# genome/breakdancer

Hardware: AMD Instinct MI355X
Metric: read-pairs/s, records resident in HBM -> scored SV table (SURVEY 8d timing i); end to end from BAM: config.timings.bam_to_table (vs_baseline is taken there) (higher is better)
Workload: dtype int32

## Files before the change

breakdancer_amd/csrc/bdx_api.hip:

```cpp
#include <hip/hip_runtime.h>

#include <algorithm>
#include <atomic>
#include <functional>
#include <memory>
#include <chrono>
#include <cmath>
#include <cstdio>
#include <cstddef>
#include <cstring>
#include <string>
#include <thread>
#include <unordered_map>
#include <utility>
#include <vector>

#include "../../include/bdx.h"
#include "bdx_buf.h"
#include "bdx_dev.h"
#include "bdx_k3.h"
#include "bdx_shard.h"
#include "bdx_scan.h"
#include "bdx_walk.h"
#include "bdx_bam_dev.h"
// ... 81 lines not shown
    std::vector<uint32_t> cnt;
    std::vector<uint32_t> cnt_local;
    uint32_t g_covered = 0;
    int32_t g_window = 0;
    uint32_t ntiles = 0, tstride = 0;
    Compact cp{};
    K3Arrays k3{};
    K4Arrays k4{};
    std::vector<double> log_tail;
    bool collect_support = false;
    std::vector<uint32_t> ov_cnt;
    uint32_t ov_covered = 0;
    bool replayed = false;
    bool use_stash = false;
    std::atomic<int> sizing{0};
    std::string sizing_err;
    std::vector<uint32_t> sup_off;
    std::vector<uint64_t> sup_idx;
    std::vector<uint8_t> sup_flag;
    std::vector<float> seqcov, lib_density, key_density;
    std::vector<HostRegion> regions;
    std::vector<uint32_t> r_pk;
    const HostRegion* reg = nullptr;
    size_t nreg = 0;
    const uint32_t* rpk = nullptr;
    std::vector<GroupPart> parts;
    WalkResult walk;
    std::unique_ptr<WalkScratch, void (*)(WalkScratch*)> walk_scratch{nullptr, walk_scratch_free};
    uint32_t n_printed = 0;
    uint32_t n_sv_host = 0;
    int speculate = 2;
    int spec_test = 0;
    uint32_t last_na = 0;
    size_t last_n = 0;
    uint32_t count_chunks = 0;
    uint32_t na_alloc = 0;
    bool region_of_fused = false;
    uint32_t join_table_clean = 0;
    float stage_ms[kNumStages] = {0};
    Event ev[8];

    Event ev_copy;
    bool copy_pending = false;
    bool k1_live = false;
    uint32_t k1_done = 0, k1_cap_tiles = 0;
    struct Stage {
        PinBuf buf;
        size_t cap = 0;
        Event done;
        bool busy = false;
    };
    Stage ring[4];
    int ring_next = 0, ring_cur = -1;
    struct KeySeg { uint64_t begin; const uint64_t* host; const uint16_t* host_qlen; const uint64_t* host_check; };
    std::vector<KeySeg> key_segs;
    DevBuf b_seg;

    size_t cls_n = (size_t)-1;
    DevBuf b_qin, b_qout;
    bool mark_dup = false;
    bool dup_done = false;
    uint64_t dup_marked = 0, dup_groups = 0;
    KdScratch kd;
};

namespace {

int fail(bdx_ctx* c, int code, const std::string& msg) {
    if (c) c->err = msg;
    return code;
}
#define NOT_WHILE_SIZING(c)                                                                                                              \
    do {                                                                                                                                 \
        if ((c)->sizing.load(std::memory_order_acquire))                                                                                 \
            return fail(c, BDX_ESTATE, "the buffers of the later stages are being sized on another thread (bdx_bamdec_finish has not returned)"); \
    } while (0)
int hipfail(bdx_ctx* c, hipError_t e, const char* what) {
    return fail(c, BDX_EHIP, std::string(what) + ": " + hipGetErrorString(e));
}
#define HIPCHK(ctx, expr)                                   \
    do {                                                    \
        hipError_t _e = (expr);                             \
        if (_e != hipSuccess) return hipfail(ctx, _e, #expr); \
    } while (0)
#define BDX_TRY(expr)                      \
    do {                                   \
        const int _rc = (expr);            \
        if (_rc != BDX_OK) return _rc;     \
    } while (0)

size_t round_up(size_t x, size_t m) { return (x + m - 1) / m * m; }

hipError_t next_lb_stamp(bdx_ctx* c, uint32_t* out) {
    if (((++c->lb_seq) & 0x3FFFFFFFu) == 0) {
        if (c->sb.b_lb.p) { const hipError_t e = hipMemsetAsync(c->sb.b_lb.p, 0, c->sb.b_lb.bytes, c->stream); if (e != hipSuccess) return e; }
        if (c->sb.b_ws6.p) { const hipError_t e = hipMemsetAsync(c->sb.b_ws6.p, 0, c->sb.b_ws6.bytes, c->stream); if (e != hipSuccess) return e; }
        ++c->lb_seq;
    }
    *out = c->lb_seq & 0x3FFFFFFFu;
    return hipSuccess;
}

int alloc_reads(bdx_ctx* c, size_t cap) {
    cap = round_up(std::max<size_t>(cap, 1), 1024);
    if (cap <= c->cap) return BDX_OK;
    if (c->copy_stream) HIPCHK(c, hipStreamSynchronize(c->copy_stream));
    HIPCHK(c, hipStreamSynchronize(c->stream));
    c->k1_live = false;
    struct Col { DevBuf* b; size_t esz; const void** slot; };
    Col cols[] = {{&c->b_tid, 4, (const void**)&c->d.tid},     {&c->b_pos, 4, (const void**)&c->d.pos},
                  {&c->b_mtid, 4, (const void**)&c->d.mtid},   {&c->b_mpos, 4, (const void**)&c->d.mpos},
                  {&c->b_isize, 4, (const void**)&c->d.isize}, {&c->b_flag, 2, (const void**)&c->d.flag},
                  {&c->b_qlen, 2, (const void**)&c->d.qlen},   {&c->b_mapq, 1, (const void**)&c->d.mapq},
                  {&c->b_lib, 1, (const void**)&c->d.lib},     {&c->b_bam, 1, (const void**)&c->d.bam},
                  {&c->b_key, 8, (const void**)&c->d.key},     {&c->b_check, 8, (const void**)&c->d.check}};
    for (Col& col : cols) {
        if (col.b == &c->b_check && !c->use_check) continue;
        DevBuf nb;
        HIPCHK(c, nb.ensure(cap * col.esz));
        if (c->n) HIPCHK(c, hipMemcpyAsync(nb.p, col.b->p, c->n * col.esz, hipMemcpyDeviceToDevice, c->stream));
        HIPCHK(c, hipStreamSynchronize(c->stream));
        col.b->release();
        *col.b = std::move(nb);
        *col.slot = col.b->p;
    }
    c->cap = cap;
    return BDX_OK;
}

void stage_view(const bdx_ctx::Stage& st, bdx_batch_buf* out) {
    char* p = (char*)st.buf.p;
    const size_t K = st.cap;
    out->name_key = (uint64_t*)p; p += K * 8;
    out->name_check = (uint64_t*)p; p += K * 8;
    out->tid = (int32_t*)p; p += K * 4;
    out->pos = (int32_t*)p; p += K * 4;
    out->mtid = (int32_t*)p; p += K * 4;
    out->mpos = (int32_t*)p; p += K * 4;
    out->isize = (int32_t*)p; p += K * 4;
    out->flag = (uint16_t*)p; p += K * 2;
    out->qlen = (uint16_t*)p; p += K * 2;
    out->mapq = (uint8_t*)p; p += K;
    out->lib = (uint8_t*)p; p += K;
    out->bam = (uint8_t*)p;
    out->capacity = K;
}

enum class RegionDst { HostAndHbm, Hbm };
struct StageDims {
    uint32_t na = 0;
    int nkeys = 0, nlibs = 0;
    bool use_check = false;
    bool k2_clears_join = false;
    RegionDst regions = RegionDst::HostAndHbm;
    bool groups_in_hbm = false, table_in_hbm = false;
    uint32_t k6_cap = 0;
    int big_walk = -1;
    uint32_t join_n = 0, join_own = 0, join_slots = 0;
    bool join_pair_lo = false;

    uint32_t join_groups() const { return join_n / 2 + 1; }
    uint32_t k6_regions() const { return std::max(na, k6_cap); }
    int walks_big() const { return big_walk >= 0 ? big_walk : (k6_regions() > 500000u ? 1 : 0); }
};

StageDims stage_dims(const bdx_ctx* c, uint32_t na) {
    StageDims d;
    d.na = na; d.nkeys = c->nkeys; d.nlibs = c->nlibs; d.use_check = c->use_check;
    d.k2_clears_join = c->force_direct_join || (!c->bucketed_join && na <= kDirectJoinMax);
    d.groups_in_hbm = c->groups_in_hbm; d.table_in_hbm = c->table_in_hbm; d.k6_cap = c->k6_cap;
    d.big_walk = c->big_walk_mode >= 0 ? c->big_walk_mode : (c->last_big_groups >= 0 ? (c->last_big_groups > 2000 ? 1 : 0) : -1);
    d.join_n = d.join_own = na; d.join_slots = d.k2_clears_join ? direct_join_slots(na) : 0;
    return d;
}

int pass1_prepare(bdx_ctx* c, uint32_t tiles_cap);
int presize_stages(bdx_ctx* c, const StageDims& dm);
int presize_stages_here(bdx_ctx* c, const StageDims& dm);
int pass1_classify(bdx_ctx* c, uint32_t upto, bool timed);

constexpr uint32_t kStreamTilesMin = 4096;

int enqueue_batch(bdx_ctx* c, const bdx_batch& b, bool lazy_keys) {
    if (c->n + b.n > c->cap) {
        BDX_TRY(alloc_reads(c, std::max(c->n + b.n, c->cap * 2)));
    }
    const size_t o = c->n, n = b.n;
    if (c->mark_dup && c->dup_done && o)
        return fail(c, BDX_ESTATE, "duplicates of this load are marked already: reads cannot be appended behind a run (bdx_reset_reads starts the next load)");
    hipStream_t s = c->copy_stream;
    if (o == 0) {
        c->key_segs.clear();
        const uint64_t tiles = (c->cap + kTile - 1) / kTile;
        if (tiles <= 0xFFFFFFFFull) {
            BDX_TRY(pass1_prepare(c, (uint32_t)tiles));
            c->k1_live = !c->mark_dup;
        }
    }
    hipStream_t s2 = s;
    HIPCHK(c, hipMemcpyAsync((void*)(c->d.tid + o), b.tid, n * 4, hipMemcpyHostToDevice, s));
    HIPCHK(c, hipMemcpyAsync((void*)(c->d.pos + o), b.pos, n * 4, hipMemcpyHostToDevice, s2));
    HIPCHK(c, hipMemcpyAsync((void*)(c->d.mtid + o), b.mtid, n * 4, hipMemcpyHostToDevice, s));
    HIPCHK(c, hipMemcpyAsync((void*)(c->d.mpos + o), b.mpos, n * 4, hipMemcpyHostToDevice, s2));
    HIPCHK(c, hipMemcpyAsync((void*)(c->d.isize + o), b.isize, n * 4, hipMemcpyHostToDevice, s));
    HIPCHK(c, hipMemcpyAsync((void*)(c->d.flag + o), b.flag, n * 2, hipMemcpyHostToDevice, s2));
    HIPCHK(c, hipMemcpyAsync((void*)(c->d.mapq + o), b.mapq, n, hipMemcpyHostToDevice, s2));
    if (c->nlibs > 1) HIPCHK(c, hipMemcpyAsync((void*)(c->d.lib + o), b.lib, n, hipMemcpyHostToDevice, s2));
    if (c->nbams > 1) HIPCHK(c, hipMemcpyAsync((void*)(c->d.bam + o), b.bam, n, hipMemcpyHostToDevice, s2));
    const uint64_t* dev_view = nullptr;
    const uint16_t* dev_qlen = nullptr;
    const uint64_t* dev_check = nullptr;
    if (lazy_keys && c->key_segs.size() < 64) {
        auto device_view = [](const void* hp) -> void* {
            hipPointerAttribute_t attr{};
            void* dp = nullptr;
            if (hipPointerGetAttributes(&attr, hp) == hipSuccess && attr.type == hipMemoryTypeHost &&
                hipHostGetDevicePointer(&dp, (void*)hp, 0) == hipSuccess)
                return dp;
            (void)hipGetLastError();
            return nullptr;
        };
        dev_view = (const uint64_t*)device_view(b.name_key);
        dev_qlen = dev_view ? (const uint16_t*)device_view(b.qlen) : nullptr;
        if (dev_qlen && c->use_check) dev_check = (const uint64_t*)device_view(b.name_check);
        if (!dev_qlen || (c->use_check && !dev_check)) dev_view = nullptr;
    }
    if (!dev_view) {
        HIPCHK(c, hipMemcpyAsync((void*)(c->d.key + o), b.name_key, n * 8, hipMemcpyHostToDevice, s2));
        HIPCHK(c, hipMemcpyAsync((void*)(c->d.qlen + o), b.qlen, n * 2, hipMemcpyHostToDevice, s));
        if (c->use_check) HIPCHK(c, hipMemcpyAsync((void*)(c->d.check + o), b.name_check, n * 8, hipMemcpyHostToDevice, s2));
    }
    if (c->key_segs.empty() || dev_view || c->key_segs.back().host)
        c->key_segs.push_back(bdx_ctx::KeySeg{(uint64_t)o, dev_view, dev_qlen, dev_check});
    HIPCHK(c, hipEventRecord(c->ev_copy, s));
    c->copy_pending = true;
    c->n += n;
    c->ran = false;
    if (o == 0) c->dup_done = false;
    if (c->k1_live) {
        const uint32_t full = (uint32_t)(c->n / kTile);
        if (full >= c->k1_done + kStreamTilesMin) {
            HIPCHK(c, hipStreamWaitEvent(c->stream, c->ev_copy, 0));
            c->copy_pending = false;
            BDX_TRY(pass1_classify(c, full, false));
        }
    }
    return BDX_OK;
}

}

extern "C" {

void bdx_opts_default(bdx_opts* o) {
    if (!o) return;
    o->min_len = 7; o->cut_sd = 3; o->max_sd = 1000000000; o->min_map_qual = 35; o->min_read_pair = 2;
    o->seq_coverage_lim = 1000; o->buffer_size = 100; o->transchr_rearrange = 0; o->fisher = 0;
    o->illumina_long_insert = 0; o->cn_lib = 0; o->print_af = 0; o->score_threshold = 30; o->chr_restricted = 0;
}

const char* bdx_strerror(int code) {
    switch (code) {
        case BDX_OK: return "ok";
        case BDX_EINVAL: return "invalid argument";
        case BDX_ENOMEM: return "out of memory";
        case BDX_EHIP: return "HIP runtime error";
        case BDX_ESTATE: return "call out of order";
        case BDX_ELIMIT: return "limit exceeded";
        default: return "internal error";
    }
}
const char* bdx_last_error(const bdx_ctx* ctx) { return ctx ? ctx->err.c_str() : ""; }
int bdx_device(const bdx_ctx* ctx) { return ctx ? ctx->device : -1; }
void* bdx_stream(const bdx_ctx* ctx) { return ctx ? (void*)ctx->stream : nullptr; }

int bdx_create(bdx_ctx** out, const bdx_opts* opts, const bdx_lib* libs, int nlibs, int nbams, int ntids,
               int max_read_window_size0, int device) {
    if (!out || !opts || !libs || nlibs < 1 || nbams < 1) return BDX_EINVAL;
    if (nlibs > 255 || nbams > 254) return BDX_ELIMIT;
    const int nkeys = opts->cn_lib ? nlibs : nbams;
    if (nkeys > 60) return BDX_ELIMIT;
    for (int i = 0; i < nlibs; ++i)
        if (libs[i].bam_index < 0 || libs[i].bam_index >= nbams) return BDX_EINVAL;
    int ndev = 0;
    if (hipGetDeviceCount(&ndev) != hipSuccess || ndev <= 0 || device < 0 || device >= ndev) return BDX_EHIP;
    if (hipSetDevice(device) != hipSuccess) return BDX_EHIP;
    std::unique_ptr<bdx_ctx> c(new (std::nothrow) bdx_ctx);
    if (!c) return BDX_ENOMEM;
    c->device = device;
    c->opts = *opts;
    c->libs.assign(libs, libs + nlibs);
    c->nlibs = nlibs; c->nbams = nbams; c->ntids = ntids; c->nkeys = nkeys; c->w0 = max_read_window_size0;
    if (c->stream.create(hipStreamNonBlocking) != hipSuccess) return BDX_EHIP;
    for (auto& e : c->ev)
        if (e.create() != hipSuccess) return BDX_EHIP;
    if (c->copy_stream.create(hipStreamNonBlocking) != hipSuccess) return BDX_EHIP;
    if (c->ev_copy.create(hipEventDisableTiming) != hipSuccess) return BDX_EHIP;
    for (auto& st : c->ring)
        if (st.done.create(hipEventDisableTiming) != hipSuccess) return BDX_EHIP;
    if (c->ev_groups.create(hipEventDisableTiming) != hipSuccess) return BDX_EHIP;
    if (c->ev_regions.create(hipEventDisableTiming) != hipSuccess) return BDX_EHIP;
    std::vector<DevLib> dl(nlibs);
    for (int i = 0; i < nlibs; ++i) {
        dl[i].upper = libs[i].uppercutoff;
        dl[i].lower = libs[i].lowercutoff;
        dl[i].min_mapq = libs[i].min_mapping_quality < 0 ? opts->min_map_qual : libs[i].min_mapping_quality;
        dl[i].key = opts->cn_lib ? i : libs[i].bam_index;
    }
    std::vector<float> means(nlibs);
    for (int i = 0; i < nlibs; ++i) means[i] = libs[i].mean_insertsize;
    if (c->b_libs.ensure(nlibs * sizeof(DevLib)) != hipSuccess ||
        hipMemcpy(c->b_libs.p, dl.data(), nlibs * sizeof(DevLib), hipMemcpyHostToDevice) != hipSuccess ||
        c->b_lib_mean.ensure(nlibs * 4) != hipSuccess ||
        hipMemcpy(c->b_lib_mean.p, means.data(), nlibs * 4, hipMemcpyHostToDevice) != hipSuccess)
        return BDX_EHIP;
    *out = c.release();
    return BDX_OK;
}

void bdx_destroy(bdx_ctx* c) {
    if (!c) return;
    (void)hipSetDevice(c->device);
// ... 323 lines not shown
    c->na_alloc = 0;
    c->regions.clear(); c->r_pk.clear(); c->parts.clear();
    c->reg = nullptr; c->nreg = 0; c->rpk = nullptr;
    c->walk.clear();
    if (!c->walk_scratch) c->walk_scratch.reset(walk_scratch_new());
    c->n_printed = 0;
    memset(&c->counts, 0, sizeof(c->counts));
    for (float& m : c->stage_ms) m = 0;

    if (c->copy_pending) {
        HIPCHK(c, hipStreamWaitEvent(s, c->ev_copy, 0));
        c->copy_pending = false;
    }
    if (!(c->k1_live && c->k1_cap_tiles >= ntiles)) {
        BDX_TRY(pass1_prepare(c, ntiles));
    }
    c->k1_live = false;
    if (c->mark_dup && c->k1_done == 0) {
        BDX_TRY(mark_duplicates(c));
    }
    const uint32_t tstride = c->tstride;
    const bool time_k1 = (c->stage_timing || c->seq % kK1EventPeriod == 0) && c->k1_done == 0 && ntiles > 0;
    {
        BDX_TRY(pass1_classify(c, ntiles, time_k1));
    }
    FinalizeParams fp{};
    fp.ntiles = ntiles; fp.tstride = tstride; fp.nblk = 0;
    fp.nfold = std::max<uint32_t>(1, std::min<uint32_t>(64, (ntiles + 1023) / 1024));
    HIPCHK(c, c->b_fold.ensure((size_t)nbams * fp.nfold * sizeof(MonoRec)));
    fp.fold_part = c->b_fold.as<MonoRec>();
    fp.nlibs = nlibs; fp.nbams = nbams; fp.nkeys = nkeys; fp.ncols = ncols; fp.ncnt = ncnt; fp.w0 = c->w0;
    fp.tile_tot = c->b_tile_tot.as<uint32_t>(); fp.tile_pre = c->b_tile_pre.as<uint32_t>(); fp.tile_mono = c->b_tile_mono.as<MonoRec>();
    {
        const uint32_t nsuper = (ntiles + kK2TilesPerWave - 1) / kK2TilesPerWave;
        const uint32_t round = 4096;
        const uint32_t rounds = std::max<uint32_t>(1, (nsuper + round - 1) / round);
        const uint32_t max_chunks = c->dbg_max_chunks > 0 ? (uint32_t)std::min(c->dbg_max_chunks, (int)kMaxChunks) : (uint32_t)kMaxChunks;
        fp.chunk_super = round * ((rounds + max_chunks - 1) / max_chunks);
        fp.nchunk = std::max<uint32_t>(1, (nsuper + fp.chunk_super - 1) / fp.chunk_super);
        HIPCHK(c, c->b_chunk_tot.ensure((size_t)ncols * kMaxChunks * 8));
        fp.chunk_tot = c->b_chunk_tot.as<uint32_t>();
        fp.chunk_base = fp.chunk_tot + (size_t)ncols * kMaxChunks;
    }
    fp.blk_cnt = c->b_blk_cnt.as<uint32_t>(); fp.cnt = c->b_cnt.as<uint32_t>(); fp.p1 = c->b_p1.as<Pass1>();
    HIPCHK(c, c->b_kdens.ensure(64 * 4));
    fp.libs = c->b_libs.as<DevLib>(); fp.cn_lib = c->opts.cn_lib; fp.key_density = c->b_kdens.as<float>();
    fp.cnt_host = c->h_cnt.as<uint32_t>(); fp.p1_host = c->h_p1.as<Pass1>();
    memset(c->h_p1.p, 0, sizeof(Pass1));
    HIPCHK(c, c->h_flags.ensure(64));
    ++c->seq;
    fp.flag_host = c->h_flags.as<uint32_t>(); fp.flag_value = c->seq;
    fp.na_cap = na_cap;
    fp.count_host = post_count && c->poll ? c->h_count.as<uint64_t>() : nullptr; fp.count_stamp = c->seq;
    c->count_chunks = fp.count_host ? fp.nchunk : 0;
    c->fp_deferred = fp;
    c->finalize2_deferred = defer_second;
    launch_finalize(fp, s, !defer_second);
    c->k1_timed = time_k1;
    return wait ? wait_pass1(c) : BDX_OK;
}

int wait_pass1(bdx_ctx* c) {
    const int ncnt = c->nlibs * kNumFlags + c->nlibs + c->nbams;
    if (!wait_flag(c, 0, c->seq)) {
        HIPCHK(c, hipStreamSynchronize(c->stream));
        if (c->h_flags.p && *((volatile uint32_t*)c->h_flags.p) != c->seq) return fail(c, BDX_EINTERNAL, "the pass-1 record did not arrive: its kernel was not launched");
    }
    c->p1 = *c->h_p1.as<Pass1>();
    c->cnt_local.assign(c->h_cnt.as<uint32_t>(), c->h_cnt.as<uint32_t>() + ncnt);
    if (c->k1_timed) {
        float ms = 0;
        if (hipEventElapsedTime(&ms, c->ev[0], c->ev[1]) == hipSuccess) c->k1_ms_last = ms;
    }
    c->stage_ms[0] = c->k1_ms_last;
    if (c->p1.n_anom > kMaxAnomalous) return fail(c, BDX_ELIMIT, "more than 2^31 anomalous reads in one context");
    if (!c->na_alloc && c->p1.n_anom) c->na_alloc = (uint32_t)std::min<uint64_t>((uint64_t)c->p1.n_anom + c->p1.n_anom / 8 + 1024, kMaxAnomalous);
    c->cls_n = c->n;
    return BDX_OK;
}

int32_t window_from(const bdx_ctx* c, const uint32_t* cnt, uint32_t covered) {
    int W = c->w0;
    for (int i = 0; i < c->nlibs; ++i) {
        const int nd = (int)(cnt[i * kNumFlags + F_LARGE] + cnt[i * kNumFlags + F_SMALL]);
        const int tmp = nd > 0 ? (int)((float)covered / (float)nd) : 50;
        W = std::min(W, tmp);
    }
    return W;
}

int set_pass1(bdx_ctx* c, const uint32_t* cnt, uint32_t covered, int32_t window, bool upload) {
    const int nlibs = c->nlibs, nkeys = c->nkeys;
    const int ncnt = nlibs * kNumFlags + nlibs + c->nbams;
    c->cnt.assign(cnt, cnt + ncnt);
    c->g_covered = covered;
    c->g_window = window;
    const uint32_t* lib_cnt = c->cnt.data() + nlibs * kNumFlags;
    const uint32_t* bam_cnt = lib_cnt + nlibs;
    c->seqcov.assign(nlibs, 0.f);
    c->lib_density.assign(nlibs, 0.f);
    c->key_density.assign(nkeys, 0.000001f);
    for (int i = 0; i < nlibs; ++i) {
        float covg = 0;
        if (lib_cnt[i] != 0 && covered != 0) covg = float(lib_cnt[i]) * c->libs[i].readlens / covered;
        c->seqcov[i] = covg;
        float dens = 0.000001f;
        if (c->opts.cn_lib) {
            if (lib_cnt[i] != 0) dens = float(lib_cnt[i]) / covered;
        } else {
            dens = float(bam_cnt[c->libs[i].bam_index]) / covered;
        }
        c->lib_density[i] = dens;
        c->key_density[c->opts.cn_lib ? i : c->libs[i].bam_index] = dens;
    }
    struct { uint32_t covered; int32_t window; } hdr{covered, window};
    static_assert(offsetof(Pass1, covered_ref_len) == 0 && offsetof(Pass1, window) == 4, "Pass1 header layout");
    if (upload) {
        HIPCHK(c, hipMemcpyAsync(c->b_p1.p, &hdr, sizeof(hdr), hipMemcpyHostToDevice, c->stream));
        HIPCHK(c, hipStreamSynchronize(c->stream));
    }
    return BDX_OK;
}

#define SZCHK(expr)                                                                                       \
    do {                                                                                                  \
        const hipError_t _e = (expr);                                                                     \
        if (_e != hipSuccess) { *err = std::string(#expr) + ": " + hipGetErrorString(_e); return BDX_EHIP; } \
    } while (0)

hipError_t size_c_maxq(StageBufs& b, size_t cap) { return b.b_c_maxq.ensure(cap * 4); }
hipError_t size_out_deg(StageBufs& b, size_t cap) { return b.b_out_deg.ensure(cap * 6 * 4); }
hipError_t size_join_words(StageBufs& b, size_t n_own, bool pair_lo) {
    const hipError_t e = b.b_partner.ensure(n_own * 4);
    return e == hipSuccess && pair_lo ? b.b_pair_lo.ensure(n_own * 4) : e;
}
hipError_t size_zero_once(DevBuf& b, size_t bytes, hipStream_t s) {
    if (b.bytes >= bytes) return hipSuccess;
    const hipError_t e = b.ensure(bytes);
    return e == hipSuccess ? hipMemsetAsync(b.p, 0, b.bytes, s) : e;
}

int size_compact(StageBufs& b, const StageDims& d, std::string* err) {
    if (!d.na) return BDX_OK;
    if (d.na > kMaxAnomalous) { *err = "more than 2^31 anomalous reads in one context"; return BDX_ELIMIT; }
    const size_t cap = d.na;
    SZCHK(b.b_c_tid.ensure(cap * 4)); SZCHK(b.b_c_pos.ensure(cap * 4)); SZCHK(b.b_c_isize.ensure(cap * 4));
    SZCHK(b.b_c_meta.ensure(cap * 4)); SZCHK(b.b_c_key.ensure(cap * 8)); SZCHK(b.b_c_nn.ensure(cap * 4));
    SZCHK(b.b_c_idx.ensure(cap * 4));
    if (d.use_check) SZCHK(b.b_c_check.ensure(cap * 8));
    SZCHK(b.b_c_pk.ensure(cap * 4 * d.nkeys));
    SZCHK(size_c_maxq(b, cap));
    if (d.k2_clears_join) {
        SZCHK(b.b_t_key.ensure((size_t)direct_join_slots(d.na) * 8));
        SZCHK(size_join_words(b, cap, true));
    }
    return BDX_OK;
}

int size_cut(StageBufs& b, const StageDims& d, hipStream_t s, std::string* err) {
    if (!d.na) return BDX_OK;
    const size_t cap = d.na;
    for (DevBuf* u : {&b.b_cand, &b.b_pre_q, &b.b_pre_rev, &b.b_pre_nonctx, &b.b_c_first, &b.b_c_rid, &b.b_region_of}) SZCHK(u->ensure(cap * 4));
    SZCHK(size_c_maxq(b, cap));
    if (d.regions != RegionDst::Hbm) {
        SZCHK(b.h_regs.ensure(cap * sizeof(RegionRec)));
        SZCHK(b.h_pk.ensure(cap * 2 * d.nkeys * 4));
    }
    SZCHK(b.b_r_rec.ensure(cap * sizeof(RegionRec)));
    SZCHK(b.b_r_pk.ensure(cap * 2 * d.nkeys * 4));
    if (d.regions == RegionDst::HostAndHbm) {
        SZCHK(size_out_deg(b, cap));
        SZCHK(b.h_counts0.ensure(sizeof(StageCounts)));
    }
    SZCHK(size_zero_once(b.b_lb, 5 * (scan_grid(d.na, 1) + 1) * 8, s));
    return BDX_OK;
}

int size_join(StageBufs& b, const StageDims& d, std::string* err) {
    if (!d.join_n) return BDX_OK;
    if (d.groups_in_hbm) SZCHK(b.b_groups.ensure((size_t)d.join_groups() * sizeof(GroupRec)));
    else SZCHK(b.h_groups.ensure((size_t)d.join_groups() * sizeof(GroupRec)));
    SZCHK(size_join_words(b, d.join_own, d.join_slots && d.join_pair_lo));
    if (d.join_slots) SZCHK(b.b_t_key.ensure((size_t)d.join_slots * 8));
    return BDX_OK;
}

struct K6Caps {
    uint32_t sv, term, cn, lib_stride;
    size_t p2, nsort;
};
K6Caps k6_caps(const StageDims& d) {
    K6Caps k{};
    const uint32_t na = d.k6_regions();
    k.sv = na / 2 + 1; k.term = na / 2 + 1; k.cn = (na / 2 + 1) * (uint32_t)d.nkeys;
    k.lib_stride = (uint32_t)std::min(d.nlibs, kK6LibStride);
    k.p2 = 1;
    while (k.p2 < k.sv) k.p2 <<= 1;
    k.nsort = std::min<size_t>(k.sv, kK6RankSortMax);
    return k;
}

int size_k6(StageBufs& b, const StageDims& d, hipStream_t s, std::string* err) {
    const size_t cap = d.k6_regions();
    if (!cap) return BDX_OK;
    const K6Caps k = k6_caps(d);
    SZCHK(size_out_deg(b, cap));
    SZCHK(b.b_parts.ensure(cap * sizeof(PartRec)));
    SZCHK(b.b_rs.ensure(cap * sizeof(RegSum)));
    SZCHK(b.b_members.ensure(cap * kK6MaxMembers * sizeof(MemberInfo)));
    SZCHK(b.b_own.ensure(cap * 7 * 4 + 64 * 4 * 4));
    if (d.walks_big()) SZCHK(b.b_member_ids.ensure(cap * kK6BigMembers * 4));
    SZCHK(b.b_slot.ensure(cap * sizeof(SvOut)));
    SZCHK(b.b_lib_stage.ensure(cap * k.lib_stride * sizeof(LibStage)));
    SZCHK(b.b_cn_stage.ensure(cap * (size_t)d.nkeys * sizeof(CnStage) + 16));
    SZCHK(b.b_t_lambda.ensure((size_t)k.term * 8)); SZCHK(b.b_t_k.ensure((size_t)k.term * 4));
    if (d.table_in_hbm) {
        SZCHK(b.b_sv_out.ensure((size_t)k.sv * sizeof(SvOut))); SZCHK(b.b_sv_key.ensure((size_t)k.sv * 8));
        SZCHK(b.b_lib_index_out.ensure((size_t)k.term * 4)); SZCHK(b.b_lib_pairs_out.ensure((size_t)k.term * 4));
        SZCHK(b.b_cn_key_out.ensure((size_t)k.cn * 4 + 16)); SZCHK(b.b_cn_value_out.ensure((size_t)k.cn * 4 + 16));
        SZCHK(b.b_ltail_out.ensure((size_t)k.term * 8));
    } else {
        SZCHK(b.h_sv_out.ensure((size_t)k.sv * sizeof(SvOut)));
        SZCHK(b.h_lib_index.ensure((size_t)k.term * 4)); SZCHK(b.h_lib_pairs.ensure((size_t)k.term * 4));
        SZCHK(b.h_cn_key.ensure((size_t)k.cn * 4 + 16)); SZCHK(b.h_cn_value.ensure((size_t)k.cn * 4 + 16));
        SZCHK(b.h_ltail_dev.ensure((size_t)k.term * 8));
    }
    SZCHK(b.h_counts2.ensure(sizeof(StageCounts)));
    SZCHK(b.b_sv_src.ensure((size_t)k.sv * 16)); SZCHK(b.b_ltail.ensure((size_t)k.term * 8));
    SZCHK(b.b_dlists.ensure((size_t)k.term * 4 + (size_t)k.cn * 8 + 64));
    SZCHK(b.b_ins.ensure(k.p2 * 12 + (size_t)k.sv * 8 + ((size_t)k.sv + 1) * 16 + k.nsort * 12 + k.nsort * 4 * kK6RankSlices + 64));
    SZCHK(size_zero_once(b.b_ws6, 4 * (scan_grid((uint32_t)cap, 1) + 1) * 8, s));
    return BDX_OK;
}

int do_compact(bdx_ctx* c) {
    HIPCHK(c, hipSetDevice(c->device));
    hipStream_t s = c->stream;
    const int nkeys = c->nkeys;
    const uint32_t na = c->na_alloc;
    if (c->stage_timing) HIPCHK(c, hipEventRecord(c->ev[2], s));
    Compact& cp = c->cp;
    cp = Compact{};
    c->k3 = K3Arrays{};
    if (na) {
        const StageDims dm = stage_dims(c, na);
        BDX_TRY(size_compact(c->sb, dm, &c->err));
        const StageBufs& b = c->sb;
        cp.tid = b.b_c_tid.as<int32_t>(); cp.pos = b.b_c_pos.as<int32_t>(); cp.isize = b.b_c_isize.as<int32_t>();
        cp.meta = b.b_c_meta.as<uint32_t>(); cp.key = b.b_c_key.as<uint64_t>(); cp.nn = b.b_c_nn.as<uint32_t>();
        cp.idx = b.b_c_idx.as<uint32_t>();
        cp.check = c->use_check ? b.b_c_check.as<uint64_t>() : nullptr;
        cp.pk = b.b_c_pk.as<uint32_t>(); cp.cap = na;
        K2Params k2{};
        k2.r = c->d; k2.n = c->n; k2.ntiles = c->ntiles; k2.tstride = c->tstride; k2.nkeys = nkeys; k2.nlibs = c->nlibs; k2.libs = c->b_libs.as<DevLib>();
        k2.cls = c->b_cls.as<uint8_t>(); k2.tile_pre = c->b_tile_pre.as<uint32_t>(); k2.c = cp;
        k2.tile_tot = c->b_tile_tot.as<uint32_t>(); k2.stash = c->use_stash ? c->b_stash.as<StashRec>() : nullptr;
        k2.chunk_tot = c->fp_deferred.chunk_tot; k2.chunk_base = c->fp_deferred.chunk_base; k2.chunk_super = c->fp_deferred.chunk_super;
        k2.fill_ptr[0] = b.b_c_maxq.as<uint32_t>(); k2.fill_words[0] = na; k2.fill_value[0] = 0u;
        c->join_table_clean = 0;
        if (dm.k2_clears_join) {
            const uint32_t slots = dm.join_slots;
            k2.fill_ptr[1] = b.b_t_key.as<uint32_t>(); k2.fill_words[1] = 2 * slots; k2.fill_value[1] = 0xFFFFFFFFu;
            k2.fill_ptr[2] = b.b_partner.as<uint32_t>(); k2.fill_words[2] = na; k2.fill_value[2] = 0xFFFFFFFFu;
            k2.fill_ptr[3] = b.b_pair_lo.as<uint32_t>(); k2.fill_words[3] = na; k2.fill_value[3] = 0xFFFFFFFFu;
            c->join_table_clean = slots;
        }
        {
            size_t ns = 0;
            BDX_TRY(upload_key_segs(c, &ns));
            if (ns) {
                k2.nseg = (int)ns;
                k2.seg_begin = c->b_seg.as<uint64_t>();
                k2.seg_ptr = (const uint64_t* const*)(c->b_seg.as<uint64_t>() + ns + 1);
                k2.seg_qlen = (const uint16_t* const*)(c->b_seg.as<uint64_t>() + 2 * ns + 1);
                k2.seg_check = (const uint64_t* const*)(c->b_seg.as<uint64_t>() + 3 * ns + 1);
            }
        }
        launch_k2(k2, k2_lds_bytes(nkeys), s, c->finalize2_deferred ? &c->fp_deferred : nullptr);
        c->finalize2_deferred = false;
    }
    if (c->finalize2_deferred) {
        launch_finalize2_only(c->fp_deferred, s);
        c->finalize2_deferred = false;
    }
    if (c->stage_timing) HIPCHK(c, hipEventRecord(c->ev[3], s));
    return BDX_OK;
}

void own_borrowed_regions(bdx_ctx* c) {
    if (!c->reg || (const void*)c->reg != c->sb.h_regs.p) return;
    const HostRegion* r = c->reg;
    const uint32_t* pk = c->rpk;
    const size_t n = c->nreg;
    std::vector<HostRegion> keep(r, r + n);
    std::vector<uint32_t> keep_pk;
    if (pk) keep_pk.assign(pk, pk + n * 2 * (size_t)c->nkeys);
    c->regions.swap(keep); c->r_pk.swap(keep_pk);
    c->reg = c->regions.data(); c->rpk = c->r_pk.data();
}

int do_cut(bdx_ctx* c, const uint32_t* tid_tail, RegionDst dst) {
    HIPCHK(c, hipSetDevice(c->device));
    hipStream_t s = c->stream;
    const uint32_t na = c->na_alloc;
    if (na) {
        StageDims dm = stage_dims(c, na);
        dm.regions = dst;
        BDX_TRY(size_cut(c->sb, dm, s, &c->err));
        const StageBufs& b = c->sb;
        K3Arrays& k3 = c->k3;
        const bool for_k6 = dst == RegionDst::HostAndHbm;
        k3.cap = na;
        k3.cand = b.b_cand.as<int32_t>(); k3.pre_q = b.b_pre_q.as<uint32_t>(); k3.pre_rev = b.b_pre_rev.as<uint32_t>();
        k3.pre_nonctx = b.b_pre_nonctx.as<uint32_t>(); k3.c_first = b.b_c_first.as<uint32_t>();
        k3.c_maxq = b.b_c_maxq.as<int32_t>(); k3.c_rid = b.b_c_rid.as<int32_t>(); k3.region_of = b.b_region_of.as<int32_t>();
        k3.r_rec = for_k6 ? b.h_regs.as<RegionRec>() : b.b_r_rec.as<RegionRec>();
        k3.r_pk = for_k6 ? b.h_pk.as<uint32_t>() : b.b_r_pk.as<uint32_t>();
        if (for_k6) {
            k3.r_rec_dev = b.b_r_rec.as<RegionRec>(); k3.r_pk_dev = b.b_r_pk.as<uint32_t>(); k3.out_deg = b.b_out_deg.as<uint32_t>();
            k3.host_copy_later = (!c->bucketed_join && na <= kDirectJoinMax) ? 1 : 0;
            memset(b.h_counts0.p, 0, sizeof(StageCounts));
            k3.counts_host = b.h_counts0.as<StageCounts>();
        } else {
            k3.r_rec_dev = nullptr; k3.r_pk_dev = nullptr; k3.host_copy_later = 0;
        }
        k3.lb_state = b.b_lb.as<unsigned long long>();
        HIPCHK(c, next_lb_stamp(c, &k3.lb_stamp));
        k3.counts = c->b_counts.as<StageCounts>();
        c->region_of_fused = for_k6 && !c->bucketed_join && na <= kDirectJoinMax;
        launch_k3(k3, c->cp, c->b_p1.as<Pass1>(), na, c->opts.min_len, c->opts.seq_coverage_lim, c->nkeys, tid_tail, !c->region_of_fused, s);
        if (for_k6 && !k3.host_copy_later) {
            BDX_TRY(signal_ready(c, 3, c->ev_regions));
        }
    }
    if (c->stage_timing) HIPCHK(c, hipEventRecord(c->ev[4], s));
    return BDX_OK;
}

int do_join_local(bdx_ctx* c, uint32_t n, const Entries& en, const uint32_t* n_ptr) {
    hipStream_t s = c->stream;
    K4Arrays& k4 = c->k4;
    k4 = K4Arrays{};
    if (!n) return BDX_OK;
    const bool direct = c->force_direct_join || (!c->bucketed_join && n <= kDirectJoinMax);
    StageDims dm = stage_dims(c, c->na_alloc);
    dm.join_n = n;
    dm.join_own = en.n_local ? std::min<uint32_t>(n, std::max<uint32_t>(c->na_alloc, 1u)) : n;
    dm.join_slots = !direct ? 0u : (c->join_table_clean && (uint64_t)n * 2 <= c->join_table_clean) ? c->join_table_clean : direct_join_slots(n);
    dm.join_pair_lo = en.want_pair_lo != 0;
    BDX_TRY(size_join(c->sb, dm, &c->err));
    StageBufs& b = c->sb;
    k4.g_cap = dm.join_groups();
    k4.g_rec = c->groups_in_hbm ? b.b_groups.as<GroupRec>() : b.h_groups.as<GroupRec>();
    k4.partner = b.b_partner.as<int32_t>();
    if (direct) {
        const uint32_t slots = dm.join_slots;
        const size_t n_own = dm.join_own;
        const bool want_lo = en.c_rid || en.want_pair_lo;
        if (c->join_table_clean != slots) {
            HIPCHK(c, hipMemsetAsync(b.b_t_key.p, 0xFF, (size_t)slots * 8, s));
            HIPCHK(c, hipMemsetAsync(b.b_partner.p, 0xFF, n_own * 4, s));
            if (en.want_pair_lo) HIPCHK(c, hipMemsetAsync(b.b_pair_lo.p, 0xFF, n_own * 4, s));
        }
        k4.pair_lo = ((c->join_table_clean == slots && want_lo) || en.want_pair_lo) ? b.b_pair_lo.as<int32_t>() : nullptr;
        c->join_table_clean = 0;
        k4.direct = 1; k4.t_mask = slots - 1;
        k4.t_key = b.b_t_key.as<uint64_t>(); k4.t_idx = b.b_t_idx.as<int32_t>();
        launch_k4_join_only(k4, en, n_ptr, n, c->b_counts.as<StageCounts>(), s);
        return BDX_OK;
    }
    uint32_t nb = 1, lg = 0;
    while (nb < (uint32_t)kMaxBuckets && (size_t)nb * 384 < n) { nb <<= 1; ++lg; }
    k4.nbuckets = nb; k4.log2b = lg;
    if ((size_t)nb * 4 > b.b_bcnt.bytes) {
        HIPCHK(c, b.b_bcnt.ensure((size_t)kMaxBuckets * 4));
        HIPCHK(c, hipMemsetAsync(b.b_bcnt.p, 0, b.b_bcnt.bytes, s));
    }
    HIPCHK(c, b.b_boff.ensure((nb + 1) * 4)); HIPCHK(c, b.b_bcur.ensure(nb * 4));
    HIPCHK(c, b.b_e_key.ensure((size_t)n * 8)); HIPCHK(c, b.b_e_idx.ensure((size_t)n * 4));
    HIPCHK(c, b.b_t_key.ensure((size_t)n * 16)); HIPCHK(c, b.b_t_idx.ensure((size_t)n * 8));
    k4.bcnt = b.b_bcnt.as<uint32_t>(); k4.boff = b.b_boff.as<uint32_t>(); k4.bcur = b.b_bcur.as<uint32_t>();
    k4.e_key = b.b_e_key.as<uint64_t>(); k4.e_idx = b.b_e_idx.as<uint32_t>();
    k4.t_key = b.b_t_key.as<uint64_t>(); k4.t_idx = b.b_t_idx.as<int32_t>();
    launch_k4_join_only(k4, en, n_ptr, n, c->b_counts.as<StageCounts>(), s);
    return BDX_OK;
}

constexpr uint32_t kBorrowRegionsMin = 32768;
void decode_regions(bdx_ctx* c, const RegionRec* rr, const uint32_t* pk, uint32_t nr, uint32_t ph, bool borrow) {
    static_assert(sizeof(HostRegion) == sizeof(RegionRec) && offsetof(HostRegion, first) == offsetof(RegionRec, first), "region layout");
    const int nkeys = c->nkeys;
    if (borrow && !ph) {
        c->reg = (const HostRegion*)rr; c->nreg = nr; c->rpk = pk;
        return;
    }
    c->regions.resize(nr + ph);
    if (ph) c->regions[0] = HostRegion{-1, -1, -1, 0, 0, 0, 0, 0, 0};
    if (nr) memcpy(c->regions.data() + ph, rr, (size_t)nr * sizeof(RegionRec));
    c->r_pk.assign((size_t)ph * 2 * nkeys, 0u);
    c->r_pk.insert(c->r_pk.end(), pk, pk + (size_t)nr * 2 * nkeys);
    c->reg = c->regions.data(); c->nreg = c->regions.size(); c->rpk = c->r_pk.data();
}

void decode_groups(bdx_ctx* c, const GroupRec* gr, uint32_t ng, uint32_t ph) {
    c->parts.resize(ng);
    for (uint32_t i = 0; i < ng; ++i) {
        const uint64_t k = gr[i].key;
        c->parts[i] = GroupPart{(uint32_t)(k >> 38) + ph, (uint32_t)((k >> 12) & ((1u << 26) - 1)) + ph, (uint8_t)(k & 15),
                                (uint8_t)((k >> 4) & 255), gr[i].pairs, gr[i].sum_isize};
    }
}

int k6_prepare(bdx_ctx* c, bool force_host, int rounds) {
    hipStream_t s = c->stream;
    K6Arrays& a = c->k6;
    a = K6Arrays{};
    const StageDims dm = stage_dims(c, c->na_alloc);
    const uint32_t na = dm.k6_regions();
    if (!na) return BDX_OK;
    BDX_TRY(size_k6(c->sb, dm, s, &c->err));
    const StageBufs& b = c->sb;
    const K6Caps k = k6_caps(dm);
    const int nkeys = c->nkeys, nlibs = c->nlibs;
    const size_t cap = na, p2 = k.p2, svc = k.sv, nsort = k.nsort;
    a.sv_cap = k.sv; a.term_cap = k.term; a.cn_cap = k.cn; a.lib_stride = k.lib_stride;
    a.old_key = b.b_ins.as<uint64_t>(); a.hs_key_dev = a.old_key + p2;
    a.old_slot = (uint32_t*)(a.hs_key_dev + svc); a.ins_T = a.old_slot + p2; a.ins_src = a.ins_T + svc + 1;
    a.ins_pre_l = a.ins_src + svc + 1; a.ins_pre_c = a.ins_pre_l + svc + 1;
    a.sorted_key = (uint64_t*)(((uintptr_t)(a.ins_pre_c + svc + 1) + 7) & ~(uintptr_t)7); a.sorted_slot = (uint32_t*)(a.sorted_key + nsort);
    a.rank_part = a.sv_cap > 2048u ? a.sorted_slot + nsort : nullptr;
    a.sv_begin = b.b_sv_src.as<uint2>(); a.sv_src = (uint32_t*)(a.sv_begin + a.sv_cap); a.ltail = b.b_ltail.as<double>();
    a.d_lib_index = b.b_dlists.as<int32_t>(); a.d_cn_key = a.d_lib_index + a.term_cap; a.d_cn_value = (float*)(a.d_cn_key + a.cn_cap);
    a.cap = na;
    a.r_rec = c->k6_r_rec ? c->k6_r_rec : b.b_r_rec.as<RegionRec>(); a.r_pk = c->k6_r_pk ? c->k6_r_pk : b.b_r_pk.as<uint32_t>();
    a.taint = c->k6_taint;
    a.region_of = c->k3.region_of; a.partner = c->k4.partner; a.pair_lo = c->k4.pair_lo; a.meta = c->cp.meta; a.isize = c->cp.isize;
    a.in_groups = c->k6_in_groups; a.in_goff = c->k6_in_goff; a.first_of = c->k6_in_groups ? c->k6_in_goff : nullptr;
    a.parts = b.b_parts.as<PartRec>();
    a.rs = b.b_rs.as<RegSum>();
    a.out_deg = b.b_out_deg.as<uint32_t>(); a.label = a.out_deg + cap; a.bad_v = a.out_deg + 2 * cap; a.bad = a.out_deg + 3 * cap;
    a.mcount = a.out_deg + 4 * cap; a.pcount = a.out_deg + 5 * cap;
    a.members = b.b_members.as<MemberInfo>();
    a.own_nsv = b.b_own.as<uint32_t>(); a.own_nacc = a.own_nsv + cap; a.own_ncn = a.own_nsv + 2 * cap; a.own_first = a.own_nsv + 3 * cap; a.slot_next = a.own_nsv + 4 * cap; a.owners = a.own_nsv + 5 * cap; a.owners_big = a.own_nsv + 6 * cap; a.emit_part = a.own_nsv + 7 * cap;
    a.big_walk = dm.walks_big();
    a.member_ids = a.big_walk ? b.b_member_ids.as<uint32_t>() : nullptr;
    a.sv_stage = b.b_slot.as<SvOut>(); a.lib_stage = b.b_lib_stage.as<LibStage>(); a.cn_stage = b.b_cn_stage.as<CnStage>();
    if (c->table_in_hbm) {
        a.sv_out = b.b_sv_out.as<SvOut>(); a.lib_index = b.b_lib_index_out.as<int32_t>(); a.lib_pairs = b.b_lib_pairs_out.as<int32_t>();
        a.cn_key = b.b_cn_key_out.as<int32_t>(); a.cn_value = b.b_cn_value_out.as<float>();
        a.sv_key = b.b_sv_key.as<unsigned long long>();
    } else {
        a.sv_out = b.h_sv_out.as<SvOut>(); a.lib_index = b.h_lib_index.as<int32_t>(); a.lib_pairs = b.h_lib_pairs.as<int32_t>();
        a.cn_key = b.h_cn_key.as<int32_t>(); a.cn_value = b.h_cn_value.as<float>();
    }
    a.sv_vx = a.sv_key ? a.sv_src + a.sv_cap : nullptr;
    a.t_lambda = b.b_t_lambda.as<double>(); a.t_k = b.b_t_k.as<int32_t>();
    a.g_rec = c->k4.g_rec; a.g_cap = c->k4.g_cap;
    a.lb_state = b.b_ws6.as<unsigned long long>();
    HIPCHK(c, next_lb_stamp(c, &a.lb_stamp));
    a.counts = c->b_counts.as<StageCounts>();
    a.hist = c->b_cnt.as<uint32_t>();
    a.key_density = c->b_kdens.as<float>();
    a.lib_mean = c->b_lib_mean.as<float>();
    a.counts_host = c->h_counts.as<StageCounts>();
    a.counts_host2 = b.h_counts2.as<StageCounts>();
    memset(c->h_counts.p, 0, sizeof(StageCounts));
    memset(b.h_counts2.p, 0, sizeof(StageCounts));
    a.p1 = c->b_p1.as<Pass1>();
    a.nlibs = nlibs; a.nkeys = nkeys; a.min_read_pair = c->opts.min_read_pair; a.chr_restricted = c->opts.chr_restricted;
    a.period = std::max(1, c->opts.buffer_size + 1);
    a.force_host = force_host ? 1 : 0;
    a.ins_plain = c->dbg_ins_plain;
    a.asm_plain = c->dbg_asm_plain;
    a.propagation_rounds = rounds ? rounds : (a.big_walk ? kK6LabelRoundsBig : kK6LabelRounds);
    if (c->poll) {
        a.flag_value = c->seq;
        a.flag_groups = c->h_flags.as<uint32_t>() + 1;
        if (c->k3.host_copy_later) a.flag_regions = c->h_flags.as<uint32_t>() + 3;
        a.mirror_in_walk = force_host ? 0 : 1;
    }
    return BDX_OK;
}

void k6_pairs(bdx_ctx* c) {
    if (c->k6.cap) launch_k6_pairs(c->k6, c->k6.cap, c->stream);
}
int k6_then_walk(bdx_ctx* c, void (*first)(const K6Arrays&, uint32_t, hipStream_t)) {
    const K6Arrays& a = c->k6;
    if (!a.cap) return BDX_OK;
    first(a, a.cap, c->stream);
    if (!c->poll) BDX_TRY(signal_ready(c, 1, c->ev_groups));
    launch_k6_walk(a, a.cap, c->stream);
    return BDX_OK;
}

int presize_stages(bdx_ctx* c, const StageDims& dm) {
    struct Guard {
        bdx_ctx* c;
        explicit Guard(bdx_ctx* c_) : c(c_) { c->sizing.fetch_add(1, std::memory_order_acq_rel); c->sizing_err.clear(); }
        ~Guard() { c->sizing.fetch_sub(1, std::memory_order_acq_rel); }
    } guard(c);
    std::string* err = &c->sizing_err;
    SZCHK(hipSetDevice(c->device));
    own_borrowed_regions(c);
    BDX_TRY(size_compact(c->sb, dm, err));
    BDX_TRY(size_cut(c->sb, dm, c->stream, err));
    BDX_TRY(size_join(c->sb, dm, err));
    return size_k6(c->sb, dm, c->stream, err);
}

int presize_stages_here(bdx_ctx* c, const StageDims& dm) {
    const int r = presize_stages(c, dm);
    if (r != BDX_OK) c->err = c->sizing_err;
    return r;
}

int do_k6_table(bdx_ctx* c) {
    hipStream_t s = c->stream;
    K6Arrays& a = c->k6;
    const uint32_t na = a.cap;
    if (!na) return BDX_OK;
    const WalkResult& H = c->walk;
    const uint32_t nh = (uint32_t)H.svs.size(), nt = (uint32_t)H.terms.size(), nc = (uint32_t)H.cn_key.size();
    a.nh = nh;
    if (nh) {
        const uint64_t period = (uint64_t)std::max(1, c->opts.buffer_size + 1);
        HIPCHK(c, c->h_hs_rec.ensure((size_t)nh * sizeof(SvOut)));
        HIPCHK(c, c->h_hs_aux.ensure((size_t)nh * 12 + 16));
        HIPCHK(c, c->h_hs_lists.ensure((size_t)nt * 16 + (size_t)nc * 8 + 16));
        memcpy(c->h_hs_rec.p, H.svs.data(), (size_t)nh * sizeof(HostSv));
        uint64_t* hkey = c->h_hs_aux.as<uint64_t>();
        uint32_t* hcnt = (uint32_t*)(hkey + nh);
        for (uint32_t j = 0; j < nh; ++j) {
            const uint64_t key = H.sv_key[j];
            const bool from_old = !((key >> 32) & 1ull);
            const uint64_t start = key & 0xffffffffull;
            const uint64_t T = from_old ? (key >> 33) * period : start;
            hkey[j] = (T << 34) | (from_old ? 0ull : 1ull << 33) | (start << 7);
            if (a.force_host) hkey[j] = 0;
            hcnt[j] = (uint32_t)H.svs[j].sv.lib_count | ((uint32_t)H.svs[j].sv.cn_count << 16);
        }
        double* lam = c->h_hs_lists.as<double>();
        int32_t* li = (int32_t*)(lam + nt);
        int32_t* lp = li + nt;
        int32_t* ck = lp + nt;
        float* cv = (float*)(ck + nc);
        for (uint32_t i = 0; i < nt; ++i) { lam[i] = H.terms[i].lambda; li[i] = H.lib_index[i]; lp[i] = H.lib_pairs[i]; }
        for (uint32_t i = 0; i < nc; ++i) { ck[i] = H.cn_key[i]; cv[i] = H.cn_value[i]; }
        a.hs_rec = c->h_hs_rec.as<SvOut>(); a.hs_key = hkey; a.hs_cnt = hcnt;
        a.hs_lambda = lam; a.hs_lib_index = li; a.hs_lib_pairs = lp; a.hs_cn_key = ck; a.hs_cn_value = cv;
    }
    a.ltail_host = c->table_in_hbm ? c->sb.b_ltail_out.as<double>() : (c->opts.fisher ? c->sb.h_ltail_dev.as<double>() : nullptr);
    a.fin_regions = (c->counts.n_regions && c->counts.n_regions <= na) ? c->counts.n_regions : na;
    HIPCHK(c, c->h_printed.ensure((size_t)k6_score_grid(a) * 4));
    a.printed_host = c->h_printed.as<uint32_t>();
    if (c->poll) { a.flag_done = c->h_flags.as<uint32_t>() + 2; a.flag_value = c->seq; }
    a.wire_rows = c->table_in_hbm ? 0 : 1;
    c->rows_packed = a.wire_rows != 0;
    launch_k6_table(a, na, std::log(10), c->opts.score_threshold, c->opts.fisher ? 0 : 1, s);
    if (!a.flag_done) {
        BDX_TRY(signal_ready(c, 2, nullptr));
    }
    return BDX_OK;
}

int materialize(bdx_ctx* c) {
    if (c->materialized) return BDX_OK;
    WalkResult& M = c->walk;
    M.clear();
    const uint32_t n = c->n_sv_total, nt = c->n_terms_total, nc = c->n_cn_total;
    if (c->rows_packed) {
        const SvWire* w = c->sb.h_sv_out.as<SvWire>();
        M.svs.resize(n);
        int32_t lb = 0, cb = 0;
        for (uint32_t i = 0; i < n; ++i) {
            const SvWire& r = w[i];
            HostSv& o = M.svs[i];
            bdx_sv& v = o.sv;
            const HostRegion& ra = c->reg[r.region[0]];
            const HostRegion& rb = r.region[1] >= 0 ? c->reg[r.region[1]] : ra;
            v.chr[0] = ra.tid; v.chr[1] = rb.tid;
            v.pos[0] = r.pos[0]; v.pos[1] = r.pos[1];
            v.fwd[0] = (int32_t)(ra.n - ra.rev); v.rev[0] = (int32_t)ra.rev;
            v.fwd[1] = (int32_t)(rb.n - rb.rev); v.rev[1] = (int32_t)rb.rev;
            v.flag = (int32_t)((r.bits >> 16) & 15u); v.size = r.size; v.score = r.score; v.num_reads = r.num_reads; v.printed = (int32_t)((r.bits >> 23) & 1u);
            v.region[0] = r.region[0]; v.region[1] = r.region[1];
            v.lib_begin = lb; v.lib_count = (int32_t)(r.bits & 255u); lb += v.lib_count;
            v.cn_begin = cb; v.cn_count = (int32_t)((r.bits >> 8) & 255u); cb += v.cn_count;
            v.allele_frequency = r.allele_frequency; v.logp = r.logp;
            o.grp_mask = (r.bits >> 20) & 7u; o.start = r.start;
        }
    } else {
        const HostSv* d = c->sb.h_sv_out.as<HostSv>();
        M.svs.assign(d, d + n);
    }
    M.lib_index.assign(c->sb.h_lib_index.as<int32_t>(), c->sb.h_lib_index.as<int32_t>() + nt);
    M.lib_pairs.assign(c->sb.h_lib_pairs.as<int32_t>(), c->sb.h_lib_pairs.as<int32_t>() + nt);
    M.cn_key.assign(c->sb.h_cn_key.as<int32_t>(), c->sb.h_cn_key.as<int32_t>() + nc);
    M.cn_value.assign(c->sb.h_cn_value.as<float>(), c->sb.h_cn_value.as<float>() + nc);
    if (c->opts.fisher) c->log_tail.assign(c->sb.h_ltail_dev.as<double>(), c->sb.h_ltail_dev.as<double>() + nt); else c->log_tail.clear();
    M.n_groups = c->n_groups_total;
    c->materialized = true;
    return BDX_OK;
}

int finish_table(bdx_ctx* c) {
    hipStream_t s = c->stream;
    const auto tf0 = std::chrono::steady_clock::now();
    if (!wait_flag(c, 2, c->seq)) {
        HIPCHK(c, hipStreamSynchronize(s));
        if (!flag_arrived(c, 2)) return fail(c, BDX_EINTERNAL, "the SV table did not arrive: its kernels were not launched");
    }
    const auto tf1 = std::chrono::steady_clock::now();
    static_assert(sizeof(HostSv) == sizeof(SvOut) && offsetof(HostSv, grp_mask) == offsetof(SvOut, grp_mask) &&
                      offsetof(HostSv, start) == offsetof(SvOut, start), "SV record layout");
    c->n_sv_host = (uint32_t)c->walk.svs.size();
    c->n_groups_total = c->walk.n_groups + c->counts.n_groups_dev;
    const StageCounts c2 = *c->sb.h_counts2.as<StageCounts>();
    if (c2.overflow) return fail(c, BDX_EINTERNAL, "SV list overflow");
    c->n_sv_total = c2.n_sv_dev; c->n_terms_total = c2.n_terms_dev; c->n_cn_total = c2.n_cn_dev;
    c->counts.n_sv_dev = c2.n_sv_dev - c->n_sv_host;
    {
        const uint32_t g = c->k6.printed_host ? k6_score_grid(c->k6) : 0u;
        const uint32_t* pb = c->k6.printed_host;
        uint32_t np = 0;
        for (uint32_t i = 0; i < g; ++i) np += pb[i];
        c->n_printed = np;
    }
    c->counts.n_old = c2.n_old;
    c->materialized = false;
    if (c->opts.fisher && !c->table_in_hbm) {
        materialize(c);
        finish_scores(c->opts, c->log_tail.data(), c->walk.svs.data(), c->walk.svs.size(), &c->n_printed);
    }
    const auto tf2 = std::chrono::steady_clock::now();
    c->stage_ms[8] = ms_between(tf0, tf1);
    c->stage_ms[9] = ms_between(tf1, tf2);
    c->stage_ms[10] = 0;
    c->ran = true;
    return BDX_OK;
}

int host_walk(bdx_ctx* c, int32_t last_maxq, bool any_anomalous) {
    HIPCHK(c, hipSetDevice(c->device));
    WalkInput wi{};
    wi.opts = c->opts; wi.libs = c->libs.data(); wi.nlibs = c->nlibs; wi.nbams = c->nbams; wi.nkeys = c->nkeys;
    wi.hist = c->cnt.data(); wi.covered_ref_len = c->g_covered; wi.key_density = c->key_density.data();
    wi.regions = c->reg; wi.nregions = c->nreg; wi.r_pk = c->rpk; wi.parts = &c->parts; wi.last_maxq = last_maxq;
    wi.any_anomalous = any_anomalous;
    c->walk.clear();
    if (!c->parts.empty()) greedy_walk(wi, c->walk_scratch.get(), c->walk);
    return BDX_OK;
}

int score_host_terms(bdx_ctx* c) {
    hipStream_t s = c->stream;
    const uint32_t nt = (uint32_t)c->walk.terms.size();
    if (nt) {
        HIPCHK(c, c->h_terms.ensure((size_t)nt * 20 + 16));
        double* hl = c->h_terms.as<double>();
        int32_t* hk = (int32_t*)(hl + nt);
        double* ho = (double*)((char*)c->h_terms.p + (((size_t)nt * 12 + 7) & ~(size_t)7));
        for (uint32_t i = 0; i < nt; ++i) { hl[i] = c->walk.terms[i].lambda; hk[i] = c->walk.terms[i].k; }
        launch_k5(hl, hk, ho, nt, s);
    }
    return BDX_OK;
}

int finish_host_walk(bdx_ctx* c) {
    hipStream_t s = c->stream;
    HIPCHK(c, hipStreamSynchronize(s));
    HIPCHK(c, hipGetLastError());
    const uint32_t nt = (uint32_t)c->walk.terms.size();
    const double* host_tail = nt ? (const double*)((char*)c->h_terms.p + (((size_t)nt * 12 + 7) & ~(size_t)7)) : nullptr;
    c->log_tail.assign(host_tail, host_tail + nt);
    finish_scores(c->opts, c->log_tail.data(), c->walk.svs.data(), c->walk.svs.size(), &c->n_printed);
    c->n_sv_host = c->n_sv_total = (uint32_t)c->walk.svs.size();
    c->n_terms_total = nt; c->n_cn_total = (uint32_t)c->walk.cn_key.size();
    c->n_groups_total = c->walk.n_groups;
    c->counts.n_sv_dev = 0;
    c->materialized = true;
    c->ran = true;
    return BDX_OK;
}

int collect_support(bdx_ctx* c, uint32_t ph) {
    c->sup_off.assign(1, 0);
    c->sup_idx.clear();
    c->sup_flag.clear();
    const uint32_t na = c->p1.n_anom;
    std::vector<int32_t> partner(na), region_of(na);
    std::vector<uint32_t> idx(na), meta(na);
    if (na) {
        HIPCHK(c, hipMemcpy(partner.data(), c->k4.partner, (size_t)na * 4, hipMemcpyDeviceToHost));
        HIPCHK(c, hipMemcpy(region_of.data(), c->k3.region_of, (size_t)na * 4, hipMemcpyDeviceToHost));
        HIPCHK(c, hipMemcpy(idx.data(), c->cp.idx, (size_t)na * 4, hipMemcpyDeviceToHost));
        HIPCHK(c, hipMemcpy(meta.data(), c->cp.meta, (size_t)na * 4, hipMemcpyDeviceToHost));
    }
    std::vector<std::pair<uint32_t, uint32_t>> pairs;
    for (const HostSv& hs : c->walk.svs) {
        pairs.clear();
        const uint32_t rA = (uint32_t)hs.sv.region[0], rB = (uint32_t)hs.sv.region[1];
        const uint32_t glo[3] = {rA, rA, rB}, ghi_[3] = {rA, rB, rB};
        for (uint32_t g = 0; g < 3; ++g) {
            if (!(hs.grp_mask & (1u << g))) continue;
            const uint32_t lo = glo[g], hi = ghi_[g];
            const uint32_t f = c->reg[hi].first, n = c->reg[hi].n;
            for (uint32_t j = f; j < f + n; ++j) {
                const int32_t p = partner[j];
                if (p < 0 || (uint32_t)p >= j) continue;
                if ((uint32_t)(region_of[p] + (int32_t)ph) != lo) continue;
                pairs.emplace_back(j, (uint32_t)p);
            }
        }
        std::sort(pairs.begin(), pairs.end());
        for (auto const& pr : pairs) {
            c->sup_idx.push_back(idx[pr.first]); c->sup_flag.push_back((uint8_t)meta_flag(meta[pr.first]));
            c->sup_idx.push_back(idx[pr.second]); c->sup_flag.push_back((uint8_t)meta_flag(meta[pr.second]));
        }
        c->sup_off.push_back((uint32_t)c->sup_idx.size());
    }
    return BDX_OK;
}

int replay_arrays(bdx_ctx* c, uint32_t na, const uint64_t* key, const int32_t* region_of, const uint32_t* meta, const int32_t* isize, uint32_t ph,
                  std::vector<uint32_t>* sup) {
    ReadWalkInput ri{};
    WalkInput& wi = ri.base;
    wi.opts = c->opts; wi.libs = c->libs.data(); wi.nlibs = c->nlibs; wi.nbams = c->nbams; wi.nkeys = c->nkeys;
    wi.hist = c->cnt.data(); wi.covered_ref_len = c->g_covered; wi.key_density = c->key_density.data();
    wi.regions = c->reg; wi.nregions = c->nreg; wi.r_pk = c->rpk; wi.parts = nullptr; wi.last_maxq = c->counts.last_maxq;
    wi.any_anomalous = na != 0;
    ri.n_reads = na; ri.key = key; ri.region_of = region_of; ri.meta = meta; ri.isize = isize;
    ri.phantom = ph;
    if (sup) { ri.support_off = &c->sup_off; ri.support = sup; }
    c->walk.clear();
    read_level_walk(ri, c->walk);
    c->counts.n_groups = 0; c->counts.n_pairs = 0;
    int rc = score_host_terms(c);
    if (rc == BDX_OK) rc = finish_host_walk(c);
    if (rc != BDX_OK) return rc;
    c->replayed = true;
    return BDX_OK;
}

void unify_names(uint64_t* key, const uint64_t* check, size_t n) {
    struct PairHash {
        size_t operator()(const std::pair<uint64_t, uint64_t>& p) const { return (size_t)(p.first ^ (p.second * 0x9E3779B97F4A7C15ull)); }
    };
    std::unordered_map<std::pair<uint64_t, uint64_t>, uint64_t, PairHash> ids;
    ids.reserve(n);
    for (size_t i = 0; i < n; ++i) key[i] = ids.emplace(std::make_pair(key[i], check[i]), (uint64_t)ids.size()).first->second;
}

int replay_reads(bdx_ctx* c, uint32_t ph) {
    hipStream_t s = c->stream;
    HIPCHK(c, hipStreamSynchronize(s));
    const uint32_t na = c->p1.n_anom;
    std::vector<uint64_t> key(na);
    std::vector<int32_t> region_of(na), isize(na);
    std::vector<uint32_t> meta(na);
    HIPCHK(c, hipMemcpy(key.data(), c->cp.key, (size_t)na * 8, hipMemcpyDeviceToHost));
    HIPCHK(c, hipMemcpy(region_of.data(), c->k3.region_of, (size_t)na * 4, hipMemcpyDeviceToHost));
    HIPCHK(c, hipMemcpy(meta.data(), c->cp.meta, (size_t)na * 4, hipMemcpyDeviceToHost));
    HIPCHK(c, hipMemcpy(isize.data(), c->cp.isize, (size_t)na * 4, hipMemcpyDeviceToHost));
    if (c->cp.check && na) {
        std::vector<uint64_t> check(na);
        HIPCHK(c, hipMemcpy(check.data(), c->cp.check, (size_t)na * 8, hipMemcpyDeviceToHost));
        unify_names(key.data(), check.data(), na);
    }
    if (ph)
        for (int32_t& r : region_of)
            if (r >= 0) r += (int32_t)ph;
    std::vector<uint32_t> sup;
    BDX_TRY(replay_arrays(c, na, key.data(), region_of.data(), meta.data(), isize.data(), ph, c->collect_support ? &sup : nullptr));
    if (c->collect_support) {
        std::vector<uint32_t> idx(na);
        HIPCHK(c, hipMemcpy(idx.data(), c->cp.idx, (size_t)na * 4, hipMemcpyDeviceToHost));
        c->sup_idx.resize(sup.size());
        c->sup_flag.resize(sup.size());
        for (size_t i = 0; i < sup.size(); ++i) { c->sup_idx[i] = idx[sup[i]]; c->sup_flag[i] = (uint8_t)meta_flag(meta[sup[i]]); }
    }
    return BDX_OK;
}

}

extern "C" {

int bdx_run(bdx_ctx* c) {
    if (!c) return BDX_EINVAL;
    NOT_WHILE_SIZING(c);
    const auto t_begin = std::chrono::steady_clock::now();
    hipStream_t s = c->stream;
    const bool ph_opt = 0 > c->opts.min_len && 0.0f < (float)c->opts.seq_coverage_lim;
    const bool force_host = c->host_walk_only || ph_opt || c->opts.min_read_pair < 1;
    auto enqueue_middle = [&]() -> int {
        BDX_TRY(do_compact(c));
        BDX_TRY(do_cut(c, nullptr, RegionDst::HostAndHbm));
        if (!c->na_alloc) return BDX_OK;
        Entries en{};
        en.key = c->cp.key; en.check = c->cp.check; en.region = c->k3.region_of; en.meta = c->cp.meta; en.isize = c->cp.isize;
        if (c->region_of_fused) {
            en.cand = c->k3.cand; en.c_rid = c->k3.c_rid; en.region_out = c->k3.region_of;
            en.k6_scratch = c->k3.out_deg; en.scratch_cap = c->k3.cap;
            if (c->k3.host_copy_later) {
                en.r_rec_dev = c->k3.r_rec_dev; en.r_pk_dev = c->k3.r_pk_dev; en.r_rec_host = c->k3.r_rec; en.r_pk_host = c->k3.r_pk;
                en.counts = c->b_counts.as<StageCounts>(); en.nkeys2 = 2 * c->nkeys;
            }
        }
        BDX_TRY(do_join_local(c, c->na_alloc, en, &c->b_p1.as<Pass1>()->n_anom));
        if (c->k3.host_copy_later && !c->poll) {
            BDX_TRY(signal_ready(c, 3, c->ev_regions));
        }
        BDX_TRY(k6_prepare(c, force_host, 0));
        return k6_then_walk(c, launch_k6_groups);
    };
    uint32_t guess = 0;
    const bool restored = !c->ov_cnt.empty();
    if (!restored && c->speculate == 2 && c->ran && c->last_n == c->n && c->last_na) {
        guess = c->spec_test ? std::max(1u, c->last_na / 2) : c->last_na + c->last_na / 8 + 1024;
        if (guess > kMaxAnomalous) guess = 0;
    } else if (!restored && c->speculate && c->n >= (1u << 20) && (c->speculate == 1 || c->n < (1u << 25))) {
        const uint64_t prior = (uint64_t)c->n / (c->spec_test ? 4096 : 32) + 4096;
        guess = prior > kMaxAnomalous ? 0 : (uint32_t)prior;
    }
    int rc;
    if (restored) {
        BDX_TRY(do_pass1(c));
        BDX_TRY(set_pass1(c, c->ov_cnt.data(), c->ov_covered, window_from(c, c->ov_cnt.data(), c->ov_covered), true));
        HIPCHK(c, hipMemcpyAsync(c->b_cnt.p, c->ov_cnt.data(), c->ov_cnt.size() * 4, hipMemcpyHostToDevice, s));
        HIPCHK(c, hipMemcpyAsync(c->b_kdens.p, c->key_density.data(), c->key_density.size() * 4, hipMemcpyHostToDevice, s));
        HIPCHK(c, hipStreamSynchronize(s));
        BDX_TRY(enqueue_middle());
    } else if (guess) {
        BDX_TRY(do_pass1(c, guess, false, true));
        c->na_alloc = guess;
        BDX_TRY(enqueue_middle());
        BDX_TRY(wait_pass1(c));
        BDX_TRY(set_pass1(c, c->cnt_local.data(), c->p1.covered_ref_len, c->p1.window, false));
        if (c->p1.n_anom > guess) {
            HIPCHK(c, hipStreamSynchronize(s));
            HIPCHK(c, hipMemcpy(&c->b_p1.as<Pass1>()->n_anom, &c->p1.n_anom, 4, hipMemcpyHostToDevice));
            HIPCHK(c, hipMemset(c->b_counts.p, 0, sizeof(StageCounts)));
            ++c->seq;
            c->na_alloc = c->p1.n_anom;
            BDX_TRY(enqueue_middle());
        }
    } else {
        BDX_TRY(do_pass1(c, 0, false, false, true));
        uint64_t count = 0;
        if (wait_count(c, &count)) {
            if (count > kMaxAnomalous) {
                HIPCHK(c, hipStreamSynchronize(s));
                return fail(c, BDX_ELIMIT, "more than 2^31 anomalous reads in one context");
            }
            if (count) c->na_alloc = (uint32_t)std::min<uint64_t>(count + count / 8 + 1024, kMaxAnomalous);
            BDX_TRY(enqueue_middle());
            BDX_TRY(wait_pass1(c));
            if (c->p1.n_anom != count) {
                HIPCHK(c, hipStreamSynchronize(s));
                return fail(c, BDX_EINTERNAL, "the count of anomalous reads posted ahead of the pass-1 record differs from the record's");
            }
            BDX_TRY(set_pass1(c, c->cnt_local.data(), c->p1.covered_ref_len, c->p1.window, false));
        } else {
            BDX_TRY(wait_pass1(c));
            BDX_TRY(set_pass1(c, c->cnt_local.data(), c->p1.covered_ref_len, c->p1.window, false));
            BDX_TRY(enqueue_middle());
        }
    }
    c->last_n = c->n;
    c->last_na = c->p1.n_anom;
    const uint32_t na = c->p1.n_anom;
    const uint32_t ph = (na && ph_opt) ? 1u : 0u;
    if (c->stage_timing) HIPCHK(c, hipEventRecord(c->ev[5], s));
    const auto t_h0 = std::chrono::steady_clock::now();
    auto t_h1 = t_h0;
    if (na) {
        if (!wait_flag(c, 3, c->seq)) {
            if (c->poll) HIPCHK(c, hipStreamSynchronize(s)); else HIPCHK(c, hipEventSynchronize(c->ev_regions));
            if (!flag_arrived(c, 3)) return fail(c, BDX_EINTERNAL, "the region table did not arrive: its kernels were not launched");
        }
        if ((uint64_t)c->sb.h_counts0.as<StageCounts>()->n_regions + ph > kMaxRegions) {
            HIPCHK(c, hipStreamSynchronize(s));
            return fail(c, BDX_ELIMIT, "more than 2^26 - 2 accepted regions in one context");
        }
        const uint32_t nr_host = c->sb.h_counts0.as<StageCounts>()->n_regions;
        const bool copy_first = c->dbg_regions_copy == 1 || (c->dbg_regions_copy == 0 && nr_host < kBorrowRegionsMin);
        if (copy_first) decode_regions(c, c->sb.h_regs.as<RegionRec>(), c->sb.h_pk.as<uint32_t>(), nr_host, ph, false);
        if (!wait_flag(c, 1, c->seq)) {
            if (c->poll) HIPCHK(c, hipStreamSynchronize(s)); else HIPCHK(c, hipEventSynchronize(c->ev_groups));
            if (!flag_arrived(c, 1)) return fail(c, BDX_EINTERNAL, "the pair groups did not arrive: their kernels were not launched");
        }
        c->counts = *c->h_counts.as<StageCounts>();
        if (!copy_first) decode_regions(c, c->sb.h_regs.as<RegionRec>(), c->sb.h_pk.as<uint32_t>(), nr_host, ph,
                                        c->dbg_regions_copy == 2 || (uint64_t)c->counts.n_groups * 8 < nr_host);
        if (c->counts.irregular) {
            t_h1 = std::chrono::steady_clock::now();
            BDX_TRY(replay_reads(c, ph));
            const auto t_r = std::chrono::steady_clock::now();
            c->stage_ms[4] = ms_between(t_h0, t_h1); c->stage_ms[5] = ms_between(t_h1, t_r); c->stage_ms[7] = ms_between(t_begin, t_r);
            return BDX_OK;
        }
        if (c->counts.overflow) return fail(c, BDX_EINTERNAL, "group list overflow");
        decode_groups(c, c->sb.h_groups.as<GroupRec>(), c->counts.n_groups, ph);
        c->last_big_groups = (int64_t)c->counts.n_groups + c->counts.n_groups_big;
    }
    t_h1 = std::chrono::steady_clock::now();
    BDX_TRY(host_walk(c, c->counts.last_maxq, na != 0));
    const auto t_h2 = std::chrono::steady_clock::now();
    if (na) {
        BDX_TRY(do_k6_table(c));
        rc = finish_table(c);
    } else {
        rc = finish_host_walk(c);
    }
    if (rc != BDX_OK) return rc;
    if (c->collect_support) {
        materialize(c);
        BDX_TRY(collect_support(c, ph));
    }
    const auto t_end = std::chrono::steady_clock::now();
    if (c->stage_timing) {
        (void)hipEventSynchronize(c->ev[5]);
        auto evms = [&](int a, int b) { float ms = 0; (void)hipEventElapsedTime(&ms, c->ev[a], c->ev[b]); return ms; };
        c->stage_ms[1] = evms(2, 3);
        c->stage_ms[2] = evms(3, 4);
        c->stage_ms[3] = evms(4, 5);
    }
    c->stage_ms[4] = ms_between(t_h0, t_h1);
    c->stage_ms[5] = ms_between(t_h1, t_h2);
    c->stage_ms[6] = ms_between(t_h2, t_end);
    c->stage_ms[7] = ms_between(t_begin, t_end);
    return BDX_OK;
}

int bdx_get_summary(const bdx_ctx* c, bdx_summary* o) {
    if (!c || !o) return BDX_EINVAL;
    if (!c->ran) return BDX_ESTATE;
    o->n_reads = c->n; o->n_anomalous = c->p1.n_anom; o->covered_ref_len = c->g_covered; o->window = c->g_window;
    o->n_candidates = c->counts.n_cand; o->n_regions = (uint32_t)c->nreg; o->n_pairs = c->counts.n_pairs;
    o->n_groups = c->n_groups_total; o->n_svs = c->n_sv_total; o->n_svs_printed = c->n_printed;
    return BDX_OK;
}

int bdx_get_counters(const bdx_ctx* c, uint32_t* lib_read_count, uint32_t* bam_read_count, uint32_t* flag_hist, float* seqcov,
                     float* density) {
    if (!c) return BDX_EINVAL;
    if (!c->ran) return BDX_ESTATE;
    const uint32_t* hist = c->cnt.data();
    const uint32_t* lib_cnt = hist + c->nlibs * kNumFlags;
    const uint32_t* bam_cnt = lib_cnt + c->nlibs;
    if (flag_hist) memcpy(flag_hist, hist, (size_t)c->nlibs * kNumFlags * 4);
    if (lib_read_count) memcpy(lib_read_count, lib_cnt, (size_t)c->nlibs * 4);
    if (bam_read_count) memcpy(bam_read_count, bam_cnt, (size_t)c->nbams * 4);
    if (seqcov) memcpy(seqcov, c->seqcov.data(), (size_t)c->nlibs * 4);
    if (density) memcpy(density, c->lib_density.data(), (size_t)c->nlibs * 4);
    return BDX_OK;
}

int bdx_get_regions(const bdx_ctx* c, bdx_region* out, size_t cap) {
    if (!c || (!out && cap)) return BDX_EINVAL;
    if (!c->ran) return BDX_ESTATE;
    const size_t n = std::min(cap, c->nreg);
    for (size_t i = 0; i < n; ++i) {
        const HostRegion& r = c->reg[i];
        const int valid = c->opts.chr_restricted ? (int)r.nonctx : (int)r.n;
        out[i] = bdx_region{r.tid, r.start, r.end, (int32_t)r.nnormal, (int32_t)(r.n - r.rev), (int32_t)r.rev, (int32_t)r.n,
                            valid >= c->opts.min_read_pair ? 1 : 0, r.maxq};
// ... 374 lines not shown
```

breakdancer_amd/csrc/bdx_k3.h:

```cpp
#pragma once
#include "../../include/bdx.h"
#include "bdx_dev.h"

namespace bdx {

struct U4;

struct StageCounts {
    uint32_t n_cand;
    uint32_t n_regions;
    int32_t last_maxq;
    uint32_t n_pairs;
    uint32_t n_groups;
    uint32_t n_entries;
    uint32_t overflow;
    uint32_t n_printed;
    uint32_t n_sv_dev;
    uint32_t n_terms_dev;
    uint32_t n_cn_dev;
    uint32_t n_groups_dev;
    uint32_t stage_sv;
    uint32_t stage_lib;
    uint32_t stage_cn;
    uint32_t n_owners;
    uint32_t n_owners_big;
    uint32_t n_groups_big;
    uint32_t n_old;
    uint32_t n_ins;
    uint32_t sort_done;
    uint32_t irregular;
};

struct RegionRec {
    int32_t tid, start, end;
    uint32_t n, rev, nonctx, nnormal;
    int32_t maxq;
    uint32_t first;
};

struct GroupRec {
    uint64_t key;
    uint32_t pairs;
    uint32_t sum_isize;
};

struct K3Arrays {
    uint32_t cap;
    int32_t* cand;
    uint32_t *pre_q, *pre_rev, *pre_nonctx;
    uint32_t* c_first;
    int32_t* c_maxq;
    int32_t* c_rid;
    int32_t* region_of;
    RegionRec* r_rec;
    uint32_t* r_pk;
    RegionRec* r_rec_dev;
    uint32_t* r_pk_dev;
    int host_copy_later;
    uint32_t* out_deg;
    unsigned long long* lb_state;
    uint32_t lb_stamp;
    StageCounts* counts;
    StageCounts* counts_host;
};

void launch_k3(const K3Arrays& a, const Compact& cp, const Pass1* p1, uint32_t n_anom_host, int min_len, int seq_coverage_lim,
               int nkeys, const uint32_t* tid_tail, bool region_of_launch, hipStream_t s);

constexpr int kMaxBuckets = 8192;
constexpr int kJoinLdsSlots = 8192;
constexpr uint32_t kDirectJoinMax = 1u << 22;
inline uint32_t direct_join_slots(uint32_t n) {
    uint32_t slots = 1024;
    while (slots < 4 * (uint64_t)n) slots <<= 1;
    return slots;
}

struct K4Arrays {
    uint32_t nbuckets;
    uint32_t log2b;
    uint32_t* bcnt;
    uint32_t* boff;
    uint32_t* bcur;
    uint64_t* e_key;
    uint32_t* e_idx;
    int32_t* partner;
    int32_t* pair_lo;
    uint64_t* t_key;
    int32_t* t_idx;
    uint32_t direct;
    uint32_t t_mask;
    GroupRec* g_rec;
    uint32_t g_cap;
};

__host__ __device__ __forceinline__ uint64_t group_pack(uint32_t rlo, uint32_t rhi, uint32_t lib, uint32_t flag) {
    return ((uint64_t)rlo << 38) | ((uint64_t)rhi << 12) | ((uint64_t)lib << 4) | (uint64_t)flag;
}
constexpr uint32_t kMaxRegions = (1u << 26) - 2;
constexpr uint32_t kMaxAnomalous = 0x7FFFFF00u;

struct Entries {
    const uint64_t* key;
    const uint64_t* check;
    const int32_t* region;
    const uint32_t* meta;
    const int32_t* isize;
    const int32_t* cand;
    const int32_t* c_rid;
    int32_t* region_out;
    const RegionRec* r_rec_dev;
    const uint32_t* r_pk_dev;
    RegionRec* r_rec_host;
    uint32_t* r_pk_host;
    const StageCounts* counts;
    int nkeys2;
    uint32_t* k6_scratch;
    uint32_t scratch_cap;
    const uint32_t* n_local;
    const uint64_t* fkey;
    const uint64_t* fcheck;
    const int32_t* fregion;
    int want_pair_lo;
};

void launch_k4_join_only(const K4Arrays& k4, const Entries& e, const uint32_t* n_ptr, uint32_t n_upper, StageCounts* counts, hipStream_t s);

constexpr int kMaxRanks = 64;
struct ExchangeEntry {
    uint64_t key;
    uint32_t order;
    int32_t region;
    uint32_t meta;
    int32_t isize;
    uint64_t check;
};
static_assert(sizeof(ExchangeEntry) == 32, "exchange entries travel as four 64-bit words");
__host__ __device__ __forceinline__ uint32_t exchange_owner(uint64_t k, uint32_t world) {
    k = (k ^ (k >> 33)) * 0xff51afd7ed558ccdull;
    k ^= k >> 29;
    return (uint32_t)(k % world);
}
struct GatherPackage { uint64_t regions_off, pk_off, groups_off; uint32_t nr, ng; };
struct GatherDesc { GatherPackage p[kMaxRanks]; int world; };
void launch_k8_place_regions(const char* all, const GatherDesc& D, uint32_t max_nr, const uint64_t* rbase, int ntids, int nkeys2, RegionRec* r_rec,
                             uint32_t* r_pk, uint32_t* err, hipStream_t s);

void launch_k5(const double* lambda, const int32_t* k, double* out, uint32_t n, hipStream_t s);

constexpr int kK6MaxMembers = 4;
constexpr int kK6MaxIn = 3;
constexpr int kK6BigMembers = 64;
constexpr int kK6LibStride = 16;
constexpr int kK6LabelRoundsBig = 8;
constexpr uint32_t kK6RankSlices = 16;
constexpr uint32_t kK6RankSortMax = 1u << 17;
constexpr int kK6LabelRounds = 2;
constexpr int kK6LabelRoundsGather = 3;

struct RegSum {
    uint32_t np_all;
    uint32_t np_emit;
    uint32_t np_self;
    uint32_t w_self;
    uint32_t n_in;
    uint32_t n_pairs;
    uint32_t n_weak;
    uint32_t big;
    uint32_t e_lo[kK6MaxIn];
    uint32_t e_w[kK6MaxIn];
    uint32_t e_off[kK6MaxIn];
    uint32_t e_cnt[kK6MaxIn];
};
constexpr uint64_t kWeakPart = 1ull << 63;

struct PartRec {
    uint64_t key;
    uint32_t pairs;
    uint32_t sum;
};

struct MemberInfo {
    uint32_t r;
    RegionRec rec;
    uint32_t np_all, np_self, w_self, n_in;
    uint32_t e_lo[kK6MaxIn], e_w[kK6MaxIn], e_off[kK6MaxIn], e_cnt[kK6MaxIn];
    uint32_t stored;
    uint32_t pad;
};
constexpr int kMemberWords = sizeof(MemberInfo) / 4;

struct SvOut {
    bdx_sv sv;
    uint32_t grp_mask;
    uint32_t start;
};

struct SvWire {
    int32_t pos[2], region[2];
    int32_t size, score, num_reads;
    float allele_frequency;
    double logp;
    uint32_t start;
    uint32_t bits;
};
static_assert(sizeof(SvWire) == 48, "twelve 32-bit words");
constexpr int kWireWords = sizeof(SvWire) / 4;

struct LibStage { int32_t lib, rc; double lambda; };
struct CnStage { int32_t key; float value; };

struct K6Arrays {
    uint32_t cap;
    const RegionRec* r_rec;
    const uint32_t* r_pk;
    const int32_t* region_of;
    const int32_t* partner;
    const int32_t* pair_lo;
    const uint32_t* meta;
    const int32_t* isize;
    const GroupRec* in_groups;
    const uint32_t* in_goff;
    const uint32_t* first_of;
    PartRec* parts;
    RegSum* rs;
    uint32_t* out_deg;
    uint32_t* label;
    uint32_t* bad_v;
    uint32_t* bad;
    uint32_t* mcount;
    uint32_t* pcount;
    MemberInfo* members;
    uint32_t* owners;
    uint32_t* own_nsv;
    uint32_t* own_nacc;
    uint32_t* own_ncn;
    uint32_t* own_first;
    uint32_t* slot_next;
    uint32_t* emit_part;
    uint32_t* owners_big;
    uint32_t* member_ids;
    SvOut* sv_stage;
    LibStage* lib_stage;
    CnStage* cn_stage;
    uint32_t lib_stride;
    uint32_t* sv_src;
    uint2* sv_begin;
    uint32_t* sv_vx;
    int32_t* d_lib_index;
    int32_t* d_cn_key;
    float* d_cn_value;
    double* t_lambda;
    int32_t* t_k;
    SvOut* sv_out;
    int32_t* lib_index;
    int32_t* lib_pairs;
    int32_t* cn_key;
    float* cn_value;
    uint32_t sv_cap, term_cap, cn_cap;
    double* ltail;
    uint32_t* printed_host;
    double* ltail_host;
    const SvOut* hs_rec;
    const uint64_t* hs_key;
    const uint32_t* hs_cnt;
    uint64_t* old_key;
    uint32_t* old_slot;
    uint64_t* sorted_key;
    uint32_t* sorted_slot;
    uint32_t* rank_part;
    uint64_t* hs_key_dev;
    uint32_t* ins_T;
    uint32_t* ins_src;
    uint32_t* ins_pre_l;
    uint32_t* ins_pre_c;
    const int32_t* hs_lib_index;
    const int32_t* hs_lib_pairs;
    const double* hs_lambda;
    const int32_t* hs_cn_key;
    const float* hs_cn_value;
    uint32_t nh;
    GroupRec* g_rec;
    uint32_t g_cap;
    unsigned long long* lb_state;
    uint32_t lb_stamp;
    StageCounts* counts;
    StageCounts* counts_host;
    StageCounts* counts_host2;
    uint32_t* flag_regions;
    uint32_t* flag_groups;
    uint32_t* flag_done;
    uint32_t flag_value;
    const uint32_t* hist;
    const float* key_density;
    const float* lib_mean;
    const Pass1* p1;
    int nlibs, nkeys, min_read_pair, chr_restricted, period, force_host;
    int mirror_in_walk;
    int big_walk;
    uint32_t fin_regions;
    int asm_plain;
    int ins_plain;
    int propagation_rounds;
    uint8_t* taint;
    int wire_rows;
    unsigned long long* sv_key;
};

void launch_k6_groups(const K6Arrays& a, uint32_t n_anom_host, hipStream_t s);
void launch_k6_pairs(const K6Arrays& a, uint32_t n_upper, hipStream_t s);
void launch_k6_components(const K6Arrays& a, uint32_t n_upper, hipStream_t s);
void launch_k6_scratch_init(uint32_t* out_deg, uint32_t cap, hipStream_t s);
void launch_k6_walk(const K6Arrays& a, uint32_t n_anom_host, hipStream_t s);
void launch_k6_table(const K6Arrays& a, uint32_t n_anom_host, double ln10, int score_threshold, int with_scores, hipStream_t s);
uint32_t k6_score_grid(const K6Arrays& a);

}
```

breakdancer_amd/csrc/bdx_scan.h:

```cpp
#pragma once
#include "bdx_dev.h"

namespace bdx {

#ifdef BDX_KPROF
static __device__ unsigned long long g_kprof[8 * 65536];
#define KPROF(row, col) do { if ((threadIdx.x & 63) == 0 && (row) < 65536u) g_kprof[(size_t)(row) * 8 + (col)] = wall_clock64(); } while (0)
#else
#define KPROF(row, col) do {} while (0)
#endif

struct U4 {
    uint32_t x, y, z, w;
};
__host__ __device__ __forceinline__ U4 operator+(const U4& a, const U4& b) { return U4{a.x + b.x, a.y + b.y, a.z + b.z, a.w + b.w}; }
__host__ __device__ __forceinline__ U4 operator-(const U4& a, const U4& b) { return U4{a.x - b.x, a.y - b.y, a.z - b.z, a.w - b.w}; }

template <class T> __device__ __forceinline__ T zero_of();
template <> __device__ __forceinline__ uint32_t zero_of<uint32_t>() { return 0u; }
template <> __device__ __forceinline__ U4 zero_of<U4>() { return U4{0, 0, 0, 0}; }

__device__ __forceinline__ uint32_t shfl_up_t(uint32_t v, int o) { return __shfl_up(v, o); }
__device__ __forceinline__ U4 shfl_up_t(const U4& v, int o) {
    return U4{(uint32_t)__shfl_up(v.x, o), (uint32_t)__shfl_up(v.y, o), (uint32_t)__shfl_up(v.z, o), (uint32_t)__shfl_up(v.w, o)};
// ... 42 lines not shown
        if (j < n) acc = acc + in(j, n);
    }
    T tot;
    block_incl_scan(acc, s_ws, &tot);
    if (threadIdx.x == 0) blk[blockIdx.x] = tot;
}

template <class T, class In, int kIters> __global__ __launch_bounds__(kScanBlock) void scan_phase1(In in, const uint32_t* n_ptr, T* blk) {
    scan_phase1_body<T, In, kIters>(in, n_ptr, blk);
}

template <class T, int kIters> __global__ __launch_bounds__(1024) void scan_phase2(T* blk, const uint32_t* n_ptr, T* total) {
    constexpr int kScanChunk = kScanBlock * kIters;
    __shared__ T s_ws[16];
    __shared__ T s_carry;
    const uint32_t n = *n_ptr;
    const uint32_t nb = (n + kScanChunk - 1) / kScanChunk;
    const int lane = threadIdx.x & 63, w = threadIdx.x >> 6;
    if (threadIdx.x == 0) s_carry = zero_of<T>();
    __syncthreads();
    for (uint32_t base = 0; base < nb; base += 1024) {
        const uint32_t i = base + threadIdx.x;
        T v = i < nb ? blk[i] : zero_of<T>();
        T inc = wave_incl_scan_t(v);
        if (lane == 63) s_ws[w] = inc;
        __syncthreads();
        T off = s_carry;
        for (int k = 0; k < w; ++k) off = off + s_ws[k];
        if (i < nb) blk[i] = off + inc - v;
        __syncthreads();
        if (threadIdx.x == 1023) s_carry = off + inc;
        __syncthreads();
    }
    if (threadIdx.x == 0) *total = s_carry;
}

template <class T, class In, class Out, int kIters, bool kSelfSum>
__global__ __launch_bounds__(kScanBlock) void scan_phase3(In in, Out out, const uint32_t* n_ptr, const T* blk) {
    constexpr int kScanChunk = kScanBlock * kIters;
    __shared__ T s_ws[kScanBlock / 64];
    const uint32_t n = *n_ptr;
    const uint32_t base = blockIdx.x * kScanChunk;
    if (base >= n) return;
    T carry;
    if (kSelfSum) {
        T acc = zero_of<T>();
        for (uint32_t i = threadIdx.x; i < blockIdx.x; i += kScanBlock) acc = acc + blk[i];
        block_incl_scan(acc, s_ws, &carry);
    } else {
        carry = blk[blockIdx.x];
    }
#pragma unroll 1
    for (int it = 0; it < kIters; ++it) {
        const uint32_t j = base + it * kScanBlock + threadIdx.x;
        if (base + it * kScanBlock >= n) break;
        T e = j < n ? in(j, n) : zero_of<T>();
        T tot;
        T inc = carry + block_incl_scan(e, s_ws, &tot);
        if (j < n) out(j, n, inc, e);
        carry = carry + tot;
    }
}

inline uint32_t scan_grid(uint32_t n_upper, int iters = kScanIters) {
    const uint32_t chunk = (uint32_t)(kScanBlock * iters);
    return n_upper ? (n_upper + chunk - 1) / chunk : 1;
}

constexpr uint32_t kScanSelfSumMax = 1024;

template <class T, int kIters = kScanIters, class In, class Out>
void scan_launch(In in, Out out, const uint32_t* n_ptr, uint32_t n_upper, T* blk_ws, T* total, hipStream_t s) {
    const uint32_t g = scan_grid(n_upper, kIters);
    hipLaunchKernelGGL((scan_phase1<T, In, kIters>), dim3(g), dim3(kScanBlock), 0, s, in, n_ptr, blk_ws);
    if (g <= kScanSelfSumMax) {
        hipLaunchKernelGGL((scan_phase3<T, In, Out, kIters, true>), dim3(g), dim3(kScanBlock), 0, s, in, out, n_ptr, blk_ws);
        return;
    }
    hipLaunchKernelGGL((scan_phase2<T, kIters>), dim3(1), dim3(1024), 0, s, blk_ws, n_ptr, total);
    hipLaunchKernelGGL((scan_phase3<T, In, Out, kIters, false>), dim3(g), dim3(kScanBlock), 0, s, in, out, n_ptr, blk_ws);
}

template <class T> struct ScanCols;
template <> struct ScanCols<uint32_t> {
    static constexpr int n = 1;
    __device__ static __forceinline__ uint32_t get(const uint32_t& v, int) { return v; }
    __device__ static __forceinline__ void set(uint32_t& v, int, uint32_t x) { v = x; }
};
template <> struct ScanCols<U4> {
    static constexpr int n = 4;
    __device__ static __forceinline__ uint32_t get(const U4& v, int c) { return c == 0 ? v.x : c == 1 ? v.y : c == 2 ? v.z : v.w; }
    __device__ static __forceinline__ void set(U4& v, int c, uint32_t x) { if (c == 0) v.x = x; else if (c == 1) v.y = x; else if (c == 2) v.z = x; else v.w = x; }
};

template <class T>
__device__ __forceinline__ T lookback_exclusive(const T& tot, unsigned long long* state, uint32_t stamp, uint32_t bid, uint32_t* s_prefix ) {
    constexpr int kCols = ScanCols<T>::n;
    constexpr int kWin = 64 / kCols;
    const unsigned long long stamp_bits = (unsigned long long)(stamp & 0x3FFFFFFFu) << 32;
    if (threadIdx.x < 64) {
        const int lane = threadIdx.x;
        if (lane < kCols)
            __hip_atomic_store(&state[(size_t)bid * kCols + lane],
                               (unsigned long long)ScanCols<T>::get(tot, lane) | stamp_bits | ((bid == 0 ? 2ull : 1ull) << 62), __ATOMIC_RELAXED,
                               __HIP_MEMORY_SCOPE_AGENT);
        const int col = lane / kWin, k = lane % kWin;
        uint32_t acc = 0;
        bool frozen = false;
        constexpr int kAhead = 4;
        for (uint32_t back = 0;; back += kWin * kAhead) {
            unsigned long long w[kAhead];
#pragma unroll
            for (int u = 0; u < kAhead; ++u) {
                const int64_t pred = (int64_t)bid - 1 - (int64_t)back - (int64_t)u * kWin - k;
                w[u] = (2ull << 62) | stamp_bits;
                if (!frozen && pred >= 0) w[u] = __hip_atomic_load(&state[(size_t)pred * kCols + col], __ATOMIC_RELAXED, __HIP_MEMORY_SCOPE_AGENT);
            }
            bool done = false;
#pragma unroll
            for (int u = 0; u < kAhead; ++u) {
                if (done) break;
                const int64_t pred = (int64_t)bid - 1 - (int64_t)back - (int64_t)u * kWin - k;
                unsigned long long x = w[u];
                if (!frozen && pred >= 0)
                    while ((x & (0x3FFFFFFFull << 32)) != stamp_bits || (x >> 62) == 0)
                        x = __hip_atomic_load(&state[(size_t)pred * kCols + col], __ATOMIC_RELAXED, __HIP_MEMORY_SCOPE_AGENT);
                const uint32_t val = (uint32_t)x, st = (uint32_t)(x >> 62);
                const uint64_t incl = __ballot(!frozen && st == 2);
                const uint64_t mine = kWin == 64 ? incl : ((incl >> (col * kWin)) & ((1ull << kWin) - 1));
                const int stop = mine ? __builtin_ctzll(mine) : kWin;
                uint32_t part = (!frozen && k <= stop) ? val : 0u;
#pragma unroll
                for (int o = 1; o < kWin; o <<= 1) part += __shfl_xor(part, o);
                acc += part;
                if (mine) frozen = true;
                if (!__ballot(!frozen)) done = true;
            }
            if (done) break;
        }
        if (k == 0) s_prefix[col] = acc;
    }
    __syncthreads();
    T carry = zero_of<T>();
#pragma unroll
    for (int c = 0; c < kCols; ++c) ScanCols<T>::set(carry, c, s_prefix[c]);
    if (threadIdx.x < kCols && bid != 0)
        __hip_atomic_store(&state[(size_t)bid * kCols + threadIdx.x],
                           (unsigned long long)(s_prefix[threadIdx.x] + ScanCols<T>::get(tot, threadIdx.x)) | stamp_bits | (2ull << 62), __ATOMIC_RELAXED,
                           __HIP_MEMORY_SCOPE_AGENT);
    return carry;
}

template <class T, class In, class Out, int kIters>
__global__ __launch_bounds__(kScanBlock) void scan_lookback(In in, Out out, const uint32_t* n_ptr, unsigned long long* state, uint32_t stamp) {
    __shared__ T s_ws[kScanBlock / 64];
    __shared__ uint32_t s_prefix[ScanCols<T>::n];
    const uint32_t n = *n_ptr;
    const uint32_t bid = blockIdx.x;
    const uint32_t base = bid * kScanBlock * kIters;
    if (base >= n) return;
    constexpr uint32_t kRow0 = ScanCols<T>::n == 4 ? 0u : 32768u;
    (void)kRow0;
    KPROF(kRow0 + bid * 4 + (threadIdx.x >> 6), 0);
    T e[kIters], inc[kIters];
#pragma unroll
    for (int it = 0; it < kIters; ++it) {
        const uint32_t j = base + it * kScanBlock + threadIdx.x;
        e[it] = j < n ? in(j, n) : zero_of<T>();
    }
    T tot = zero_of<T>();
#pragma unroll
    for (int it = 0; it < kIters; ++it) {
        T t;
        inc[it] = tot + block_incl_scan(e[it], s_ws, &t);
        tot = tot + t;
    }
    KPROF(kRow0 + bid * 4 + (threadIdx.x >> 6), 1);
    const T carry = lookback_exclusive<T>(tot, state, stamp, bid, s_prefix);
    KPROF(kRow0 + bid * 4 + (threadIdx.x >> 6), 2);
#pragma unroll
    for (int it = 0; it < kIters; ++it) {
        const uint32_t j = base + it * kScanBlock + threadIdx.x;
        if (j < n) out(j, n, carry + inc[it], e[it]);
    }
    KPROF(kRow0 + bid * 4 + (threadIdx.x >> 6), 3);
}

template <class T, int kIters = 1, class In, class Out>
void scan_launch_lb(In in, Out out, const uint32_t* n_ptr, uint32_t n_upper, unsigned long long* state, uint32_t stamp, hipStream_t s) {
    const uint32_t g = scan_grid(n_upper, kIters);
    hipLaunchKernelGGL((scan_lookback<T, In, Out, kIters>), dim3(g), dim3(kScanBlock), 0, s, in, out, n_ptr, state, stamp);
}

}
```

breakdancer_amd/csrc/k3_regions.hip:

```cpp
#include "bdx_k3.h"

#include "bdx_scan.h"

namespace bdx {

struct HeadIn {
    const int32_t* tid;
    const int32_t* pos;
    const uint32_t* meta;
    const Pass1* p1;
    __device__ U4 operator()(uint32_t j, uint32_t) const {
        const int W = p1->window;
        const bool head = j == 0 || tid[j] != tid[j - 1] || pos[j] - pos[j - 1] > W;
        const uint32_t m = meta[j];
        return U4{head ? 1u : 0u, (uint32_t)meta_qlen(m), (uint32_t)meta_rev(m), meta_flag(m) != F_CTX ? 1u : 0u};
    }
};

struct HeadOut {
    K3Arrays a;
    const int32_t* tid;
    int per_tid;
    __device__ void operator()(uint32_t j, uint32_t n, const U4& inc, const U4& e) const {
        const int c = (int)inc.x - 1;
        if (j == n - 1) a.counts->n_cand = inc.x;
        a.cand[j] = c;
        a.pre_q[j] = inc.y;
        a.pre_rev[j] = inc.z;
        a.pre_nonctx[j] = inc.w;
        if (e.x) a.c_first[c] = j;
        const int target = e.x ? c - 1 : c;
        const bool other_chromosome = per_tid && e.x && j > 0 && tid[j] != tid[j - 1];
        const int lane = (int)(threadIdx.x & 63u);
        int v = (target >= 0 && !other_chromosome) ? (int)e.y : INT32_MIN;
#pragma unroll
        for (int o = 1; o < 64; o <<= 1) {
            const int pv = __shfl_up(v, o), pt = __shfl_up(target, o);
            if (lane >= o && pt == target) v = max(v, pv);
        }
        const int nt = __shfl_down(target, 1);
        const bool last_of_run = lane == 63 || j == n - 1 || nt != target;
        if (last_of_run && target >= 0 && v != INT32_MIN) atomicMax(&a.c_maxq[target], v);
    }
};

struct CandStats {
    uint32_t first, last, n, rev, nonctx, nnormal;
    int32_t maxq;
    bool accept;
};

struct CandCtx {
    K3Arrays a;
    Compact cp;
    const Pass1* p1;
    int min_len, seq_coverage_lim;
    const uint32_t* tid_tail;
    __device__ CandStats stats(uint32_t c, uint32_t nc) const {
        CandStats s;
        const uint32_t na = p1->n_anom;
        const uint32_t f = a.c_first[c];
        const uint32_t nxt = c + 1 < nc ? a.c_first[c + 1] : na;
        const uint32_t l = nxt - 1;
        const int start = cp.pos[f], end = cp.pos[l];
        s.first = f; s.last = l; s.n = nxt - f;
        s.rev = a.pre_rev[l] - (f ? a.pre_rev[f - 1] : 0u);
        s.nonctx = a.pre_nonctx[l] - (f ? a.pre_nonctx[f - 1] : 0u);
        const bool chrom_last = tid_tail && (c + 1 == nc || cp.tid[nxt] != cp.tid[f]);
        const uint32_t* tl = chrom_last ? tid_tail + 4 * (size_t)cp.tid[f] : nullptr;
        const uint32_t e = (c + 1 < nc && !chrom_last) ? nxt : l;
        int qsum = (int)(a.pre_q[e] - a.pre_q[f]);
        int maxq = a.c_maxq[c];
        const bool tail_closes = chrom_last && tl[0];
        if (tail_closes) {
            const int tail_qlen = (int)tl[1];
            qsum += tail_qlen;
            maxq = max(maxq, tail_qlen);
        }
        s.maxq = maxq;
        const float cov = __fdiv_rn((float)qsum, (float)(end - start + 1 + maxq));
        s.accept = (end - start > min_len) && (cov < (float)seq_coverage_lim);
        const uint32_t nn_end = chrom_last ? tl[2] : (c + 1 < nc ? cp.nn[nxt] : p1->n_normal);
        s.nnormal = nn_end - cp.nn[f];
        return s;
    }
};

struct AcceptIn {
    CandCtx x;
    __device__ uint32_t operator()(uint32_t c, uint32_t nc) const { return x.stats(c, nc).accept ? 1u : 0u; }
};
struct AcceptOut {
    CandCtx x;
    int nkeys;
    __device__ void operator()(uint32_t c, uint32_t n, uint32_t inc, uint32_t e) const {
        const K3Arrays& a = x.a;
        const Compact& cp = x.cp;
        a.c_rid[c] = e ? (int)inc - 1 : -1;
        if (c != n - 1 && !e) return;
        const CandStats st = x.stats(c, n);
        if (c == n - 1) {
            a.counts->last_maxq = st.maxq; a.counts->n_regions = inc;
            if (a.counts_host) { a.counts_host->last_maxq = st.maxq; a.counts_host->n_regions = inc; a.counts_host->n_cand = n; }
        }
        if (!e) return;
        const uint32_t r = inc - 1;
        const uint32_t f = st.first, l = st.last;
        RegionRec rr;
        rr.tid = cp.tid[f]; rr.start = cp.pos[f]; rr.end = cp.pos[l];
        rr.n = st.n; rr.rev = st.rev; rr.nonctx = st.nonctx; rr.nnormal = st.nnormal;
        rr.maxq = st.maxq;
        rr.first = f;
        const bool to_host = !a.host_copy_later;
        if (to_host) a.r_rec[r] = rr;
        if (a.r_rec_dev) a.r_rec_dev[r] = rr;
        for (int k = 0; k < nkeys; ++k) {
            const uint32_t pf = cp.pk[(size_t)k * cp.cap + f], pl = cp.pk[(size_t)k * cp.cap + l];
            if (to_host) {
                a.r_pk[(size_t)r * 2 * nkeys + k] = pf;
                a.r_pk[(size_t)r * 2 * nkeys + nkeys + k] = pl;
            }
            if (a.r_pk_dev) { a.r_pk_dev[(size_t)r * 2 * nkeys + k] = pf; a.r_pk_dev[(size_t)r * 2 * nkeys + nkeys + k] = pl; }
        }
    }
};


__global__ __launch_bounds__(256) void k3_region_of_kernel(K3Arrays a, const Pass1* p1) {
    const uint32_t j = blockIdx.x * blockDim.x + threadIdx.x;
    if (j < p1->n_anom) {
        a.region_of[j] = a.c_rid[a.cand[j]];
        if (a.out_deg) {
            a.out_deg[j] = 0;
            a.out_deg[(size_t)a.cap + j] = j;
            a.out_deg[2 * (size_t)a.cap + j] = 0;
            a.out_deg[3 * (size_t)a.cap + j] = 0;
            a.out_deg[4 * (size_t)a.cap + j] = 0;
            a.out_deg[5 * (size_t)a.cap + j] = 0;
        }
    }
}

void launch_k3(const K3Arrays& a, const Compact& cp, const Pass1* p1, uint32_t n_anom_host, int min_len, int seq_coverage_lim,
               int nkeys, const uint32_t* tid_tail, bool region_of_launch, hipStream_t s) {
    if (n_anom_host == 0) return;
    const uint32_t* n_ptr = &p1->n_anom;
    HeadIn hin{cp.tid, cp.pos, cp.meta, p1};
    HeadOut hout{a, cp.tid, tid_tail ? 1 : 0};
    const size_t nblk = scan_grid(a.cap, 1);
    if (n_anom_host > (1u << 19)) scan_launch_lb<U4, 2>(hin, hout, n_ptr, n_anom_host, a.lb_state, a.lb_stamp, s);
    else scan_launch_lb<U4, 1>(hin, hout, n_ptr, n_anom_host, a.lb_state, a.lb_stamp, s);
    const CandCtx cx{a, cp, p1, min_len, seq_coverage_lim, tid_tail};
    scan_launch_lb<uint32_t, 1>(AcceptIn{cx}, AcceptOut{cx, nkeys}, &a.counts->n_cand, n_anom_host, a.lb_state + 4 * nblk, a.lb_stamp, s);
    if (region_of_launch) hipLaunchKernelGGL(k3_region_of_kernel, dim3((n_anom_host + 255) / 256), dim3(256), 0, s, a, p1);
}

}

__global__ void k3_noop_kernel() {}
namespace bdx { void warm_k3(hipStream_t s) { hipLaunchKernelGGL(k3_noop_kernel, dim3(1), dim3(64), 0, s); } }

#ifdef BDX_KPROF
extern "C" int bdx_debug_kprof3(unsigned long long* out, size_t n) {
    const int rc = (int)hipMemcpyFromSymbol(out, HIP_SYMBOL(bdx::g_kprof), n * sizeof(unsigned long long));
    void* p = nullptr;
    if (hipGetSymbolAddress(&p, HIP_SYMBOL(bdx::g_kprof)) == hipSuccess) (void)hipMemset(p, 0, sizeof(unsigned long long) * 8 * 65536);
    return rc;
}
#endif
```

breakdancer_amd/csrc/k4_join.hip:

```cpp
#include "bdx_k3.h"
#include "bdx_scan.h"

namespace bdx {

__device__ __forceinline__ uint64_t mix64(uint64_t h) {
    h ^= h >> 33;
    h *= 0xff51afd7ed558ccdull;
    h ^= h >> 33;
    h *= 0xc4ceb9fe1a85ec53ull;
    h ^= h >> 33;
    return h;
}
__device__ __forceinline__ uint32_t bucket_of(uint64_t h, uint32_t log2b) { return log2b ? (uint32_t)(h >> (64 - log2b)) : 0u; }

constexpr int kPartChunk = 512;

__global__ __launch_bounds__(256) void k4_count_kernel(K4Arrays k4, Entries en, const uint32_t* n_ptr) {
    extern __shared__ __attribute__((aligned(16))) unsigned char smem[];
    uint32_t* s_h = (uint32_t*)smem;
    const uint32_t na = *n_ptr;
    const uint32_t base = blockIdx.x * kPartChunk;
    if (base >= na) return;
    for (uint32_t b = threadIdx.x; b < k4.nbuckets; b += 256) s_h[b] = 0;
    __syncthreads();
    for (int it = 0; it < kPartChunk / 256; ++it) {
        const uint32_t j = base + it * 256 + threadIdx.x;
        if (j < na) atomicAdd(&s_h[bucket_of(mix64(en.key[j]), k4.log2b)], 1u);
    }
    __syncthreads();
    for (uint32_t b = threadIdx.x; b < k4.nbuckets; b += 256)
        if (s_h[b]) atomicAdd(&k4.bcnt[b], s_h[b]);
}

__global__ __launch_bounds__(1024) void k4_bucket_scan_kernel(K4Arrays k4, StageCounts* counts) {
    __shared__ uint32_t s_ws[16];
    __shared__ uint32_t s_carry;
    const int lane = threadIdx.x & 63, w = threadIdx.x >> 6;
    if (threadIdx.x == 0) s_carry = 0;
    __syncthreads();
    for (uint32_t base = 0; base < k4.nbuckets; base += 1024) {
        const uint32_t i = base + threadIdx.x;
        const uint32_t v = i < k4.nbuckets ? k4.bcnt[i] : 0u;
        const uint32_t inc = wave_incl_scan(v);
        if (lane == 63) s_ws[w] = inc;
        __syncthreads();
        uint32_t off = s_carry;
        for (int k = 0; k < w; ++k) off += s_ws[k];
        if (i < k4.nbuckets) { k4.boff[i] = off + inc - v; k4.bcur[i] = 0; k4.bcnt[i] = 0; }
        __syncthreads();
        if (threadIdx.x == 1023) s_carry = off + inc;
        __syncthreads();
    }
    if (threadIdx.x == 0) { k4.boff[k4.nbuckets] = s_carry; counts->n_entries = s_carry; }
}

__global__ __launch_bounds__(256) void k4_scatter_kernel(K4Arrays k4, Entries en, const uint32_t* n_ptr) {
    extern __shared__ __attribute__((aligned(16))) unsigned char smem[];
    uint32_t* s_h = (uint32_t*)smem;
    uint32_t* s_base = s_h + k4.nbuckets;
    const uint32_t na = *n_ptr;
    const uint32_t base = blockIdx.x * kPartChunk;
    if (base >= na) return;
    for (uint32_t b = threadIdx.x; b < k4.nbuckets; b += 256) s_h[b] = 0;
    __syncthreads();
    for (int it = 0; it < kPartChunk / 256; ++it) {
        const uint32_t j = base + it * 256 + threadIdx.x;
        if (j < na) atomicAdd(&s_h[bucket_of(mix64(en.key[j]), k4.log2b)], 1u);
    }
    __syncthreads();
    for (uint32_t b = threadIdx.x; b < k4.nbuckets; b += 256) {
        const uint32_t c = s_h[b];
        if (c) s_base[b] = k4.boff[b] + atomicAdd(&k4.bcur[b], c);
        s_h[b] = 0;
    }
    __syncthreads();
    for (int it = 0; it < kPartChunk / 256; ++it) {
        const uint32_t j = base + it * 256 + threadIdx.x;
        if (j < na) {
            const uint64_t key = en.key[j];
            const uint32_t b = bucket_of(mix64(key), k4.log2b);
            const uint32_t slot = s_base[b] + atomicAdd(&s_h[b], 1u);
            k4.e_key[slot] = key;
            k4.e_idx[slot] = j;
        }
    }
}

constexpr uint32_t kMaxProbes = 4096;

template <bool kLds>
__device__ __forceinline__ void join_bucket(uint64_t* tkey, int32_t* tidx, uint32_t cap, const K4Arrays& k4, const int32_t* region,
                                            const uint64_t* check, uint32_t off, uint32_t cnt, StageCounts* counts) {
    for (uint32_t s = threadIdx.x; s < cap; s += blockDim.x) tidx[s] = -1;
    __syncthreads();
    for (uint32_t e = threadIdx.x; e < cnt; e += blockDim.x) {
        const uint64_t key = k4.e_key[off + e];
        const int32_t j = (int32_t)k4.e_idx[off + e];
        uint32_t s = (uint32_t)(mix64(key) & 0xffffffffu) % cap;
        uint32_t probes = 0;
        bool placed = true;
        while (atomicCAS(&tidx[s], -1, j) != -1) {
            s = s + 1 == cap ? 0 : s + 1;
            if (++probes > kMaxProbes) { placed = false; break; }
        }
        if (placed) tkey[s] = key;
        else counts->irregular = 1;
    }
    __syncthreads();
    for (uint32_t e = threadIdx.x; e < cnt; e += blockDim.x) {
        const uint64_t key = k4.e_key[off + e];
        const int32_t j = (int32_t)k4.e_idx[off + e];
        uint32_t s = (uint32_t)(mix64(key) & 0xffffffffu) % cap;
        int32_t mate = -1;
        const uint32_t lim = cap < kMaxProbes ? cap : kMaxProbes;
        for (uint32_t probes = 0; probes < lim; ++probes) {
            const int32_t o = tidx[s];
            if (o == -1) break;
            if (o != j && tkey[s] == key && (!check || check[o] == check[j])) {
                if (mate != -1) counts->irregular = 1;
                mate = o;
            }
            s = s + 1 == cap ? 0 : s + 1;
        }
        if (mate >= 0 && (region[j] < 0 || region[mate] < 0)) mate = -2;
        k4.partner[j] = mate;
    }
}

__global__ __launch_bounds__(256) void k4_join_kernel(K4Arrays k4, const int32_t* region, const uint64_t* check, StageCounts* counts) {
    extern __shared__ __attribute__((aligned(16))) unsigned char smem[];
    const uint32_t b = blockIdx.x;
    const uint32_t off = k4.boff[b], cnt = k4.boff[b + 1] - off;
    if (cnt == 0) return;
    if (2 * cnt <= (uint32_t)kJoinLdsSlots) {
        uint64_t* tkey = (uint64_t*)smem;
        int32_t* tidx = (int32_t*)(tkey + kJoinLdsSlots);
        join_bucket<true>(tkey, tidx, 2 * cnt, k4, region, check, off, cnt, counts);
    } else {
        join_bucket<false>(k4.t_key + 2 * (size_t)off, k4.t_idx + 2 * (size_t)off, 2 * cnt, k4, region, check, off, cnt, counts);
    }
}

constexpr uint32_t kJoinForwardBlocks = 32;
__global__ __launch_bounds__(256) void k4_direct_join_kernel(K4Arrays k4, Entries en, const uint32_t* n_ptr, StageCounts* counts) {
    const uint32_t na = *n_ptr;
    const uint32_t fwd = en.r_rec_host ? kJoinForwardBlocks : 0u;
    if (blockIdx.x < fwd) {
        const uint32_t nr = en.counts->n_regions;
        const uint32_t t = blockIdx.x * 256 + threadIdx.x, gsz = fwd * 256;
        constexpr uint32_t kw = sizeof(RegionRec) / 4;
        {
            const uint32_t words = nr * kw, quads = words / 4;
            const uint4* src = (const uint4*)en.r_rec_dev;
            uint4* dst = (uint4*)en.r_rec_host;
            for (uint32_t i = t; i < quads; i += gsz) dst[i] = src[i];
            if (t < words - quads * 4) ((uint32_t*)en.r_rec_host)[quads * 4 + t] = ((const uint32_t*)en.r_rec_dev)[quads * 4 + t];
        }
        {
            const uint32_t words = nr * (uint32_t)en.nkeys2, quads = words / 4;
            const uint4* src = (const uint4*)en.r_pk_dev;
            uint4* dst = (uint4*)en.r_pk_host;
            for (uint32_t i = t; i < quads; i += gsz) dst[i] = src[i];
            if (t < words - quads * 4) en.r_pk_host[quads * 4 + t] = en.r_pk_dev[quads * 4 + t];
        }
    }
    const uint32_t j = blockIdx.x < fwd ? 0xFFFFFFFFu : (blockIdx.x - fwd) * 256 + threadIdx.x;
    const uint32_t kp = (blockIdx.x - fwd) * 4 + (threadIdx.x >> 6);
    (void)kp;
    KPROF(kp, 0);
    KPROF(kp, 1);
    if (j >= na) return;
    const uint32_t nl = en.n_local ? *en.n_local : na;
    const bool jf = j >= nl;
    int rj;
    if (jf) {
        rj = en.fregion[j - nl];
    } else if (en.c_rid) {
        rj = en.c_rid[en.cand[j]];
        en.region_out[j] = rj;
        if (en.k6_scratch) {
            const size_t cap = en.scratch_cap;
            en.k6_scratch[j] = 0; en.k6_scratch[cap + j] = j; en.k6_scratch[2 * cap + j] = 0; en.k6_scratch[3 * cap + j] = 0;
            en.k6_scratch[4 * cap + j] = 0; en.k6_scratch[5 * cap + j] = 0;
        }
    } else {
        rj = en.region[j];
    }
    const uint64_t key = jf ? en.fkey[j - nl] : en.key[j];
    const uint64_t chk = en.check ? (jf ? en.fcheck[j - nl] : en.check[j]) : 0ull;
    const uint64_t h = mix64(key);
    if (key != 0x5555AAAA5555AAAAull) KPROF(kp, 2);
    const uint32_t tag = (uint32_t)(h >> 32);
    unsigned long long* table = (unsigned long long*)k4.t_key;
    const unsigned long long mine = ((unsigned long long)tag << 32) | j;
    uint32_t s = (uint32_t)h & k4.t_mask;
    for (uint32_t probes = 0; probes <= kMaxProbes; ++probes) {
        const unsigned long long old = atomicCAS(&table[s], ~0ull, mine);
        if (probes == 0 && old != 0x5555AAAA5555AAAAull) KPROF(kp, 3);
        if (old == ~0ull) return;
        if ((uint32_t)(old >> 32) == tag) {
            const uint32_t o = (uint32_t)old;
            const bool of = o >= nl;
            const uint64_t okey = of ? en.fkey[o - nl] : en.key[o];
            if (okey == key && (!en.check || (of ? en.fcheck[o - nl] : en.check[o]) == chk)) {
                const int ro = of ? en.fregion[o - nl] : (en.c_rid ? en.c_rid[en.cand[o]] : en.region[o]);
                const bool alive = rj >= 0 && ro >= 0;
                if (!jf) k4.partner[j] = alive ? (int32_t)o : -2;
                if (!of && atomicExch(&k4.partner[o], alive ? (int32_t)j : -2) != -1) counts->irregular = 1;
                if (alive && k4.pair_lo) {
                    if (jf != of) {
                        if (jf) k4.pair_lo[o] = rj; else k4.pair_lo[j] = ro;
                    } else if (!jf) {
                        if (o < j) k4.pair_lo[j] = ro;
                        else k4.pair_lo[o] = rj;
                    }
                }
                KPROF(kp, 4);
                return;
            }
        }
        s = (s + 1) & k4.t_mask;
    }
    counts->irregular = 1;
}

void launch_k4_join_only(const K4Arrays& k4, const Entries& en, const uint32_t* n_ptr, uint32_t n_anom_host, StageCounts* counts,
                         hipStream_t s) {
    if (n_anom_host == 0) return;
    const uint32_t g = (n_anom_host + kPartChunk - 1) / kPartChunk;
    if (k4.direct) {
        const uint32_t gd = (n_anom_host + 255) / 256 + (en.r_rec_host ? kJoinForwardBlocks : 0u);
        hipLaunchKernelGGL(k4_direct_join_kernel, dim3(gd), dim3(256), 0, s, k4, en, n_ptr, counts);
        return;
    }
    hipLaunchKernelGGL(k4_count_kernel, dim3(g), dim3(256), (size_t)k4.nbuckets * 4, s, k4, en, n_ptr);
    hipLaunchKernelGGL(k4_bucket_scan_kernel, dim3(1), dim3(1024), 0, s, k4, counts);
    hipLaunchKernelGGL(k4_scatter_kernel, dim3(g), dim3(256), (size_t)k4.nbuckets * 8, s, k4, en, n_ptr);
    static bool attr_set = false;
    if (!attr_set) {
        (void)hipFuncSetAttribute((const void*)k4_join_kernel, hipFuncAttributeMaxDynamicSharedMemorySize, kJoinLdsSlots * 12);
        attr_set = true;
    }
    hipLaunchKernelGGL(k4_join_kernel, dim3(k4.nbuckets), dim3(256), (size_t)kJoinLdsSlots * 12, s, k4, en.region, en.check, counts);
}

}

__global__ void k4_noop_kernel() {}
namespace bdx { void warm_k4(hipStream_t s) { hipLaunchKernelGGL(k4_noop_kernel, dim3(1), dim3(64), 0, s); } }

#ifdef BDX_KPROF
extern "C" int bdx_debug_kprof4(unsigned long long* out, size_t n) {
    const int rc = (int)hipMemcpyFromSymbol(out, HIP_SYMBOL(bdx::g_kprof), n * sizeof(unsigned long long));
    void* p = nullptr;
    if (hipGetSymbolAddress(&p, HIP_SYMBOL(bdx::g_kprof)) == hipSuccess) (void)hipMemset(p, 0, sizeof(unsigned long long) * 8 * 65536);
    return rc;
}
#endif
```

breakdancer_amd/csrc/k6_assemble.hip:

```cpp
#include <algorithm>
#include <cstdint>

#include "bdx_k3.h"

#include "bdx_poisson.h"
#include "bdx_scan.h"

namespace bdx {

namespace {

__device__ __forceinline__ uint64_t readlane64(uint64_t v, int l) {
    const uint32_t lo = (uint32_t)__builtin_amdgcn_readlane((int)(uint32_t)v, l);
    const uint32_t hi = (uint32_t)__builtin_amdgcn_readlane((int)(uint32_t)(v >> 32), l);
    return ((uint64_t)hi << 32) | lo;
}

__device__ __forceinline__ uint32_t wave_sum_u32(uint32_t v) {
#pragma unroll
    for (int o = 32; o > 0; o >>= 1) v += __shfl_xor(v, o);
    return v;
}

__device__ __forceinline__ uint32_t wave_reserve(uint32_t need, uint32_t* counter) {
    const uint32_t inc = wave_incl_scan(need);
    const uint32_t tot = (uint32_t)__shfl((int)inc, 63);
    uint32_t base = 0;
    if ((threadIdx.x & 63) == 63 && tot) base = atomicAdd(counter, tot);
    base = (uint32_t)__shfl((int)base, 63);
    return base + inc - need;
}

struct GrpRange {
    uint32_t beg, cnt;
};

__device__ __forceinline__ bool region_stored(const RegionRec& R, const K6Arrays& a) {
    const int valid = a.chr_restricted ? (int)R.nonctx : (int)R.n;
    return valid >= a.min_read_pair;
}

}

struct Merged {
    uint32_t cnt, sum;
    uint32_t gw;
    uint32_t rank, gparts;
    uint32_t total, wself;
    uint64_t lmask;
    bool leader, gleader;
};

template <bool kWeighted>
__device__ __forceinline__ Merged merge_items(uint64_t key, uint32_t wc, uint32_t ws, bool has, uint32_t r, int lane) {
    Merged m{};
    const uint64_t hasmask = __ballot(has);
    uint32_t eq_before = 0;
    for (uint64_t mm = hasmask; mm; mm &= mm - 1) {
        const int t = __builtin_ctzll(mm);
        const uint64_t kt = readlane64(key, t);
        const uint32_t st = (uint32_t)__builtin_amdgcn_readlane((int)ws, t);
        const uint32_t ct = kWeighted ? (uint32_t)__builtin_amdgcn_readlane((int)wc, t) : 1u;
        const bool eq = kt == key;
        m.cnt += eq ? ct : 0u;
        m.sum += eq ? st : 0u;
        eq_before += (eq && t < lane) ? 1u : 0u;
        m.gw += ((kt >> 12) == (key >> 12)) ? ct : 0u;
        if (kWeighted) {
            m.total += ct;
            m.wself += (uint32_t)(kt >> 12) == r ? ct : 0u;
        }
    }
    if (!kWeighted) {
        m.total = (uint32_t)__popcll(hasmask);
        m.wself = (uint32_t)__popcll(__ballot(has && (uint32_t)(key >> 12) == r));
    }
    m.leader = has && eq_before == 0;
    m.lmask = __ballot(m.leader);
    bool lo_first = true;
    for (uint64_t mm = m.lmask; mm; mm &= mm - 1) {
        const int t = __builtin_ctzll(mm);
        const uint64_t kt = readlane64(key, t);
        const bool same_lo = (kt >> 12) == (key >> 12);
        m.gparts += same_lo ? 1u : 0u;
        if (kt < key) {
            ++m.rank;
            if (same_lo) lo_first = false;
        }
    }
    m.gleader = m.leader && lo_first;
    return m;
}

__global__ __launch_bounds__(256) void k6_pairs_kernel(K6Arrays a) {
    __shared__ PartRec s_stash[4][64];
    const int lane = threadIdx.x & 63, w = threadIdx.x >> 6;
    const uint32_t nwaves = gridDim.x * 4;
    if (a.flag_regions && blockIdx.x == 0 && threadIdx.x == 0) {
        __threadfence_system();
        *(volatile uint32_t*)a.flag_regions = a.flag_value;
    }
    if (blockIdx.x == 0 && a.emit_part) a.emit_part[threadIdx.x] = 0;
    const uint32_t NR = a.counts->n_regions;
    const uint32_t mrp = (uint32_t)max(a.min_read_pair, 0);
    for (uint32_t r = blockIdx.x * 4 + (threadIdx.x >> 6); r < NR; r += nwaves) {
        const RegionRec rr = a.r_rec[r];
        const uint32_t first = a.first_of ? a.first_of[r] : rr.first, n = rr.n;
        RegSum rs{};
        auto load_read = [&](uint32_t c0, uint64_t& key, uint32_t& is) -> bool {
            const uint32_t i = c0 + lane;
            key = ~0ull;
            is = 0;
            if (i >= n) return false;
            const uint32_t j = first + i;
            int32_t plo;
            if (a.pair_lo) {
                plo = a.pair_lo[j];
            } else {
                const int32_t p = a.partner[j];
                plo = (p >= 0 && (uint32_t)p < j) ? a.region_of[p] : -1;
            }
            if (plo < 0) return false;
            const uint32_t m = a.meta[j];
            key = ((uint64_t)(uint32_t)plo << 12) | ((uint64_t)meta_lib(m) << 4) | (uint64_t)meta_flag(m);
            is = (uint32_t)a.isize[j];
            return true;
        };
        uint64_t key = ~0ull;
        uint32_t is = 0;
        bool has = false, merged = false;
        Merged m{};
        if (a.in_groups) {
            const uint32_t g0 = a.in_goff[r], ng = a.in_goff[r + 1] - g0;
            auto load_group = [&](uint32_t c0, uint64_t& k, uint32_t& cnt, uint32_t& sm) -> bool {
                const uint32_t i = c0 + lane;
                k = ~0ull; cnt = 0; sm = 0;
                if (i >= ng) return false;
                const GroupRec g = a.in_groups[g0 + i];
                k = ((g.key >> 38) << 12) | (g.key & 0xFFFull);
                cnt = g.pairs; sm = g.sum_isize;
                return true;
            };
            if (ng <= 64) {
                uint32_t cnt;
                has = load_group(0, key, cnt, is);
                if (__ballot(has)) {
                    m = merge_items<true>(key, cnt, is, has, r, lane);
                    merged = true;
                }
            } else {
                rs.big = 1u;
                for (uint32_t c0 = 0; c0 < ng; c0 += 64) {
                    uint64_t ck;
                    uint32_t cc, ci;
                    const bool ch = load_group(c0, ck, cc, ci);
                    const Merged cm = merge_items<true>(ck, cc, ci, ch, r, lane);
                    const uint32_t clo = (uint32_t)(ck >> 12);
                    rs.n_pairs += cm.total;
                    rs.w_self += cm.wself;
                    if (cm.gleader && clo < r) {
                        atomicAdd(&a.out_deg[clo], 1u);
                        a.bad_v[clo] = 1u;
                        if (a.taint && a.r_rec[clo].n == 0) { a.taint[clo] = 1; a.taint[r] = 1; }
                    }
                    if (lane == 0) a.bad_v[r] = 1u;
                    const uint32_t nl = (uint32_t)__popcll(cm.lmask);
                    uint32_t base = 0;
                    if (lane == 0) base = atomicAdd(&a.counts->n_groups, nl);
                    base = (uint32_t)__builtin_amdgcn_readfirstlane((int)base);
                    if (cm.leader) {
                        const uint32_t o = base + cm.rank;
                        if (o < a.g_cap) {
                            GroupRec g;
                            g.key = group_pack(clo, r, (uint32_t)((ck >> 4) & 255), (uint32_t)(ck & 15));
                            g.pairs = cm.cnt;
                            g.sum_isize = cm.sum;
                            a.g_rec[o] = g;
                        } else {
                            a.counts->overflow = 1;
                        }
                    }
                }
            }
        } else if (n <= 64) {
            has = load_read(0, key, is);
            if (__ballot(has)) {
                m = merge_items<false>(key, 1u, is, has, r, lane);
                merged = true;
            }
        } else {
            uint32_t np = 0;
            bool fits = true;
            for (uint32_t c0 = 0; c0 < n && fits; c0 += 64) {
                uint64_t ck;
                uint32_t ci;
                const bool ch = load_read(c0, ck, ci);
                if (!__ballot(ch)) continue;
                const Merged cm = merge_items<false>(ck, 1u, ci, ch, r, lane);
                const uint32_t nl = (uint32_t)__popcll(cm.lmask);
                if (np + nl > 64u) { fits = false; break; }
                if (cm.leader) s_stash[w][np + cm.rank] = PartRec{ck, cm.cnt, cm.sum};
                np += nl;
            }
            __builtin_amdgcn_wave_barrier();
            if (fits) {
                if (np) {
                    has = (uint32_t)lane < np;
                    const PartRec q = has ? s_stash[w][lane] : PartRec{~0ull, 0u, 0u};
                    key = q.key;
                    m = merge_items<true>(key, q.pairs, q.sum, has, r, lane);
                    merged = true;
                }
            } else {
                rs.big = 1u;
                for (uint32_t c0 = 0; c0 < n; c0 += 64) {
                    uint64_t ck;
                    uint32_t ci;
                    const bool ch = load_read(c0, ck, ci);
                    if (!__ballot(ch)) continue;
                    const Merged cm = merge_items<false>(ck, 1u, ci, ch, r, lane);
                    const uint32_t clo = (uint32_t)(ck >> 12);
                    rs.n_pairs += cm.total;
                    rs.w_self += cm.wself;
                    if (cm.gleader && clo < r) {
                        atomicAdd(&a.out_deg[clo], 1u);
                        a.bad_v[clo] = 1u;
                        if (a.taint && a.r_rec[clo].n == 0) { a.taint[clo] = 1; a.taint[r] = 1; }
                    }
                    if (lane == 0) a.bad_v[r] = 1u;
                    const uint32_t nl = (uint32_t)__popcll(cm.lmask);
                    uint32_t base = 0;
                    if (lane == 0) base = atomicAdd(&a.counts->n_groups, nl);
                    base = (uint32_t)__builtin_amdgcn_readfirstlane((int)base);
                    if (cm.leader) {
                        const uint32_t o = base + cm.rank;
                        if (o < a.g_cap) {
                            GroupRec g;
                            g.key = group_pack(clo, r, (uint32_t)((ck >> 4) & 255), (uint32_t)(ck & 15));
                            g.pairs = cm.cnt;
                            g.sum_isize = cm.sum;
                            a.g_rec[o] = g;
                        } else {
                            a.counts->overflow = 1;
                        }
                    }
                }
            }
            __builtin_amdgcn_wave_barrier();
        }
        if (merged) {
            const uint32_t lo = (uint32_t)(key >> 12);
            rs.n_pairs = m.total;
            rs.w_self = m.wself;
            const bool strong = m.gw >= mrp;
            const bool in_edge = m.gleader && lo < r && strong;
            const uint64_t gl_in = __ballot(in_edge);
            if (in_edge) atomicAdd(&a.out_deg[lo], 1u);
            if (a.taint && in_edge && a.r_rec[lo].n == 0) { a.taint[lo] = 1; a.taint[r] = 1; }
            rs.np_all = (uint32_t)__popcll(m.lmask);
            rs.np_self = (uint32_t)__popcll(__ballot(m.leader && lo == r));
            rs.np_emit = (uint32_t)__popcll(__ballot(m.leader && (lo == r || strong)));
            rs.n_weak = (uint32_t)__popcll(__ballot(m.gleader && lo < r && !strong));
            rs.n_in = (uint32_t)__popcll(gl_in);
            if (rs.n_in > (uint32_t)kK6MaxIn) {
                if (in_edge) a.bad_v[lo] = 1u;
                if (lane == 0) a.bad_v[r] = 1u;
            } else {
                if (in_edge && !a.force_host) {
                    const uint32_t lr = a.label[r], ll = a.label[lo];
                    if (lr < ll) atomicMin(&a.label[lo], lr);
                    else if (ll < lr) atomicMin(&a.label[r], ll);
                }
                uint64_t mm = gl_in;
#pragma unroll
                for (int e = 0; e < kK6MaxIn; ++e) {
                    if (mm) {
                        const int t = __builtin_ctzll(mm);
                        mm &= mm - 1;
                        rs.e_lo[e] = (uint32_t)__builtin_amdgcn_readlane((int)lo, t);
                        rs.e_w[e] = (uint32_t)__builtin_amdgcn_readlane((int)m.gw, t);
                        rs.e_off[e] = (uint32_t)__builtin_amdgcn_readlane((int)m.rank, t);
                        rs.e_cnt[e] = (uint32_t)__builtin_amdgcn_readlane((int)m.gparts, t);
                    }
                }
            }
            if (m.leader) a.parts[first + m.rank] = PartRec{(lo < r && !strong) ? (key | kWeakPart) : key, m.cnt, m.sum};
        }
        if (lane == 0) a.rs[r] = rs;
    }
}

__global__ __launch_bounds__(256) void k6_label_kernel(K6Arrays a) {
    const uint32_t r = blockIdx.x * blockDim.x + threadIdx.x;
    if (r >= a.counts->n_regions) return;
    const RegSum* s = &a.rs[r];
    const uint32_t n_in = s->n_in;
    if (s->big || n_in == 0 || n_in > (uint32_t)kK6MaxIn) return;
    for (uint32_t e = 0; e < n_in; ++e) {
        const uint32_t lo = s->e_lo[e];
        const uint32_t lr = a.label[r], ll = a.label[lo];
        if (lr < ll) atomicMin(&a.label[lo], lr);
        else if (ll < lr) atomicMin(&a.label[r], ll);
    }
    const uint32_t l = a.label[r], l2 = a.label[l];
    if (l2 < l) atomicMin(&a.label[r], l2);
}

__global__ __launch_bounds__(256) void k6_classify_kernel(K6Arrays a) {
    const uint32_t r = blockIdx.x * blockDim.x + threadIdx.x;
    if (r >= a.counts->n_regions) return;
    const RegSum* s = &a.rs[r];
    const uint32_t n_in = s->n_in;
    const bool hub = s->big || n_in > (uint32_t)kK6MaxIn;
    if (!hub && n_in == 0 && a.out_deg[r] == 0 && s->np_self == 0) return;
    const uint32_t L = a.label[r];
    if (hub || a.bad_v[r] || (a.taint && a.taint[r])) a.bad[L] = 1u;
    if (!hub) {
#pragma unroll
        for (uint32_t e = 0; e < (uint32_t)kK6MaxIn; ++e) {
            if (e < n_in) {
                const uint32_t ll = a.label[s->e_lo[e]];
                if (ll != L) { a.bad[L] = 1u; a.bad[ll] = 1u; }
            }
        }
    }
    const uint32_t slot = atomicAdd(&a.mcount[L], 1u);
    if (a.big_walk && slot < (uint32_t)kK6BigMembers) a.member_ids[(size_t)L * kK6BigMembers + slot] = r;
    if (slot < (uint32_t)kK6MaxMembers) {
        static_assert(sizeof(MemberInfo) == 7 * 16 && sizeof(RegionRec) == 36 && offsetof(MemberInfo, rec) == 4 && offsetof(MemberInfo, np_all) == 40 &&
                          offsetof(MemberInfo, e_lo) == 56 && offsetof(MemberInfo, stored) == 104, "a member's record is seven 16-byte words");
        const uint32_t* rw = (const uint32_t*)&a.r_rec[r];
        const uint32_t r0 = rw[0], r1 = rw[1], r2 = rw[2], r3 = rw[3], r4 = rw[4], r5 = rw[5], r6 = rw[6], r7 = rw[7], r8 = a.first_of ? a.first_of[r] : rw[8];
        const uint32_t stored = (int)(a.chr_restricted ? r5 : r3) >= a.min_read_pair ? 1u : 0u;
        uint4* dst = (uint4*)&a.members[(size_t)L * kK6MaxMembers + slot];
        dst[0] = make_uint4(r, r0, r1, r2);
        dst[1] = make_uint4(r3, r4, r5, r6);
        dst[2] = make_uint4(r7, r8, s->np_all, s->np_self);
        dst[3] = make_uint4(s->w_self, hub ? 0u : n_in, s->e_lo[0], s->e_lo[1]);
        dst[4] = make_uint4(s->e_lo[2], s->e_w[0], s->e_w[1], s->e_w[2]);
        dst[5] = make_uint4(s->e_off[0], s->e_off[1], s->e_off[2], s->e_cnt[0]);
        dst[6] = make_uint4(s->e_cnt[1], s->e_cnt[2], stored, 0u);
    }
    if (s->np_emit) atomicAdd(&a.pcount[L], s->np_emit);
}

namespace {

struct RunConst {
    const float* lib_mean;
    const uint32_t* hist;
    const float* key_density;
    uint32_t covered;
};

constexpr int kFewLibs = 4;
__device__ bool assemble_sv(const K6Arrays& a, const RunConst& rc_, const PartRec* P, uint32_t A, int32_t B, const RegionRec& ra, const RegionRec& rb,
                            const uint32_t* pk_last_a, const uint32_t* pk_first_b, const GrpRange (&gs)[3], int max_readlen,
                            uint32_t slot, uint32_t start, bool store, uint32_t* nacc_out, uint32_t* ncn_out, uint32_t kprow = ~0u) {
    (void)kprow;
    KPROF(kprow, 0);
    const uint32_t lib_room = a.lib_stride;
    const int mrp = a.min_read_pair;
    int cv[kNumFlags];
#pragma unroll
    for (int f = 0; f < kNumFlags; ++f) cv[f] = 0;
    int num_pairs = 0;
    const PartRec none_part{0ull, 0u, 0u};
#pragma unroll
    for (int g = 0; g < 3; ++g)
        for (uint32_t i = 0; i < gs[g].cnt; i += 4) {
            PartRec q[4];
#pragma unroll
            for (int u = 0; u < 4; ++u) q[u] = i + u < gs[g].cnt ? P[gs[g].beg + i + u] : none_part;
#pragma unroll
            for (int u = 0; u < 4; ++u) {
                const int f = (int)(q[u].key & 15);
                const int pr = (int)q[u].pairs;
#pragma unroll
                for (int ff = 0; ff < kNumFlags; ++ff) cv[ff] += f == ff ? pr : 0;
                num_pairs += pr;
            }
        }
    if (num_pairs != 0x7FFFFFFF) KPROF(kprow, 1);
    if (num_pairs < mrp) return false;
    int flag = BDX_NA, flag_count;
    {
        int best = 0, bestv = cv[0];
#pragma unroll
        for (int f = 1; f < kNumFlags; ++f)
            if (cv[f] > bestv) { best = f; bestv = cv[f]; }
        if (bestv > 0) flag = best;
        flag_count = bestv > 0 ? bestv : cv[BDX_NA];
    }
    if (flag_count < mrp) return false;

    int chr[2], pos[2], fwd[2], rev[2];
    chr[0] = ra.tid; pos[0] = ra.start; pos[1] = ra.end;
    fwd[0] = (int)(ra.n - ra.rev); rev[0] = (int)ra.rev;
    int total_region_size = ra.end - ra.start + 1;
    if (B >= 0) {
        fwd[1] = (int)(rb.n - rb.rev); rev[1] = (int)rb.rev;
        if (flag == BDX_ARP_RF) pos[1] = rb.end + max_readlen - 5;
        else if (flag == BDX_ARP_FF) { pos[0] = pos[1]; pos[1] = rb.end + max_readlen - 5; }
        else if (flag == BDX_ARP_RR) pos[1] = rb.start;
        else { pos[0] = pos[1]; pos[1] = rb.start; }
        chr[1] = rb.tid;
        total_region_size += rb.end - rb.start + 1;
    } else {
        fwd[1] = fwd[0]; rev[1] = rev[0]; chr[1] = ra.tid; pos[1] = ra.end;
    }

    LibStage* ls = a.lib_stage + (size_t)slot * a.lib_stride;
    uint32_t nacc = 0;
    float diff = 0.0f;
    if (a.nlibs >= 2 && a.nlibs <= kFewLibs && !a.asm_plain) {
        int rcL[kFewLibs], spL[kFewLibs];
#pragma unroll
        for (int l = 0; l < kFewLibs; ++l) { rcL[l] = 0; spL[l] = 0; }
#pragma unroll
        for (int g = 0; g < 3; ++g)
            for (uint32_t i = 0; i < gs[g].cnt; i += 4) {
                PartRec q[4];
#pragma unroll
                for (int u = 0; u < 4; ++u) q[u] = i + u < gs[g].cnt ? P[gs[g].beg + i + u] : none_part;
#pragma unroll
                for (int u = 0; u < 4; ++u) {
                    const bool mine = (int)(q[u].key & 15) == flag;
                    const int lib = (int)((q[u].key >> 4) & 255);
#pragma unroll
                    for (int l = 0; l < kFewLibs; ++l) {
                        rcL[l] += (mine && lib == l) ? (int)q[u].pairs : 0;
                        spL[l] += (mine && lib == l) ? (int)q[u].sum : 0;
                    }
                }
            }
#pragma unroll
        for (int l = 0; l < kFewLibs; ++l) {
            if (rcL[l] == 0) continue;
            diff = __fadd_rn(diff, __fsub_rn((float)spL[l], __fmul_rn((float)rcL[l], rc_.lib_mean[l])));
            const uint32_t nflag = rc_.hist[(size_t)l * kNumFlags + flag];
            double lambda = __dmul_rn((double)total_region_size, __ddiv_rn((double)nflag, (double)rc_.covered));
            lambda = (1.0e-10 < lambda) ? lambda : 1.0e-10;
            if (store && nacc < lib_room) ls[nacc] = LibStage{l, rcL[l], lambda};
            ++nacc;
        }
    } else {
    uint32_t idx[3] = {0, 0, 0};
#pragma unroll
    for (int g = 0; g < 3; ++g)
        while (idx[g] < gs[g].cnt && (int)(P[gs[g].beg + idx[g]].key & 15) != flag) ++idx[g];
    while (true) {
        int best = 256;
#pragma unroll
        for (int g = 0; g < 3; ++g)
            if (idx[g] < gs[g].cnt) best = min(best, (int)((P[gs[g].beg + idx[g]].key >> 4) & 255));
        if (best == 256) break;
        int rc = 0, span = 0;
#pragma unroll
        for (int g = 0; g < 3; ++g)
            if (idx[g] < gs[g].cnt && (int)((P[gs[g].beg + idx[g]].key >> 4) & 255) == best) {
                rc += (int)P[gs[g].beg + idx[g]].pairs;
// ... 973 lines not shown
    }
}

__global__ __launch_bounds__(kScanBlock) void k6_score_kernel(K6Arrays a, double ln10, int score_threshold, int with_scores) {
    __shared__ uint32_t s_rec[kScanBlock / 64][64 * kSvWords];
    __shared__ uint32_t s_fromw[kScanBlock / 64][64];
    __shared__ uint32_t s_printed;
    const uint32_t tid = threadIdx.x;
    const int lane = tid & 63, w = tid >> 6;
    const uint32_t bid = blockIdx.x;
    const uint32_t kp = 32768u + 16384u + (bid * 4 + w < 16384u ? bid * 4 + w : 16383u);
    (void)kp;
    KPROF(kp, 0);
    if (tid == 0) s_printed = 0;
    __syncthreads();
    const uint32_t n_sv = a.counts->overflow ? 0u : a.counts->n_sv_dev;
    for (uint32_t c0 = (bid * (kScanBlock / 64) + (uint32_t)w) * 64u; c0 < n_sv; c0 += gridDim.x * kScanBlock) {
        const uint32_t cnt = min(64u, n_sv - c0);
        const bool act = (uint32_t)lane < cnt;
        uint32_t* rec = s_rec[w];
        const uint32_t from = act ? a.sv_src[c0 + lane] : 0u;
        const uint2 bg = act ? a.sv_begin[c0 + lane] : make_uint2(0u, 0u);
        s_fromw[w][lane] = from;
        __builtin_amdgcn_wave_barrier();
        for (uint32_t i = lane; i < cnt * kSvWords; i += 64) {
            const uint32_t sv = i / kSvWords, wd = i - sv * kSvWords;
            const uint32_t f = s_fromw[w][sv];
            const uint32_t* src = (f & 0x80000000u) ? (const uint32_t*)(a.hs_rec + (f & 0x7FFFFFFFu)) : (const uint32_t*)(a.sv_stage + f);
            rec[i] = src[wd];
        }
        __builtin_amdgcn_wave_barrier();
        KPROF(kp, 3);
        SvOut* o = (SvOut*)rec + (act ? lane : 0);
        const bool hosted = (from & 0x80000000u) != 0;
        const int32_t nl = act ? o->sv.lib_count : 0, ncn = act ? o->sv.cn_count : 0;
        const int32_t l0 = o->sv.lib_begin, k0 = o->sv.cn_begin;
        if (act) { o->sv.lib_begin = (int32_t)bg.x; o->sv.cn_begin = (int32_t)bg.y; }
        int32_t max_nl = nl, max_ncn = ncn;
#pragma unroll
        for (int off = 32; off > 0; off >>= 1) { max_nl = max(max_nl, __shfl_xor(max_nl, off)); max_ncn = max(max_ncn, __shfl_xor(max_ncn, off)); }
        double logp = 0.0, err = 0.0;
        for (int32_t q = 0; q < max_nl; ++q) {
            const bool a2 = q < nl;
            double lam = 1.0;
            int32_t k = 0, li = 0;
            if (a2) {
                if (hosted) { lam = a.hs_lambda[l0 + q]; k = a.hs_lib_pairs[l0 + q]; li = a.hs_lib_index[l0 + q]; }
                else { const LibStage t = a.lib_stage[(size_t)from * a.lib_stride + q]; lam = t.lambda; k = t.rc; li = t.lib; }
            }
            const double lt = poisson_term(lam, k, a2, lane);
            if (a2) {
                a.lib_index[bg.x + q] = li;
                a.lib_pairs[bg.x + q] = k;
                if (a.ltail_host) a.ltail_host[bg.x + q] = lt;
                const double tmp_a = __dsub_rn(lt, err);
                const double tmp_b = __dadd_rn(logp, tmp_a);
                err = __dsub_rn(__dsub_rn(tmp_b, logp), tmp_a);
                logp = tmp_b;
            }
        }
        for (int32_t t = 0; t < max_ncn; ++t) {
            if (t < ncn) {
                int32_t key;
                float value;
                if (hosted) { key = a.hs_cn_key[k0 + t]; value = a.hs_cn_value[k0 + t]; }
                else { const CnStage cn = a.cn_stage[(size_t)from * a.nkeys + t]; key = cn.key; value = cn.value; }
                a.cn_key[bg.y + t] = key;
                a.cn_value[bg.y + t] = value;
            }
        }
        bool pr = false;
        if (act && with_scores) {
            const double phred_tmp = __ddiv_rn(__dmul_rn(-10.0, logp), ln10);
            const double r = __dadd_rn(phred_tmp, 0.5);
            int phred;
            if (phred_tmp > 99.0) phred = 99;
            else if (r != r || r >= 2147483648.0 || r <= -2147483649.0) phred = INT32_MIN;
            else phred = (int)r;
            pr = phred > score_threshold;
            o->sv.logp = logp;
            o->sv.score = phred;
            o->sv.printed = pr ? 1 : 0;
        }
        if (a.sv_key && act) {
            const unsigned long long T = a.sv_vx[c0 + lane], st = o->start;
            a.sv_key[c0 + lane] = (T << kKeyShiftT) | (T == st ? 1ull << 33 : 0ull) | (st << kKeyShiftStart);
        }
        const uint32_t npr = (uint32_t)__popcll(__ballot(pr));
        if (lane == 0 && npr) atomicAdd(&s_printed, npr);
        KPROF(kp, 4);
        __builtin_amdgcn_wave_barrier();
        if (a.wire_rows) {
            SvWire wr{};
            if (act) {
                wr.pos[0] = o->sv.pos[0]; wr.pos[1] = o->sv.pos[1]; wr.region[0] = o->sv.region[0]; wr.region[1] = o->sv.region[1];
                wr.size = o->sv.size; wr.score = o->sv.score; wr.num_reads = o->sv.num_reads; wr.allele_frequency = o->sv.allele_frequency;
                wr.logp = o->sv.logp; wr.start = o->start;
                wr.bits = ((uint32_t)o->sv.lib_count & 255u) | (((uint32_t)o->sv.cn_count & 255u) << 8) | (((uint32_t)o->sv.flag & 15u) << 16) |
                          ((o->grp_mask & 7u) << 20) | ((o->sv.printed ? 1u : 0u) << 23);
            }
            __builtin_amdgcn_wave_barrier();
            if (act) {
                uint32_t* q = rec + lane * kWireWords;
                const uint32_t* src = (const uint32_t*)&wr;
#pragma unroll
                for (int k = 0; k < kWireWords; ++k) q[k] = src[k];
            }
            __builtin_amdgcn_wave_barrier();
            uint32_t* dst = (uint32_t*)a.sv_out + (size_t)c0 * kWireWords;
            for (uint32_t i = lane; i < cnt * kWireWords; i += 64) dst[i] = rec[i];
        } else {
            uint32_t* dst = (uint32_t*)(a.sv_out + c0);
            for (uint32_t i = lane; i < cnt * kSvWords; i += 64) dst[i] = rec[i];
        }
        __builtin_amdgcn_wave_barrier();
    }
    __syncthreads();
    if (tid == 0) {
        if (s_printed) atomicAdd(&a.counts->n_printed, s_printed);
        if (a.printed_host) a.printed_host[bid] = s_printed;
    }
    KPROF(kp, 5);
}

__global__ __launch_bounds__(64) void k6_done_kernel(K6Arrays a) {
    if (threadIdx.x == 0) {
        if (a.counts_host2) a.counts_host2->n_printed = a.counts->n_printed;
        if (a.flag_done) {
            __threadfence_system();
            *(volatile uint32_t*)a.flag_done = a.flag_value;
        }
    }
}

__global__ __launch_bounds__(256) void k6_scratch_init_kernel(uint32_t* out_deg, uint32_t cap) {
    for (uint32_t j = blockIdx.x * 256 + threadIdx.x; j < cap; j += gridDim.x * 256) {
        out_deg[j] = 0;
        out_deg[(size_t)cap + j] = j;
        out_deg[2 * (size_t)cap + j] = 0;
        out_deg[3 * (size_t)cap + j] = 0;
        out_deg[4 * (size_t)cap + j] = 0;
        out_deg[5 * (size_t)cap + j] = 0;
    }
}

void launch_k6_scratch_init(uint32_t* out_deg, uint32_t cap, hipStream_t s) {
    if (!cap) return;
    hipLaunchKernelGGL(k6_scratch_init_kernel, dim3(std::min<uint32_t>((cap + 255) / 256, 4096u)), dim3(256), 0, s, out_deg, cap);
}

void launch_k6_pairs(const K6Arrays& a, uint32_t n_anom_host, hipStream_t s) {
    if (n_anom_host == 0) return;
    const uint32_t gp = std::min<uint32_t>((n_anom_host / 8 + 3) / 4 + 1, 16384u);
    hipLaunchKernelGGL(k6_pairs_kernel, dim3(gp), dim3(256), 0, s, a);
}

void launch_k6_components(const K6Arrays& a, uint32_t n_anom_host, hipStream_t s) {
    if (n_anom_host == 0) return;
    constexpr uint32_t kRegionThreads = 64;
    const uint32_t grs = (n_anom_host + kRegionThreads - 1) / kRegionThreads;
    if (!a.force_host)
        for (int i = 1; i < a.propagation_rounds; ++i) hipLaunchKernelGGL(k6_label_kernel, dim3(grs), dim3(kRegionThreads), 0, s, a);
    hipLaunchKernelGGL(k6_classify_kernel, dim3(grs), dim3(kRegionThreads), 0, s, a);
    hipLaunchKernelGGL(k6_emit_kernel, dim3(grs), dim3(kRegionThreads), 0, s, a);
    if (a.counts_host && !a.mirror_in_walk) hipLaunchKernelGGL(k6_mirror_kernel, dim3(1), dim3(64), 0, s, a);
}

void launch_k6_groups(const K6Arrays& a, uint32_t n_anom_host, hipStream_t s) {
    launch_k6_pairs(a, n_anom_host, s);
    launch_k6_components(a, n_anom_host, s);
}

void launch_k6_walk(const K6Arrays& a, uint32_t n_anom_host, hipStream_t s) {
    if (n_anom_host == 0 || a.force_host) return;
    const uint32_t gp = std::min<uint32_t>((n_anom_host / 8 + 3) / 4 + 1, 16384u);
    hipLaunchKernelGGL(k6_walk_kernel, dim3(std::min<uint32_t>(n_anom_host / WalkTab::kStride / 4 + 1, 8192u)), dim3(64), 0, s, a);
    if (a.big_walk) hipLaunchKernelGGL(k6_walk_big_kernel, dim3(gp / 8 + 1), dim3(256), 0, s, a);
    if (a.rank_part) hipLaunchKernelGGL(k6_ranksort_kernel, dim3(kRankGrid), dim3(kScanBlock), 0, s, a);
}

uint32_t k6_score_grid(const K6Arrays& a) { return std::max(1u, std::min(1024u, (a.sv_cap + kScanBlock - 1) / kScanBlock)); }

void launch_k6_table(const K6Arrays& a, uint32_t n_anom_host, double ln10, int score_threshold, int with_scores, hipStream_t s) {
    if (n_anom_host) {
        hipLaunchKernelGGL(k6_insert_kernel, dim3(1), dim3(kInsThreads), 0, s, a);
        hipLaunchKernelGGL(k6_place_kernel, dim3(scan_grid(a.fin_regions ? a.fin_regions : a.cap, 1)), dim3(kScanBlock), 0, s, a);
        hipLaunchKernelGGL(k6_score_kernel, dim3(k6_score_grid(a)), dim3(kScanBlock), 0, s, a, ln10, score_threshold, with_scores);
    }
    if (!a.printed_host || a.flag_done) hipLaunchKernelGGL(k6_done_kernel, dim3(1), dim3(64), 0, s, a);
}

}

__global__ void k6_noop_kernel() {}
namespace bdx { void warm_k6(hipStream_t s) { hipLaunchKernelGGL(k6_noop_kernel, dim3(1), dim3(64), 0, s); } }

#ifdef BDX_KPROF
extern "C" int bdx_debug_kprof(unsigned long long* out, size_t n) {
    const int rc = (int)hipMemcpyFromSymbol(out, HIP_SYMBOL(bdx::g_kprof), n * sizeof(unsigned long long));
    void* p = nullptr;
    if (hipGetSymbolAddress(&p, HIP_SYMBOL(bdx::g_kprof)) == hipSuccess) (void)hipMemset(p, 0, sizeof(unsigned long long) * 8 * 65536);
    return rc;
}
#endif
```

Before: 29.01 billion.

## Fuse mate join into cut kernel and region-of writes into k6 pairs

When the direct join path is active with fused region_of, the mate-pair hash join now launches alongside the k3 cut scan through a new combined cut-join kernel, replacing the separate do_join_local pass. The k6 pairs kernel gains a template variant that writes region_out itself and takes partner regions from c_rid[cand[p]]. Extra blocks in that launch forward region records and keys to the host buffers, and the readiness flag moves to the label and classify kernels. This removes separate kernel launches and passes over the anomalous reads. In exchange it adds ordering dependencies between the kernels and a new -1 guard in the host fallback.

```diff
diff --git a/breakdancer_amd/csrc/bdx_api.hip b/breakdancer_amd/csrc/bdx_api.hip
--- a/breakdancer_amd/csrc/bdx_api.hip
+++ b/breakdancer_amd/csrc/bdx_api.hip
@@ -257,6 +257,7 @@
     int nkeys = 0, nlibs = 0;
     bool use_check = false;
     bool k2_clears_join = false;
+    bool k2_pair_lo = false;
     RegionDst regions = RegionDst::HostAndHbm;
     bool groups_in_hbm = false, table_in_hbm = false;
     uint32_t k6_cap = 0;
@@ -273,6 +274,7 @@
     StageDims d;
     d.na = na; d.nkeys = c->nkeys; d.nlibs = c->nlibs; d.use_check = c->use_check;
     d.k2_clears_join = c->force_direct_join || (!c->bucketed_join && na <= kDirectJoinMax);
+    d.k2_pair_lo = c->force_direct_join;
     d.groups_in_hbm = c->groups_in_hbm; d.table_in_hbm = c->table_in_hbm; d.k6_cap = c->k6_cap;
     d.big_walk = c->big_walk_mode >= 0 ? c->big_walk_mode : (c->last_big_groups >= 0 ? (c->last_big_groups > 2000 ? 1 : 0) : -1);
     d.join_n = d.join_own = na; d.join_slots = d.k2_clears_join ? direct_join_slots(na) : 0;
@@ -902,7 +904,8 @@
     SZCHK(size_c_maxq(b, cap));
     if (d.k2_clears_join) {
         SZCHK(b.b_t_key.ensure((size_t)direct_join_slots(d.na) * 8));
-        SZCHK(size_join_words(b, cap, true));
+        SZCHK(size_join_words(b, cap, d.k2_pair_lo));
+        if (!d.k2_pair_lo) SZCHK(b.b_region_of.ensure(cap * 4));
     }
     return BDX_OK;
 }
@@ -1012,7 +1015,7 @@
             const uint32_t slots = dm.join_slots;
             k2.fill_ptr[1] = b.b_t_key.as<uint32_t>(); k2.fill_words[1] = 2 * slots; k2.fill_value[1] = 0xFFFFFFFFu;
             k2.fill_ptr[2] = b.b_partner.as<uint32_t>(); k2.fill_words[2] = na; k2.fill_value[2] = 0xFFFFFFFFu;
-            k2.fill_ptr[3] = b.b_pair_lo.as<uint32_t>(); k2.fill_words[3] = na; k2.fill_value[3] = 0xFFFFFFFFu;
+            k2.fill_ptr[3] = dm.k2_pair_lo ? b.b_pair_lo.as<uint32_t>() : b.b_region_of.as<uint32_t>(); k2.fill_words[3] = na; k2.fill_value[3] = 0xFFFFFFFFu;
             c->join_table_clean = slots;
         }
         {
@@ -1047,6 +1050,37 @@
     if (pk) keep_pk.assign(pk, pk + n * 2 * (size_t)c->nkeys);
     c->regions.swap(keep); c->r_pk.swap(keep_pk);
     c->reg = c->regions.data(); c->rpk = c->r_pk.data();
+}
+
+int prepare_join(bdx_ctx* c, uint32_t n, const uint32_t* n_local, bool want_pair_lo, bool* direct) {
+    hipStream_t s = c->stream;
+    K4Arrays& k4 = c->k4;
+    k4 = K4Arrays{};
+    *direct = c->force_direct_join || (!c->bucketed_join && n <= kDirectJoinMax);
+    if (!n) return BDX_OK;
+    StageDims dm = stage_dims(c, c->na_alloc);
+    dm.join_n = n;
+    dm.join_own = n_local ? std::min<uint32_t>(n, std::max<uint32_t>(c->na_alloc, 1u)) : n;
+    dm.join_slots = !*direct ? 0u : (c->join_table_clean && (uint64_t)n * 2 <= c->join_table_clean) ? c->join_table_clean : direct_join_slots(n);
+    dm.join_pair_lo = want_pair_lo;
+    BDX_TRY(size_join(c->sb, dm, &c->err));
+    StageBufs& b = c->sb;
+    k4.g_cap = dm.join_groups();
+    k4.g_rec = c->groups_in_hbm ? b.b_groups.as<GroupRec>() : b.h_groups.as<GroupRec>();
+    k4.partner = b.b_partner.as<int32_t>();
+    if (!*direct) return BDX_OK;
+    const uint32_t slots = dm.join_slots;
+    const size_t n_own = dm.join_own;
+    if (c->join_table_clean != slots) {
+        HIPCHK(c, hipMemsetAsync(b.b_t_key.p, 0xFF, (size_t)slots * 8, s));
+        HIPCHK(c, hipMemsetAsync(b.b_partner.p, 0xFF, n_own * 4, s));
+        if (want_pair_lo) HIPCHK(c, hipMemsetAsync(b.b_pair_lo.p, 0xFF, n_own * 4, s));
+    }
+    k4.pair_lo = want_pair_lo ? b.b_pair_lo.as<int32_t>() : nullptr;
+    c->join_table_clean = 0;
+    k4.direct = 1; k4.t_mask = slots - 1;
+    k4.t_key = b.b_t_key.as<uint64_t>(); k4.t_idx = b.b_t_idx.as<int32_t>();
+    return BDX_OK;
 }
 
 int do_cut(bdx_ctx* c, const uint32_t* tid_tail, RegionDst dst) {
@@ -1078,7 +1112,17 @@
         HIPCHK(c, next_lb_stamp(c, &k3.lb_stamp));
         k3.counts = c->b_counts.as<StageCounts>();
         c->region_of_fused = for_k6 && !c->bucketed_join && na <= kDirectJoinMax;
-        launch_k3(k3, c->cp, c->b_p1.as<Pass1>(), na, c->opts.min_len, c->opts.seq_coverage_lim, c->nkeys, tid_tail, !c->region_of_fused, s);
+        MateJoin mj{};
+        if (c->region_of_fused) {
+            if (!c->join_table_clean) HIPCHK(c, hipMemsetAsync(b.b_region_of.p, 0xFF, (size_t)na * 4, s));
+            bool direct = false;
+            BDX_TRY(prepare_join(c, na, nullptr, false, &direct));
+            mj.key = c->cp.key; mj.check = c->cp.check; mj.partner = c->k4.partner;
+            mj.table = (unsigned long long*)c->k4.t_key; mj.t_mask = c->k4.t_mask;
+            mj.k6_scratch = k3.out_deg; mj.scratch_cap = k3.cap;
+            mj.counts = k3.counts;
+        }
+        launch_k3(k3, c->cp, c->b_p1.as<Pass1>(), na, c->opts.min_len, c->opts.seq_coverage_lim, c->nkeys, tid_tail, c->region_of_fused ? &mj : nullptr, s);
         if (for_k6 && !k3.host_copy_later) {
             BDX_TRY(signal_ready(c, 3, c->ev_regions));
         }
@@ -1089,33 +1133,12 @@
 
 int do_join_local(bdx_ctx* c, uint32_t n, const Entries& en, const uint32_t* n_ptr) {
     hipStream_t s = c->stream;
+    bool direct = false;
+    BDX_TRY(prepare_join(c, n, en.n_local, en.want_pair_lo != 0, &direct));
+    if (!n) return BDX_OK;
     K4Arrays& k4 = c->k4;
-    k4 = K4Arrays{};
-    if (!n) return BDX_OK;
-    const bool direct = c->force_direct_join || (!c->bucketed_join && n <= kDirectJoinMax);
-    StageDims dm = stage_dims(c, c->na_alloc);
-    dm.join_n = n;
-    dm.join_own = en.n_local ? std::min<uint32_t>(n, std::max<uint32_t>(c->na_alloc, 1u)) : n;
-    dm.join_slots = !direct ? 0u : (c->join_table_clean && (uint64_t)n * 2 <= c->join_table_clean) ? c->join_table_clean : direct_join_slots(n);
-    dm.join_pair_lo = en.want_pair_lo != 0;
-    BDX_TRY(size_join(c->sb, dm, &c->err));
     StageBufs& b = c->sb;
-    k4.g_cap = dm.join_groups();
-    k4.g_rec = c->groups_in_hbm ? b.b_groups.as<GroupRec>() : b.h_groups.as<GroupRec>();
-    k4.partner = b.b_partner.as<int32_t>();
     if (direct) {
-        const uint32_t slots = dm.join_slots;
-        const size_t n_own = dm.join_own;
-        const bool want_lo = en.c_rid || en.want_pair_lo;
-        if (c->join_table_clean != slots) {
-            HIPCHK(c, hipMemsetAsync(b.b_t_key.p, 0xFF, (size_t)slots * 8, s));
-            HIPCHK(c, hipMemsetAsync(b.b_partner.p, 0xFF, n_own * 4, s));
-            if (en.want_pair_lo) HIPCHK(c, hipMemsetAsync(b.b_pair_lo.p, 0xFF, n_own * 4, s));
-        }
-        k4.pair_lo = ((c->join_table_clean == slots && want_lo) || en.want_pair_lo) ? b.b_pair_lo.as<int32_t>() : nullptr;
-        c->join_table_clean = 0;
-        k4.direct = 1; k4.t_mask = slots - 1;
-        k4.t_key = b.b_t_key.as<uint64_t>(); k4.t_idx = b.b_t_idx.as<int32_t>();
         launch_k4_join_only(k4, en, n_ptr, n, c->b_counts.as<StageCounts>(), s);
         return BDX_OK;
     }
@@ -1185,6 +1208,10 @@
     a.r_rec = c->k6_r_rec ? c->k6_r_rec : b.b_r_rec.as<RegionRec>(); a.r_pk = c->k6_r_pk ? c->k6_r_pk : b.b_r_pk.as<uint32_t>();
     a.taint = c->k6_taint;
     a.region_of = c->k3.region_of; a.partner = c->k4.partner; a.pair_lo = c->k4.pair_lo; a.meta = c->cp.meta; a.isize = c->cp.isize;
+    if (c->region_of_fused) {
+        a.cand = c->k3.cand; a.c_rid = c->k3.c_rid; a.region_out = c->k3.region_of;
+        if (c->k3.host_copy_later) { a.fwd_rec = c->k3.r_rec; a.fwd_pk = c->k3.r_pk; }
+    }
     a.in_groups = c->k6_in_groups; a.in_goff = c->k6_in_goff; a.first_of = c->k6_in_groups ? c->k6_in_goff : nullptr;
     a.parts = b.b_parts.as<PartRec>();
     a.rs = b.b_rs.as<RegSum>();
@@ -1459,6 +1486,7 @@
             for (uint32_t j = f; j < f + n; ++j) {
                 const int32_t p = partner[j];
                 if (p < 0 || (uint32_t)p >= j) continue;
+                if (region_of[p] < 0) continue;
                 if ((uint32_t)(region_of[p] + (int32_t)ph) != lo) continue;
                 pairs.emplace_back(j, (uint32_t)p);
             }
@@ -1549,22 +1577,16 @@
         BDX_TRY(do_compact(c));
         BDX_TRY(do_cut(c, nullptr, RegionDst::HostAndHbm));
         if (!c->na_alloc) return BDX_OK;
-        Entries en{};
-        en.key = c->cp.key; en.check = c->cp.check; en.region = c->k3.region_of; en.meta = c->cp.meta; en.isize = c->cp.isize;
-        if (c->region_of_fused) {
-            en.cand = c->k3.cand; en.c_rid = c->k3.c_rid; en.region_out = c->k3.region_of;
-            en.k6_scratch = c->k3.out_deg; en.scratch_cap = c->k3.cap;
-            if (c->k3.host_copy_later) {
-                en.r_rec_dev = c->k3.r_rec_dev; en.r_pk_dev = c->k3.r_pk_dev; en.r_rec_host = c->k3.r_rec; en.r_pk_host = c->k3.r_pk;
-                en.counts = c->b_counts.as<StageCounts>(); en.nkeys2 = 2 * c->nkeys;
-            }
-        }
-        BDX_TRY(do_join_local(c, c->na_alloc, en, &c->b_p1.as<Pass1>()->n_anom));
-        if (c->k3.host_copy_later && !c->poll) {
-            BDX_TRY(signal_ready(c, 3, c->ev_regions));
+        if (!c->region_of_fused) {
+            Entries en{};
+            en.key = c->cp.key; en.check = c->cp.check; en.region = c->k3.region_of; en.meta = c->cp.meta; en.isize = c->cp.isize;
+            BDX_TRY(do_join_local(c, c->na_alloc, en, &c->b_p1.as<Pass1>()->n_anom));
         }
         BDX_TRY(k6_prepare(c, force_host, 0));
-        return k6_then_walk(c, launch_k6_groups);
+        if (!c->k3.host_copy_later || c->poll) return k6_then_walk(c, launch_k6_groups);
+        k6_pairs(c);
+        BDX_TRY(signal_ready(c, 3, c->ev_regions));
+        return k6_then_walk(c, launch_k6_components);
     };
     uint32_t guess = 0;
     const bool restored = !c->ov_cnt.empty();
diff --git a/breakdancer_amd/csrc/bdx_cut.h b/breakdancer_amd/csrc/bdx_cut.h
--- /dev/null
+++ b/breakdancer_amd/csrc/bdx_cut.h
@@ -0,0 +1,50 @@
+#pragma once
+#include "bdx_k3.h"
+#include "bdx_scan.h"
+
+namespace bdx {
+
+struct HeadIn {
+    const int32_t* tid;
+    const int32_t* pos;
+    const uint32_t* meta;
+    const Pass1* p1;
+    __device__ U4 operator()(uint32_t j, uint32_t) const {
+        const int W = p1->window;
+        const bool head = j == 0 || tid[j] != tid[j - 1] || pos[j] - pos[j - 1] > W;
+        const uint32_t m = meta[j];
+        return U4{head ? 1u : 0u, (uint32_t)meta_qlen(m), (uint32_t)meta_rev(m), meta_flag(m) != F_CTX ? 1u : 0u};
+    }
+};
+
+struct HeadOut {
+    K3Arrays a;
+    const int32_t* tid;
+    int per_tid;
+    __device__ void operator()(uint32_t j, uint32_t n, const U4& inc, const U4& e) const {
+        const int c = (int)inc.x - 1;
+        if (j == n - 1) a.counts->n_cand = inc.x;
+        a.cand[j] = c;
+        a.pre_q[j] = inc.y;
+        a.pre_rev[j] = inc.z;
+        a.pre_nonctx[j] = inc.w;
+        if (e.x) a.c_first[c] = j;
+        const int target = e.x ? c - 1 : c;
+        const bool other_chromosome = per_tid && e.x && j > 0 && tid[j] != tid[j - 1];
+        const int lane = (int)(threadIdx.x & 63u);
+        int v = (target >= 0 && !other_chromosome) ? (int)e.y : INT32_MIN;
+#pragma unroll
+        for (int o = 1; o < 64; o <<= 1) {
+            const int pv = __shfl_up(v, o), pt = __shfl_up(target, o);
+            if (lane >= o && pt == target) v = max(v, pv);
+        }
+        const int nt = __shfl_down(target, 1);
+        const bool last_of_run = lane == 63 || j == n - 1 || nt != target;
+        if (last_of_run && target >= 0 && v != INT32_MIN) atomicMax(&a.c_maxq[target], v);
+    }
+};
+
+void launch_k4_cut_join(const HeadIn& hin, const HeadOut& hout, const uint32_t* n_ptr, uint32_t n_upper, int iters, unsigned long long* lb_state,
+                        uint32_t lb_stamp, const MateJoin& mj, hipStream_t s);
+
+}
diff --git a/breakdancer_amd/csrc/bdx_k3.h b/breakdancer_amd/csrc/bdx_k3.h
--- a/breakdancer_amd/csrc/bdx_k3.h
+++ b/breakdancer_amd/csrc/bdx_k3.h
@@ -64,12 +64,14 @@
     StageCounts* counts_host;
 };
 
+struct MateJoin;
 void launch_k3(const K3Arrays& a, const Compact& cp, const Pass1* p1, uint32_t n_anom_host, int min_len, int seq_coverage_lim,
-               int nkeys, const uint32_t* tid_tail, bool region_of_launch, hipStream_t s);
+               int nkeys, const uint32_t* tid_tail, const MateJoin* beside, hipStream_t s);
 
 constexpr int kMaxBuckets = 8192;
 constexpr int kJoinLdsSlots = 8192;
 constexpr uint32_t kDirectJoinMax = 1u << 22;
+constexpr uint32_t kJoinForwardBlocks = 32;
 inline uint32_t direct_join_slots(uint32_t n) {
     uint32_t slots = 1024;
     while (slots < 4 * (uint64_t)n) slots <<= 1;
@@ -106,22 +108,22 @@
     const int32_t* region;
     const uint32_t* meta;
     const int32_t* isize;
-    const int32_t* cand;
-    const int32_t* c_rid;
-    int32_t* region_out;
-    const RegionRec* r_rec_dev;
-    const uint32_t* r_pk_dev;
-    RegionRec* r_rec_host;
-    uint32_t* r_pk_host;
-    const StageCounts* counts;
-    int nkeys2;
-    uint32_t* k6_scratch;
-    uint32_t scratch_cap;
     const uint32_t* n_local;
     const uint64_t* fkey;
     const uint64_t* fcheck;
     const int32_t* fregion;
     int want_pair_lo;
+};
+
+struct MateJoin {
+    const uint64_t* key;
+    const uint64_t* check;
+    int32_t* partner;
+    unsigned long long* table;
+    uint32_t t_mask;
+    uint32_t* k6_scratch;
+    uint32_t scratch_cap;
+    StageCounts* counts;
 };
 
 void launch_k4_join_only(const K4Arrays& k4, const Entries& e, const uint32_t* n_ptr, uint32_t n_upper, StageCounts* counts, hipStream_t s);
@@ -217,6 +219,11 @@
     const int32_t* region_of;
     const int32_t* partner;
     const int32_t* pair_lo;
+    const int32_t* cand;
+    const int32_t* c_rid;
+    int32_t* region_out;
+    RegionRec* fwd_rec;
+    uint32_t* fwd_pk;
     const uint32_t* meta;
     const int32_t* isize;
     const GroupRec* in_groups;
diff --git a/breakdancer_amd/csrc/bdx_scan.h b/breakdancer_amd/csrc/bdx_scan.h
--- a/breakdancer_amd/csrc/bdx_scan.h
+++ b/breakdancer_amd/csrc/bdx_scan.h
@@ -218,7 +218,7 @@
 }
 
 template <class T, class In, class Out, int kIters>
-__global__ __launch_bounds__(kScanBlock) void scan_lookback(In in, Out out, const uint32_t* n_ptr, unsigned long long* state, uint32_t stamp) {
+__device__ __forceinline__ void scan_lookback_body(const In& in, const Out& out, const uint32_t* n_ptr, unsigned long long* state, uint32_t stamp) {
     __shared__ T s_ws[kScanBlock / 64];
     __shared__ uint32_t s_prefix[ScanCols<T>::n];
     const uint32_t n = *n_ptr;
@@ -252,6 +252,11 @@
     KPROF(kRow0 + bid * 4 + (threadIdx.x >> 6), 3);
 }
 
+template <class T, class In, class Out, int kIters>
+__global__ __launch_bounds__(kScanBlock) void scan_lookback(In in, Out out, const uint32_t* n_ptr, unsigned long long* state, uint32_t stamp) {
+    scan_lookback_body<T, In, Out, kIters>(in, out, n_ptr, state, stamp);
+}
+
 template <class T, int kIters = 1, class In, class Out>
 void scan_launch_lb(In in, Out out, const uint32_t* n_ptr, uint32_t n_upper, unsigned long long* state, uint32_t stamp, hipStream_t s) {
     const uint32_t g = scan_grid(n_upper, kIters);
diff --git a/breakdancer_amd/csrc/k3_regions.hip b/breakdancer_amd/csrc/k3_regions.hip
--- a/breakdancer_amd/csrc/k3_regions.hip
+++ b/breakdancer_amd/csrc/k3_regions.hip
@@ -1,48 +1,9 @@
 #include "bdx_k3.h"
 
+#include "bdx_cut.h"
 #include "bdx_scan.h"
 
 namespace bdx {
-
-struct HeadIn {
-    const int32_t* tid;
-    const int32_t* pos;
-    const uint32_t* meta;
-    const Pass1* p1;
-    __device__ U4 operator()(uint32_t j, uint32_t) const {
-        const int W = p1->window;
-        const bool head = j == 0 || tid[j] != tid[j - 1] || pos[j] - pos[j - 1] > W;
-        const uint32_t m = meta[j];
-        return U4{head ? 1u : 0u, (uint32_t)meta_qlen(m), (uint32_t)meta_rev(m), meta_flag(m) != F_CTX ? 1u : 0u};
-    }
-};
-
-struct HeadOut {
-    K3Arrays a;
-    const int32_t* tid;
-    int per_tid;
-    __device__ void operator()(uint32_t j, uint32_t n, const U4& inc, const U4& e) const {
-        const int c = (int)inc.x - 1;
-        if (j == n - 1) a.counts->n_cand = inc.x;
-        a.cand[j] = c;
-        a.pre_q[j] = inc.y;
-        a.pre_rev[j] = inc.z;
-        a.pre_nonctx[j] = inc.w;
-        if (e.x) a.c_first[c] = j;
-        const int target = e.x ? c - 1 : c;
-        const bool other_chromosome = per_tid && e.x && j > 0 && tid[j] != tid[j - 1];
-        const int lane = (int)(threadIdx.x & 63u);
-        int v = (target >= 0 && !other_chromosome) ? (int)e.y : INT32_MIN;
-#pragma unroll
-        for (int o = 1; o < 64; o <<= 1) {
-            const int pv = __shfl_up(v, o), pt = __shfl_up(target, o);
-            if (lane >= o && pt == target) v = max(v, pv);
-        }
-        const int nt = __shfl_down(target, 1);
-        const bool last_of_run = lane == 63 || j == n - 1 || nt != target;
-        if (last_of_run && target >= 0 && v != INT32_MIN) atomicMax(&a.c_maxq[target], v);
-    }
-};
 
 struct CandStats {
     uint32_t first, last, n, rev, nonctx, nnormal;
@@ -142,17 +103,19 @@
 }
 
 void launch_k3(const K3Arrays& a, const Compact& cp, const Pass1* p1, uint32_t n_anom_host, int min_len, int seq_coverage_lim,
-               int nkeys, const uint32_t* tid_tail, bool region_of_launch, hipStream_t s) {
+               int nkeys, const uint32_t* tid_tail, const MateJoin* beside, hipStream_t s) {
     if (n_anom_host == 0) return;
     const uint32_t* n_ptr = &p1->n_anom;
     HeadIn hin{cp.tid, cp.pos, cp.meta, p1};
     HeadOut hout{a, cp.tid, tid_tail ? 1 : 0};
     const size_t nblk = scan_grid(a.cap, 1);
-    if (n_anom_host > (1u << 19)) scan_launch_lb<U4, 2>(hin, hout, n_ptr, n_anom_host, a.lb_state, a.lb_stamp, s);
+    const bool two = n_anom_host > (1u << 19);
+    if (beside) launch_k4_cut_join(hin, hout, n_ptr, n_anom_host, two ? 2 : 1, a.lb_state, a.lb_stamp, *beside, s);
+    else if (two) scan_launch_lb<U4, 2>(hin, hout, n_ptr, n_anom_host, a.lb_state, a.lb_stamp, s);
     else scan_launch_lb<U4, 1>(hin, hout, n_ptr, n_anom_host, a.lb_state, a.lb_stamp, s);
     const CandCtx cx{a, cp, p1, min_len, seq_coverage_lim, tid_tail};
     scan_launch_lb<uint32_t, 1>(AcceptIn{cx}, AcceptOut{cx, nkeys}, &a.counts->n_cand, n_anom_host, a.lb_state + 4 * nblk, a.lb_stamp, s);
-    if (region_of_launch) hipLaunchKernelGGL(k3_region_of_kernel, dim3((n_anom_host + 255) / 256), dim3(256), 0, s, a, p1);
+    if (!beside) hipLaunchKernelGGL(k3_region_of_kernel, dim3((n_anom_host + 255) / 256), dim3(256), 0, s, a, p1);
 }
 
 }
diff --git a/breakdancer_amd/csrc/k4_join.hip b/breakdancer_amd/csrc/k4_join.hip
--- a/breakdancer_amd/csrc/k4_join.hip
+++ b/breakdancer_amd/csrc/k4_join.hip
@@ -1,4 +1,5 @@
 #include "bdx_k3.h"
+#include "bdx_cut.h"
 #include "bdx_scan.h"
 
 namespace bdx {
@@ -141,51 +142,17 @@
     }
 }
 
-constexpr uint32_t kJoinForwardBlocks = 32;
 __global__ __launch_bounds__(256) void k4_direct_join_kernel(K4Arrays k4, Entries en, const uint32_t* n_ptr, StageCounts* counts) {
     const uint32_t na = *n_ptr;
-    const uint32_t fwd = en.r_rec_host ? kJoinForwardBlocks : 0u;
-    if (blockIdx.x < fwd) {
-        const uint32_t nr = en.counts->n_regions;
-        const uint32_t t = blockIdx.x * 256 + threadIdx.x, gsz = fwd * 256;
-        constexpr uint32_t kw = sizeof(RegionRec) / 4;
-        {
-            const uint32_t words = nr * kw, quads = words / 4;
-            const uint4* src = (const uint4*)en.r_rec_dev;
-            uint4* dst = (uint4*)en.r_rec_host;
-            for (uint32_t i = t; i < quads; i += gsz) dst[i] = src[i];
-            if (t < words - quads * 4) ((uint32_t*)en.r_rec_host)[quads * 4 + t] = ((const uint32_t*)en.r_rec_dev)[quads * 4 + t];
-        }
-        {
-            const uint32_t words = nr * (uint32_t)en.nkeys2, quads = words / 4;
-            const uint4* src = (const uint4*)en.r_pk_dev;
-            uint4* dst = (uint4*)en.r_pk_host;
-            for (uint32_t i = t; i < quads; i += gsz) dst[i] = src[i];
-            if (t < words - quads * 4) en.r_pk_host[quads * 4 + t] = en.r_pk_dev[quads * 4 + t];
-        }
-    }
-    const uint32_t j = blockIdx.x < fwd ? 0xFFFFFFFFu : (blockIdx.x - fwd) * 256 + threadIdx.x;
-    const uint32_t kp = (blockIdx.x - fwd) * 4 + (threadIdx.x >> 6);
+    const uint32_t j = blockIdx.x * 256 + threadIdx.x;
+    const uint32_t kp = blockIdx.x * 4 + (threadIdx.x >> 6);
     (void)kp;
     KPROF(kp, 0);
     KPROF(kp, 1);
     if (j >= na) return;
     const uint32_t nl = en.n_local ? *en.n_local : na;
     const bool jf = j >= nl;
-    int rj;
-    if (jf) {
-        rj = en.fregion[j - nl];
-    } else if (en.c_rid) {
-        rj = en.c_rid[en.cand[j]];
-        en.region_out[j] = rj;
-        if (en.k6_scratch) {
-            const size_t cap = en.scratch_cap;
-            en.k6_scratch[j] = 0; en.k6_scratch[cap + j] = j; en.k6_scratch[2 * cap + j] = 0; en.k6_scratch[3 * cap + j] = 0;
-            en.k6_scratch[4 * cap + j] = 0; en.k6_scratch[5 * cap + j] = 0;
-        }
-    } else {
-        rj = en.region[j];
-    }
+    const int rj = jf ? en.fregion[j - nl] : en.region[j];
     const uint64_t key = jf ? en.fkey[j - nl] : en.key[j];
     const uint64_t chk = en.check ? (jf ? en.fcheck[j - nl] : en.check[j]) : 0ull;
     const uint64_t h = mix64(key);
@@ -203,7 +170,7 @@
             const bool of = o >= nl;
             const uint64_t okey = of ? en.fkey[o - nl] : en.key[o];
             if (okey == key && (!en.check || (of ? en.fcheck[o - nl] : en.check[o]) == chk)) {
-                const int ro = of ? en.fregion[o - nl] : (en.c_rid ? en.c_rid[en.cand[o]] : en.region[o]);
+                const int ro = of ? en.fregion[o - nl] : en.region[o];
                 const bool alive = rj >= 0 && ro >= 0;
                 if (!jf) k4.partner[j] = alive ? (int32_t)o : -2;
                 if (!of && atomicExch(&k4.partner[o], alive ? (int32_t)j : -2) != -1) counts->irregular = 1;
@@ -224,12 +191,63 @@
     counts->irregular = 1;
 }
 
+__device__ __forceinline__ void mate_join_body(const MateJoin& mj, const uint32_t* n_ptr, uint32_t wg) {
+    const uint32_t j = wg * 256 + threadIdx.x;
+    const uint32_t kp = 32768u + wg * 4 + (threadIdx.x >> 6);
+    (void)kp;
+    KPROF(kp, 0);
+    if (j >= *n_ptr) return;
+    if (mj.k6_scratch) {
+        const size_t cap = mj.scratch_cap;
+        mj.k6_scratch[j] = 0; mj.k6_scratch[cap + j] = j; mj.k6_scratch[2 * cap + j] = 0; mj.k6_scratch[3 * cap + j] = 0;
+        mj.k6_scratch[4 * cap + j] = 0; mj.k6_scratch[5 * cap + j] = 0;
+    }
+    const uint64_t key = mj.key[j];
+    const uint64_t chk = mj.check ? mj.check[j] : 0ull;
+    const uint64_t h = mix64(key);
+    if (key != 0x5555AAAA5555AAAAull) KPROF(kp, 2);
+    const uint32_t tag = (uint32_t)(h >> 32);
+    const unsigned long long mine = ((unsigned long long)tag << 32) | j;
+    uint32_t s = (uint32_t)h & mj.t_mask;
+    for (uint32_t probes = 0; probes <= kMaxProbes; ++probes) {
+        const unsigned long long old = atomicCAS(&mj.table[s], ~0ull, mine);
+        if (probes == 0 && old != 0x5555AAAA5555AAAAull) KPROF(kp, 3);
+        if (old == ~0ull) return;
+        if ((uint32_t)(old >> 32) == tag) {
+            const uint32_t o = (uint32_t)old;
+            if (mj.key[o] == key && (!mj.check || mj.check[o] == chk)) {
+                mj.partner[j] = (int32_t)o;
+                if (atomicExch(&mj.partner[o], (int32_t)j) != -1) mj.counts->irregular = 1;
+                KPROF(kp, 4);
+                return;
+            }
+        }
+        s = (s + 1) & mj.t_mask;
+    }
+    mj.counts->irregular = 1;
+}
+
+template <int kIters>
+__global__ __launch_bounds__(256) void k4_cut_join_kernel(HeadIn hin, HeadOut hout, const uint32_t* n_ptr, unsigned long long* lb_state,
+                                                          uint32_t lb_stamp, uint32_t g_scan, MateJoin mj) {
+    if (blockIdx.x < g_scan) scan_lookback_body<U4, HeadIn, HeadOut, kIters>(hin, hout, n_ptr, lb_state, lb_stamp);
+    else mate_join_body(mj, n_ptr, blockIdx.x - g_scan);
+}
+
+void launch_k4_cut_join(const HeadIn& hin, const HeadOut& hout, const uint32_t* n_ptr, uint32_t n_upper, int iters, unsigned long long* lb_state,
+                        uint32_t lb_stamp, const MateJoin& mj, hipStream_t s) {
+    if (n_upper == 0) return;
+    const uint32_t g_scan = scan_grid(n_upper, iters), g_join = (n_upper + 255) / 256;
+    if (iters == 2) hipLaunchKernelGGL(k4_cut_join_kernel<2>, dim3(g_scan + g_join), dim3(256), 0, s, hin, hout, n_ptr, lb_state, lb_stamp, g_scan, mj);
+    else hipLaunchKernelGGL(k4_cut_join_kernel<1>, dim3(g_scan + g_join), dim3(256), 0, s, hin, hout, n_ptr, lb_state, lb_stamp, g_scan, mj);
+}
+
 void launch_k4_join_only(const K4Arrays& k4, const Entries& en, const uint32_t* n_ptr, uint32_t n_anom_host, StageCounts* counts,
                          hipStream_t s) {
     if (n_anom_host == 0) return;
     const uint32_t g = (n_anom_host + kPartChunk - 1) / kPartChunk;
     if (k4.direct) {
-        const uint32_t gd = (n_anom_host + 255) / 256 + (en.r_rec_host ? kJoinForwardBlocks : 0u);
+        const uint32_t gd = (n_anom_host + 255) / 256;
         hipLaunchKernelGGL(k4_direct_join_kernel, dim3(gd), dim3(256), 0, s, k4, en, n_ptr, counts);
         return;
     }
diff --git a/breakdancer_amd/csrc/k6_assemble.hip b/breakdancer_amd/csrc/k6_assemble.hip
--- a/breakdancer_amd/csrc/k6_assemble.hip
+++ b/breakdancer_amd/csrc/k6_assemble.hip
@@ -92,20 +92,42 @@
     return m;
 }
 
-__global__ __launch_bounds__(256) void k6_pairs_kernel(K6Arrays a) {
+template <bool kBeside>
+__global__ __launch_bounds__(256) void k6_pairs_kernel(K6Arrays a, uint32_t fwd, uint32_t gp) {
     __shared__ PartRec s_stash[4][64];
+    const GroupRec* const in_groups = kBeside ? nullptr : a.in_groups;
+    const uint32_t* const first_of = kBeside ? nullptr : a.first_of;
+    uint8_t* const taint = kBeside ? nullptr : a.taint;
+    const int32_t* const pair_lo = kBeside ? nullptr : a.pair_lo;
+    if (kBeside && blockIdx.x < fwd) {
+        const uint32_t nr = a.counts->n_regions;
+        const uint32_t t = blockIdx.x * 256 + threadIdx.x, gsz = fwd * 256;
+        constexpr uint32_t kw = sizeof(RegionRec) / 4;
+        {
+            const uint32_t words = nr * kw, quads = words / 4;
+            const uint4* src = (const uint4*)a.r_rec;
+            uint4* dst = (uint4*)a.fwd_rec;
+            for (uint32_t i = t; i < quads; i += gsz) dst[i] = src[i];
+            if (t < words - quads * 4) ((uint32_t*)a.fwd_rec)[quads * 4 + t] = ((const uint32_t*)a.r_rec)[quads * 4 + t];
+        }
+        {
+            const uint32_t words = nr * 2u * (uint32_t)a.nkeys, quads = words / 4;
+            const uint4* src = (const uint4*)a.r_pk;
+            uint4* dst = (uint4*)a.fwd_pk;
+            for (uint32_t i = t; i < quads; i += gsz) dst[i] = src[i];
+            if (t < words - quads * 4) a.fwd_pk[quads * 4 + t] = a.r_pk[quads * 4 + t];
+        }
+        return;
+    }
+    const uint32_t pb = blockIdx.x - fwd;
     const int lane = threadIdx.x & 63, w = threadIdx.x >> 6;
-    const uint32_t nwaves = gridDim.x * 4;
-    if (a.flag_regions && blockIdx.x == 0 && threadIdx.x == 0) {
-        __threadfence_system();
-        *(volatile uint32_t*)a.flag_regions = a.flag_value;
-    }
-    if (blockIdx.x == 0 && a.emit_part) a.emit_part[threadIdx.x] = 0;
+    const uint32_t nwaves = gp * 4;
+    if (pb == 0 && a.emit_part) a.emit_part[threadIdx.x] = 0;
     const uint32_t NR = a.counts->n_regions;
     const uint32_t mrp = (uint32_t)max(a.min_read_pair, 0);
-    for (uint32_t r = blockIdx.x * 4 + (threadIdx.x >> 6); r < NR; r += nwaves) {
+    for (uint32_t r = pb * 4 + (threadIdx.x >> 6); r < NR; r += nwaves) {
         const RegionRec rr = a.r_rec[r];
-        const uint32_t first = a.first_of ? a.first_of[r] : rr.first, n = rr.n;
+        const uint32_t first = first_of ? first_of[r] : rr.first, n = rr.n;
         RegSum rs{};
         auto load_read = [&](uint32_t c0, uint64_t& key, uint32_t& is) -> bool {
             const uint32_t i = c0 + lane;
@@ -113,30 +135,33 @@
             is = 0;
             if (i >= n) return false;
             const uint32_t j = first + i;
+            if (kBeside) a.region_out[j] = (int32_t)r;
+            const uint32_t m = a.meta[j];
+            const uint32_t isz = (uint32_t)a.isize[j];
             int32_t plo;
-            if (a.pair_lo) {
-                plo = a.pair_lo[j];
+            if (pair_lo) {
+                plo = pair_lo[j];
             } else {
                 const int32_t p = a.partner[j];
-                plo = (p >= 0 && (uint32_t)p < j) ? a.region_of[p] : -1;
+                plo = -1;
+                if (p >= 0 && (uint32_t)p < j) plo = kBeside ? a.c_rid[a.cand[p]] : a.region_of[p];
             }
             if (plo < 0) return false;
-            const uint32_t m = a.meta[j];
             key = ((uint64_t)(uint32_t)plo << 12) | ((uint64_t)meta_lib(m) << 4) | (uint64_t)meta_flag(m);
-            is = (uint32_t)a.isize[j];
+            is = isz;
             return true;
         };
         uint64_t key = ~0ull;
         uint32_t is = 0;
         bool has = false, merged = false;
         Merged m{};
-        if (a.in_groups) {
+        if (in_groups) {
             const uint32_t g0 = a.in_goff[r], ng = a.in_goff[r + 1] - g0;
             auto load_group = [&](uint32_t c0, uint64_t& k, uint32_t& cnt, uint32_t& sm) -> bool {
                 const uint32_t i = c0 + lane;
                 k = ~0ull; cnt = 0; sm = 0;
                 if (i >= ng) return false;
-                const GroupRec g = a.in_groups[g0 + i];
+                const GroupRec g = in_groups[g0 + i];
                 k = ((g.key >> 38) << 12) | (g.key & 0xFFFull);
                 cnt = g.pairs; sm = g.sum_isize;
                 return true;
@@ -161,7 +186,7 @@
                     if (cm.gleader && clo < r) {
                         atomicAdd(&a.out_deg[clo], 1u);
                         a.bad_v[clo] = 1u;
-                        if (a.taint && a.r_rec[clo].n == 0) { a.taint[clo] = 1; a.taint[r] = 1; }
+                        if (taint && a.r_rec[clo].n == 0) { taint[clo] = 1; taint[r] = 1; }
                     }
                     if (lane == 0) a.bad_v[r] = 1u;
                     const uint32_t nl = (uint32_t)__popcll(cm.lmask);
@@ -225,7 +250,7 @@
                     if (cm.gleader && clo < r) {
                         atomicAdd(&a.out_deg[clo], 1u);
                         a.bad_v[clo] = 1u;
-                        if (a.taint && a.r_rec[clo].n == 0) { a.taint[clo] = 1; a.taint[r] = 1; }
+                        if (taint && a.r_rec[clo].n == 0) { taint[clo] = 1; taint[r] = 1; }
                     }
                     if (lane == 0) a.bad_v[r] = 1u;
                     const uint32_t nl = (uint32_t)__popcll(cm.lmask);
@@ -256,7 +281,7 @@
             const bool in_edge = m.gleader && lo < r && strong;
             const uint64_t gl_in = __ballot(in_edge);
             if (in_edge) atomicAdd(&a.out_deg[lo], 1u);
-            if (a.taint && in_edge && a.r_rec[lo].n == 0) { a.taint[lo] = 1; a.taint[r] = 1; }
+            if (taint && in_edge && a.r_rec[lo].n == 0) { taint[lo] = 1; taint[r] = 1; }
             rs.np_all = (uint32_t)__popcll(m.lmask);
             rs.np_self = (uint32_t)__popcll(__ballot(m.leader && lo == r));
             rs.np_emit = (uint32_t)__popcll(__ballot(m.leader && (lo == r || strong)));
@@ -290,7 +315,15 @@
     }
 }
 
-__global__ __launch_bounds__(256) void k6_label_kernel(K6Arrays a) {
+__device__ __forceinline__ void k6_ready(uint32_t* ready, uint32_t value) {
+    if (ready && blockIdx.x == 0 && threadIdx.x == 0) {
+        __threadfence_system();
+        *(volatile uint32_t*)ready = value;
+    }
+}
+
+__global__ __launch_bounds__(256) void k6_label_kernel(K6Arrays a, uint32_t* ready) {
+    k6_ready(ready, a.flag_value);
     const uint32_t r = blockIdx.x * blockDim.x + threadIdx.x;
     if (r >= a.counts->n_regions) return;
     const RegSum* s = &a.rs[r];
@@ -306,7 +339,8 @@
     if (l2 < l) atomicMin(&a.label[r], l2);
 }
 
-__global__ __launch_bounds__(256) void k6_classify_kernel(K6Arrays a) {
+__global__ __launch_bounds__(256) void k6_classify_kernel(K6Arrays a, uint32_t* ready) {
+    k6_ready(ready, a.flag_value);
     const uint32_t r = blockIdx.x * blockDim.x + threadIdx.x;
     if (r >= a.counts->n_regions) return;
     const RegSum* s = &a.rs[r];
@@ -1586,16 +1620,22 @@
 void launch_k6_pairs(const K6Arrays& a, uint32_t n_anom_host, hipStream_t s) {
     if (n_anom_host == 0) return;
     const uint32_t gp = std::min<uint32_t>((n_anom_host / 8 + 3) / 4 + 1, 16384u);
-    hipLaunchKernelGGL(k6_pairs_kernel, dim3(gp), dim3(256), 0, s, a);
+    const uint32_t fwd = a.fwd_rec ? kJoinForwardBlocks : 0u;
+    if (a.cand) hipLaunchKernelGGL(k6_pairs_kernel<true>, dim3(fwd + gp), dim3(256), 0, s, a, fwd, gp);
+    else hipLaunchKernelGGL(k6_pairs_kernel<false>, dim3(gp), dim3(256), 0, s, a, 0u, gp);
 }
 
 void launch_k6_components(const K6Arrays& a, uint32_t n_anom_host, hipStream_t s) {
     if (n_anom_host == 0) return;
     constexpr uint32_t kRegionThreads = 64;
     const uint32_t grs = (n_anom_host + kRegionThreads - 1) / kRegionThreads;
+    uint32_t* ready = a.flag_regions;
     if (!a.force_host)
-        for (int i = 1; i < a.propagation_rounds; ++i) hipLaunchKernelGGL(k6_label_kernel, dim3(grs), dim3(kRegionThreads), 0, s, a);
-    hipLaunchKernelGGL(k6_classify_kernel, dim3(grs), dim3(kRegionThreads), 0, s, a);
+        for (int i = 1; i < a.propagation_rounds; ++i) {
+            hipLaunchKernelGGL(k6_label_kernel, dim3(grs), dim3(kRegionThreads), 0, s, a, ready);
+            ready = nullptr;
+        }
+    hipLaunchKernelGGL(k6_classify_kernel, dim3(grs), dim3(kRegionThreads), 0, s, a, ready);
     hipLaunchKernelGGL(k6_emit_kernel, dim3(grs), dim3(kRegionThreads), 0, s, a);
     if (a.counts_host && !a.mirror_in_walk) hipLaunchKernelGGL(k6_mirror_kernel, dim3(1), dim3(64), 0, s, a);
 }
```

Result: no change. 29.60 billion (median of 2 runs) (+2.0%).
